# MicahZoltu/lodestar

Measured on AMD Instinct MI355X. Metric: verified signature sets/sec (mainnet attestation mix), higher is better.
Workload: dtype u32 (381-bit Montgomery; device products on 14x28-bit limbs); 1 GPU; c3: gossip attestation flood, 6 slot(s) per batch, 7 batches in flight per GPU; slots_per_batch=6, sets_per_gpu=116736, jobs_per_gpu=104448, pubkeys_per_gpu=1683456, parallelism=dp1 (sets sharded), exchange=False, inflight=7, world_size_seen=1, pubkeys=indices into the GPU-resident table, signing_roots_per_gpu=6918

## Files before the change

### include/lodestar_bls.h

```cpp
#ifndef LODESTAR_BLS_H
#define LODESTAR_BLS_H
#include <stddef.h>
#include <stdint.h>

#ifdef __cplusplus
extern "C" {
#endif

#define LB_OK 0
#define LB_BAD_ENCODING 1
#define LB_POINT_NOT_ON_CURVE 2
#define LB_POINT_NOT_IN_GROUP 3
#define LB_AGGR_TYPE_MISMATCH 4
#define LB_VERIFY_FAIL 5
#define LB_PK_IS_INFINITY 6
#define LB_BAD_SCALAR 7
#define LB_INVALID_SIZE 10
#define LB_EMPTY_AGGREGATE_ARRAY 11
#define LB_EMPTY_SIGNATURE_SET 12
#define LB_ERR_ARGUMENT 100
#define LB_ERR_DEVICE 101
#define LB_ERR_NO_DEVICE 102

typedef struct lb_engine lb_engine;
typedef struct lb_batch lb_batch;

const char* lb_error_name(int32_t code);

int32_t lb_abi_version(void);

int32_t lb_engine_create(int32_t device, lb_engine** out);
#define LB_ENGINE_LATENCY 1u
int32_t lb_engine_create_ex(int32_t device, uint32_t flags, lb_engine** out);
void lb_engine_destroy(lb_engine* e);
int32_t lb_engine_cu_count(const lb_engine* e);

int32_t lb_batch_create(lb_engine* e, uint32_t n_jobs, const uint32_t* job_offsets,
                        const uint32_t* set_pk_offsets, const uint8_t* pubkeys,
                        const uint8_t* signing_roots, const uint8_t* signatures,
                        const uint32_t* sig_sizes, lb_batch** out);
void lb_batch_destroy(lb_batch* b);
uint32_t lb_batch_num_sets(const lb_batch* b);
uint32_t lb_batch_num_jobs(const lb_batch* b);

int32_t lb_batch_verify(lb_engine* e, lb_batch* b, const uint64_t* scalars, int32_t* out_job);

int32_t lb_batch_partial(lb_engine* e, lb_batch* b, const uint64_t* scalars, uint8_t* out576,
                         int32_t* out_job);
int32_t lb_fp12_product_is_one(lb_engine* e, const uint8_t* partials576, uint32_t n, int32_t* ok);
int32_t lb_batch_search_after_partial(lb_engine* e, lb_batch* b, int32_t* out_job);

int32_t lb_verify_jobs(lb_engine* e, uint32_t n_jobs, const uint32_t* job_offsets,
                       const uint32_t* set_pk_offsets, const uint8_t* pubkeys,
                       const uint8_t* signing_roots, const uint8_t* signatures,
                       const uint32_t* sig_sizes, const uint64_t* scalars, int32_t* out_job);
int32_t lb_verify_jobs_indexed(lb_engine* e, uint32_t n_jobs, const uint32_t* job_offsets,
                               const uint32_t* set_pk_offsets, const uint32_t* pk_indices,
                               const uint8_t* signing_roots, const uint8_t* signatures,
                               const uint32_t* sig_sizes, const uint64_t* scalars, int32_t* out_job);

void* lb_host_alloc(size_t bytes);
void lb_host_free(void* p);

int32_t lb_aggregate_pubkeys(lb_engine* e, uint32_t n_sets, const uint32_t* set_pk_offsets,
                             const uint8_t* pubkeys, uint8_t* out96, int32_t* out_status);

int32_t lb_aggregate_signatures(lb_engine* e, uint32_t n_groups, const uint32_t* group_offsets,
                                const uint8_t* sigs96, const uint32_t* sig_sizes, int32_t validate,
                                uint8_t* out96, int32_t* out_status);

int32_t lb_g1_decompress(lb_engine* e, uint32_t n, const uint8_t* in48, uint8_t* out96, int32_t* out_status,
                         int32_t validate);

int32_t lb_merkleize(lb_engine* e, uint32_t n_trees, const uint32_t* chunk_offsets, const uint8_t* chunks32,
                     const uint32_t* depths, const uint64_t* mix_lengths, uint8_t* out_roots32);

int32_t lb_kzg_load_setup(lb_engine* e, const uint8_t* g1_48, uint32_t n_g1, const uint8_t* g2_96, uint32_t n_g2,
                          int32_t* out_status);

int32_t lb_g1_lincomb(lb_engine* e, uint32_t n, const uint8_t* points48, const uint8_t* scalars32, uint8_t* out48);

int32_t lb_kzg_verify_proof(lb_engine* e, const uint8_t* commitment48, const uint8_t* z32, const uint8_t* y32,
                            const uint8_t* proof48, int32_t* ok);

int32_t lb_sk_to_pk(lb_engine* e, uint32_t n, const uint8_t* sks32, uint8_t* out48, uint8_t* out96);
int32_t lb_sign(lb_engine* e, uint32_t n, const uint8_t* sks32, const uint8_t* msgs32, uint8_t* out96);

int32_t lb_pubkey_table_append(lb_engine* e, uint32_t n, const uint8_t* keys, uint32_t key_size, int32_t validate,
                               int32_t* out_status, uint32_t* out_first_index);
uint32_t lb_pubkey_table_size(const lb_engine* e);

int32_t lb_batch_create_indexed(lb_engine* e, uint32_t n_jobs, const uint32_t* job_offsets,
                                const uint32_t* set_pk_offsets, const uint32_t* pk_indices,
                                const uint8_t* signing_roots, const uint8_t* signatures,
                                const uint32_t* sig_sizes, lb_batch** out);

int32_t lb_engine_set_profiling(lb_engine* e, int32_t enable);
int32_t lb_engine_last_profile(lb_engine* e, const char** names, float* ms, int32_t cap, int32_t* n);

#ifdef __cplusplus
}
#endif
#endif
```

### lodestar_amd/_native.py

```python
from __future__ import annotations

import ctypes
import os

LIB_PATH = os.environ.get("LODESTAR_BLS_LIB") or os.path.join(os.path.dirname(os.path.abspath(__file__)),
                                                               "liblodestar_bls.so")

LB_OK = 0
LB_BAD_ENCODING = 1
LB_POINT_NOT_ON_CURVE = 2
LB_POINT_NOT_IN_GROUP = 3
LB_AGGR_TYPE_MISMATCH = 4
LB_VERIFY_FAIL = 5
LB_PK_IS_INFINITY = 6
LB_BAD_SCALAR = 7
LB_INVALID_SIZE = 10
LB_EMPTY_AGGREGATE_ARRAY = 11
LB_EMPTY_SIGNATURE_SET = 12
LB_ERR_ARGUMENT = 100
LB_ERR_DEVICE = 101
LB_ERR_NO_DEVICE = 102


class NativeUnavailable(RuntimeError):
    pass


_u8p = ctypes.POINTER(ctypes.c_uint8)
_u32p = ctypes.POINTER(ctypes.c_uint32)
_u64p = ctypes.POINTER(ctypes.c_uint64)
_i32p = ctypes.POINTER(ctypes.c_int32)
_vp = ctypes.c_void_p

SIGNATURES = {
    "lb_error_name": (ctypes.c_char_p, [ctypes.c_int32]),
    "lb_abi_version": (ctypes.c_int32, []),
    "lb_engine_create": (ctypes.c_int32, [ctypes.c_int32, ctypes.POINTER(_vp)]),
    "lb_engine_create_ex": (ctypes.c_int32, [ctypes.c_int32, ctypes.c_uint32, ctypes.POINTER(_vp)]),
    "lb_engine_destroy": (None, [_vp]),
    "lb_engine_cu_count": (ctypes.c_int32, [_vp]),
    "lb_batch_create": (ctypes.c_int32, [_vp, ctypes.c_uint32, _u32p, _u32p, _u8p, _u8p, _u8p, _u32p,
                                         ctypes.POINTER(_vp)]),
    "lb_batch_destroy": (None, [_vp]),
    "lb_batch_num_sets": (ctypes.c_uint32, [_vp]),
    "lb_batch_num_jobs": (ctypes.c_uint32, [_vp]),
    "lb_batch_verify": (ctypes.c_int32, [_vp, _vp, _u64p, _i32p]),
    "lb_batch_partial": (ctypes.c_int32, [_vp, _vp, _u64p, _u8p, _i32p]),
    "lb_batch_search_after_partial": (ctypes.c_int32, [_vp, _vp, _i32p]),
    "lb_fp12_product_is_one": (ctypes.c_int32, [_vp, _u8p, ctypes.c_uint32, _i32p]),
    "lb_verify_jobs": (ctypes.c_int32, [_vp, ctypes.c_uint32, _u32p, _u32p, _u8p, _u8p, _u8p, _u32p, _u64p,
                                        _i32p]),
    "lb_verify_jobs_indexed": (ctypes.c_int32, [_vp, ctypes.c_uint32, _u32p, _u32p, _u32p, _u8p, _u8p, _u32p,
                                                _u64p, _i32p]),
    "lb_host_alloc": (_vp, [ctypes.c_size_t]),
    "lb_host_free": (None, [_vp]),
    "lb_aggregate_pubkeys": (ctypes.c_int32, [_vp, ctypes.c_uint32, _u32p, _u8p, _u8p, _i32p]),
    "lb_aggregate_signatures": (ctypes.c_int32, [_vp, ctypes.c_uint32, _u32p, _u8p, _u32p, ctypes.c_int32, _u8p,
                                                 _i32p]),
    "lb_g1_decompress": (ctypes.c_int32, [_vp, ctypes.c_uint32, _u8p, _u8p, _i32p, ctypes.c_int32]),
    "lb_merkleize": (ctypes.c_int32, [_vp, ctypes.c_uint32, _u32p, _u8p, _u32p, _u64p, _u8p]),
    "lb_kzg_load_setup": (ctypes.c_int32, [_vp, _u8p, ctypes.c_uint32, _u8p, ctypes.c_uint32, _i32p]),
    "lb_g1_lincomb": (ctypes.c_int32, [_vp, ctypes.c_uint32, _u8p, _u8p, _u8p]),
    "lb_kzg_verify_proof": (ctypes.c_int32, [_vp, _u8p, _u8p, _u8p, _u8p, _i32p]),
    "lb_sk_to_pk": (ctypes.c_int32, [_vp, ctypes.c_uint32, _u8p, _u8p, _u8p]),
    "lb_sign": (ctypes.c_int32, [_vp, ctypes.c_uint32, _u8p, _u8p, _u8p]),
    "lb_pubkey_table_append": (ctypes.c_int32, [_vp, ctypes.c_uint32, _u8p, ctypes.c_uint32, ctypes.c_int32, _i32p,
                                                _u32p]),
    "lb_pubkey_table_size": (ctypes.c_uint32, [_vp]),
    "lb_batch_create_indexed": (ctypes.c_int32, [_vp, ctypes.c_uint32, _u32p, _u32p, _u32p, _u8p, _u8p, _u32p,
                                                 ctypes.POINTER(_vp)]),
    "lb_engine_set_profiling": (ctypes.c_int32, [_vp, ctypes.c_int32]),
    "lb_engine_last_profile": (ctypes.c_int32, [_vp, ctypes.POINTER(ctypes.c_char_p),
                                                ctypes.POINTER(ctypes.c_float), ctypes.c_int32, _i32p]),
}

_lib = None


def load(path: str = LIB_PATH) -> ctypes.CDLL:
    global _lib
    if _lib is not None:
        return _lib
    if not os.path.exists(path):
        raise NativeUnavailable(
            f"{path} not found: build it with `python -m lodestar_amd.build` (hipcc, gfx950)")
    lib = ctypes.CDLL(path)
    for name, (res, args) in SIGNATURES.items():
        fn = getattr(lib, name)
        fn.restype = res
        fn.argtypes = args
    _lib = lib
    return lib


def error_name(code: int) -> str:
    return load().lb_error_name(int(code)).decode()
```

### lodestar_amd/build.py

```python
from __future__ import annotations

import os
import subprocess
import sys
import time

ROOT = os.path.dirname(os.path.dirname(os.path.abspath(__file__)))
CSRC = os.path.join(ROOT, "lodestar_amd", "csrc")
INC = os.path.join(ROOT, "include")
LIB = os.path.join(ROOT, "lodestar_amd", "liblodestar_bls.so")
HARNESS = os.path.join(ROOT, "build", "lb_harness.so")
CPU_POOL = os.path.join(ROOT, "build", "lb_cpu_pool.so")
HIPCC = os.environ.get("HIPCC", "/opt/rocm/bin/hipcc")


def _sources(*names):
    return [os.path.join(CSRC, n) for n in names]


def _stale(target, deps):
    if not os.path.exists(target):
        return True
    t = os.path.getmtime(target)
    return any(os.path.getmtime(d) > t for d in deps)


def _deps():
    hdrs = [os.path.join(CSRC, f) for f in os.listdir(CSRC)]
    return hdrs + [os.path.join(INC, "lodestar_bls.h")]


def _jobs():
    n = os.cpu_count() or 4
    try:
        n = len(os.sched_getaffinity(0))
    except (AttributeError, OSError):
        pass
    return max(1, min(16, n, int(os.environ.get("MAX_JOBS", "16") or 16)))


def build_lib(force=False, verbose=True, extra_flags=(), out=None):
    out = out or LIB
    if not force and not extra_flags and not _stale(out, _deps()):
        return out
    sys.path.insert(0, os.path.join(ROOT, "tools"))
    import gen_kdecls
    cur = open(gen_kdecls.OUT).read() if os.path.exists(gen_kdecls.OUT) else ""
    if cur != gen_kdecls.render():
        with open(gen_kdecls.OUT, "w") as f:
            f.write(gen_kdecls.render())
    odir = os.path.join(ROOT, "build", "obj" + ("" if out == LIB else "_" + os.path.basename(out)))
    os.makedirs(odir, exist_ok=True)
    base = [HIPCC, "--offload-arch=gfx950", "-O3", "-std=c++17", "-fPIC", "-Wno-unused-result",
            "-Wno-unused-value", "-I" + INC, "-I" + CSRC, *extra_flags]
    units = [(os.path.join(CSRC, "lb_engine.hip"), "99", os.path.join(odir, "engine.o"))]
    units += [(os.path.join(CSRC, "lb_kgroup.hip"), str(g), os.path.join(odir, f"kgroup{g}.o"))
              for g in range(gen_kdecls.N_GROUPS)]
    order = [u for u in units if u[1] in ("3", "6", "8", "9", "7")] + [u for u in units if u[1] not in ("3", "6", "8", "9", "7")]
    running, failed = [], []
    t0 = time.time()
    kdeps = [d for d in _deps() if os.path.basename(d) != "lb_engine.hip"]
    pend = [u for u in order if force or extra_flags or _stale(u[2], _deps() if u[1] == "99" else kdeps)]
    while pend or running:
        while pend and len(running) < _jobs():
            src, g, obj = pend.pop(0)
            cmd = base + ["-DLB_KGROUP=" + g, "-c", src, "-o", obj]
            if verbose:
                print("[build]", " ".join(cmd[-5:]), flush=True)
            running.append((subprocess.Popen(cmd), g, time.time()))
        time.sleep(0.2)
        for r in list(running):
            rc = r[0].poll()
            if rc is not None:
                running.remove(r)
                if verbose:
                    print(f"[build] group {r[1]} done in {time.time() - r[2]:.0f} s (rc {rc})", flush=True)
                if rc != 0:
                    failed.append(r[1])
    if failed:
        raise subprocess.CalledProcessError(1, f"hipcc (groups {failed})")
    cmd = [HIPCC, "--offload-arch=gfx950", "-shared", "-fPIC", *[u[2] for u in units], "-o", out + ".tmp"]
    subprocess.run(cmd, check=True)
    os.replace(out + ".tmp", out)
    if verbose:
        print(f"[build] {out} in {time.time() - t0:.0f} s", flush=True)
    return out


def build_harness(force=False, verbose=True):
    src = os.path.join(ROOT, "tests", "harness", "lb_harness.cpp")
    os.makedirs(os.path.dirname(HARNESS), exist_ok=True)
    if not force and not _stale(HARNESS, _deps() + [src]):
        return HARNESS
    cmd = ["g++", "-O2", "-shared", "-fPIC", "-I" + INC, "-I" + CSRC, src, "-o", HARNESS + ".tmp"]
    if verbose:
        print("[build]", " ".join(cmd), flush=True)
    subprocess.run(cmd, check=True)
    os.replace(HARNESS + ".tmp", HARNESS)
    return HARNESS


def build_cpu_pool(force=False, verbose=True):
    src = os.path.join(ROOT, "oracle", "cpu_pool.cpp")
    if not os.path.exists(src):
        return None
    os.makedirs(os.path.dirname(CPU_POOL), exist_ok=True)
    if not force and not _stale(CPU_POOL, _deps() + [src]):
        return CPU_POOL
    cmd = ["g++", "-O3", "-shared", "-fPIC", "-pthread", "-I" + INC, "-I" + CSRC, src,
           "-o", CPU_POOL + ".tmp"]
    if verbose:
        print("[build]", " ".join(cmd), flush=True)
    subprocess.run(cmd, check=True)
    os.replace(CPU_POOL + ".tmp", CPU_POOL)
    return CPU_POOL


UBENCH = ["fpmul_asm"]


def build_ubench(force=False, verbose=True):
    out = []
    for name in UBENCH:
        src = os.path.join(ROOT, "tools", "ubench", name + ".hip")
        dst = os.path.join(ROOT, "tools", "ubench", name)
        if force or _stale(dst, _deps() + [src]):
            cmd = [HIPCC, "--offload-arch=gfx950", "-O3", "-std=c++17", "-Wno-unused-result", "-Wno-unused-value",
                   "-I" + INC, "-I" + CSRC, src, "-o", dst]
            if verbose:
                print("[build]", " ".join(cmd), flush=True)
            subprocess.run(cmd, check=True)
        out.append(dst)
    return out


NAPI = os.path.join(ROOT, "lodestar_amd", "napi", "lodestar_bls.node")


def build_napi(force=False, verbose=True):
    src = os.path.join(ROOT, "lodestar_amd", "napi", "lb_napi.c")
    hdr = "/usr/include/node/node_api.h"
    if not os.path.exists(hdr):
        return None
    if not force and not _stale(NAPI, [src, LIB, os.path.join(INC, "lodestar_bls.h")]):
        return NAPI
    cmd = ["gcc", "-O2", "-shared", "-fPIC", "-pthread", "-I/usr/include/node", "-I" + INC, src, "-o", NAPI + ".tmp",
           "-L" + os.path.dirname(LIB), "-llodestar_bls", "-Wl,-rpath,$ORIGIN/.."]
    if verbose:
        print("[build]", " ".join(cmd), flush=True)
    subprocess.run(cmd, check=True)
    os.replace(NAPI + ".tmp", NAPI)
    return NAPI


def build_all(force=False):
    build_lib(force)
    build_napi(force)
    build_harness(force)
    build_cpu_pool(force)
    build_ubench(force)


if __name__ == "__main__":
    build_all(force="--force" in sys.argv)
```

### lodestar_amd/csrc/lb_curve.h

```cpp
#pragma once
#include "lb_field.h"

template <class F>
struct jac {
  F x, y, z;
};
template <class F>
struct aff {
  F x, y;
};

typedef jac<fp> g1j;
typedef jac<fp2> g2j;
typedef aff<fp> g1a;
typedef aff<fp2> g2a;

template <class T, class S>
LB_HD aff<T> aff_as(const aff<S>& a) {
  return aff<T>{T{a.x}, T{a.y}};
}
template <class T, class S>
LB_HD jac<T> jac_as(const jac<S>& a) {
  return jac<T>{T{a.x}, T{a.y}, T{a.z}};
}
// ... 22 lines not shown
LB_HD jac<F> jac_neg(const jac<F>& p) {
  return jac<F>{p.x, f_neg(p.y), p.z};
}

template <class F>
LB_HD jac<F> jac_dbl_i(const jac<F>& p) {
  F A = f_sqr(p.x);
  F B = f_sqr(p.y);
  F C = f_sqr(B);
  F D = f_dbl(f_sub(f_sub(f_sqr(f_add(p.x, B)), A), C));
  F E = f_mul3(A);
  F Fv = f_sqr(E);
  jac<F> r;
  r.x = f_sub(Fv, f_dbl(D));
  r.y = f_sub(f_mul(E, f_sub(D, r.x)), f_mul8(C));
  r.z = f_dbl(f_mul(p.y, p.z));
  return r;
}

template <class F>
LB_NI jac<F> jac_dbl(jac<F> p) {
  return jac_dbl_i(p);
}

template <class F, bool kInl = false>
LB_HD jac<F> jac_add_i(const jac<F>& p, const jac<F>& q) {
  if (jac_is_inf(p)) return q;
  if (jac_is_inf(q)) return p;
  F Z1Z1 = f_sqr(p.z);
  F Z2Z2 = f_sqr(q.z);
  F U1 = f_mul(p.x, Z2Z2);
  F U2 = f_mul(q.x, Z1Z1);
  F S1 = f_mul(f_mul(p.y, q.z), Z2Z2);
  F S2 = f_mul(f_mul(q.y, p.z), Z1Z1);
  F H = f_sub(U2, U1);
  F rr = f_dbl(f_sub(S2, S1));
  if (f_is_zero(H)) {
    if (f_is_zero(rr)) {
      if constexpr (kInl) return jac_dbl_i(p);
      else return jac_dbl(p);
    }
    return jac_infinity<F>();
  }
  F I = f_sqr(f_dbl(H));
  F J = f_mul(H, I);
  F V = f_mul(U1, I);
  jac<F> r;
  r.x = f_sub(f_sub(f_sqr(rr), J), f_dbl(V));
  r.y = f_sub(f_mul(rr, f_sub(V, r.x)), f_dbl(f_mul(S1, J)));
  r.z = f_mul(f_sub(f_sub(f_sqr(f_add(p.z, q.z)), Z1Z1), Z2Z2), H);
  return r;
}

template <class F>
LB_NI jac<F> jac_add(jac<F> p, jac<F> q) {
  return jac_add_i(p, q);
}

template <class F, bool kInl = false>
LB_HD jac<F> jac_add_aff_i(const jac<F>& p, const aff<F>& q) {
  if (jac_is_inf(p)) return jac_from_aff(q);
  F Z1Z1 = f_sqr(p.z);
  F U2 = f_mul(q.x, Z1Z1);
  F S2 = f_mul(f_mul(q.y, p.z), Z1Z1);
  F H = f_sub(U2, p.x);
  F rr = f_dbl(f_sub(S2, p.y));
  if (f_is_zero(H)) {
    if (f_is_zero(rr)) {
      if constexpr (kInl) return jac_dbl_i(p);
      else return jac_dbl(p);
    }
    return jac_infinity<F>();
  }
  F HH = f_sqr(H);
  F I = f_dbl(f_dbl(HH));
  F J = f_mul(H, I);
  F V = f_mul(p.x, I);
  jac<F> r;
  r.x = f_sub(f_sub(f_sqr(rr), J), f_dbl(V));
  r.y = f_sub(f_mul(rr, f_sub(V, r.x)), f_dbl(f_mul(p.y, J)));
  r.z = f_sub(f_sub(f_sqr(f_add(p.z, H)), Z1Z1), HH);
  return r;
}

template <class F>
LB_NI jac<F> jac_add_aff(jac<F> p, aff<F> q) {
  return jac_add_aff_i(p, q);
}

template <class F>
LB_NI bool jac_eq(jac<F> p, jac<F> q) {
  bool pi = jac_is_inf(p), qi = jac_is_inf(q);
  if (pi || qi) return pi && qi;
  F Z1Z1 = f_sqr(p.z), Z2Z2 = f_sqr(q.z);
  if (!f_eq(f_mul(p.x, Z2Z2), f_mul(q.x, Z1Z1))) return false;
  return f_eq(f_mul(f_mul(p.y, q.z), Z2Z2), f_mul(f_mul(q.y, p.z), Z1Z1));
}

template <class F>
LB_NI bool jac_to_aff(aff<F>& out, jac<F> p) {
  F zi = f_inv(p.z);
  F zi2 = f_sqr(zi);
  out.x = f_mul(p.x, zi2);
  out.y = f_mul(f_mul(p.y, zi2), zi);
  return !jac_is_inf(p);
}

LB_HD void g1_to_aff_inl(g1a& out, const g1j& p) {
  const fp zi = fp_inv_i(p.z), zi2 = fp_sqr(zi);
  out.x = fp_mul(p.x, zi2);
  out.y = fp_mul(fp_mul(p.y, zi2), zi);
}
LB_HD void g2_to_aff_inl(g2a& out, const g2j& p) {
  const fp ni = fp_inv_i(fp_add(fp_sqr(p.z.c0), fp_sqr(p.z.c1)));
  const fp2 zi{fp_mul(p.z.c0, ni), fp_neg(fp_mul(p.z.c1, ni))};
  const fp2 zi2 = fp2_sqr(zi);
  out.x = fp2_mul(p.x, zi2);
  out.y = fp2_mul(fp2_mul(p.y, zi2), zi);
}

template <class F>
LB_NI jac<F> jac_mul_u64(aff<F> p, uint64_t k) {
  jac<F> acc = jac_infinity<F>();
  for (int i = 63; i >= 0; i--) {
    acc = jac_dbl_i(acc);
    if ((k >> i) & 1ull) acc = jac_add_aff_i(acc, p);
  }
  return acc;
}

template <class F, bool kInl = false>
LB_HD jac<F> jac_mul_2d_i(const aff<F>& t1, const aff<F>& t2, const aff<F>& t3, uint64_t k0, uint64_t k1, int bits) {
  jac<F> acc = jac_infinity<F>();
  for (int i = bits - 1; i >= 0; i--) {
    acc = jac_dbl_i(acc);
    const uint32_t d = (uint32_t)((k0 >> i) & 1u) | ((uint32_t)((k1 >> i) & 1u) << 1);
    aff<F> t;
    t.x = d == 1u ? t1.x : (d == 2u ? t2.x : t3.x);
    t.y = d == 1u ? t1.y : (d == 2u ? t2.y : t3.y);
    jac<F> s = jac_add_aff_i<F, kInl>(acc, t);
    if (d != 0u) acc = s;
  }
  return acc;
}
template <class F, bool kInl = false>
LB_HD jac<F> jac_mul_glv_i(const aff<F>& t1, const aff<F>& t2, const aff<F>& t3, uint64_t w) {
  return jac_mul_2d_i<F, kInl>(t1, t2, t3, w & 0xffffffffu, w >> 32, 32);
}
template <class F>
LB_NI jac<F> jac_mul_glv(aff<F> t1, aff<F> t2, aff<F> t3, uint64_t w) {
  return jac_mul_glv_i(t1, t2, t3, w);
}

template <class F>
LB_NI jac<F> jac_mul_u64_jac(jac<F> p, uint64_t k) {
  jac<F> acc = jac_infinity<F>();
  for (int i = 63; i >= 0; i--) {
    acc = jac_dbl_i(acc);
    if ((k >> i) & 1ull) acc = jac_add_i(acc, p);
  }
  return acc;
}

template <class F>
LB_NI jac<F> jac_mul_u256(aff<F> p, const uint32_t* k) {
  jac<F> acc = jac_infinity<F>();
  for (int i = 255; i >= 0; i--) {
    acc = jac_dbl_i(acc);
    if ((k[i >> 5] >> (i & 31)) & 1u) acc = jac_add_aff_i(acc, p);
  }
  return acc;
}

template <class F, bool kInl = false>
LB_HD jac<F> jac_mul_xabs_i(const jac<F>& p) {
  jac<F> acc = p;
  for (int i = 62; i >= 0; i--) {
    acc = jac_dbl_i(acc);
    if ((LB_X_ABS >> i) & 1ull) acc = jac_add_i<F, kInl>(acc, p);
  }
  return acc;
}
template <class F>
LB_NI jac<F> jac_mul_xabs(jac<F> p) {
  return jac_mul_xabs_i(p);
}

LB_HD g2j g2_psi(const g2j& p) {
  g2j r;
  r.x = fp2_mul(fp2_conj(p.x), fp2_load(LB_PSI_CX));
  r.y = fp2_mul(fp2_conj(p.y), fp2_load(LB_PSI_CY));
  r.z = fp2_conj(p.z);
  return r;
}
LB_HD g2j g2_psi2(const g2j& p) {
  g2j r;
  r.x = fp2_mul_fp(p.x, fp_load(LB_PSI2_CX));
  r.y = fp2_mul_fp(p.y, fp_load(LB_PSI2_CY));
  r.z = p.z;
  return r;
}

LB_HD bool g2_in_subgroup(const g2j& p) {
  if (jac_is_inf(p)) return true;
  g2j xp = jac_neg(jac_mul_xabs(p));
  return jac_eq(g2_psi(p), xp);
}

template <bool kInl>
LB_HD fp lean_mul(const fp& a, const fp& b) {
#if defined(__HIP_DEVICE_COMPILE__)
  if constexpr (kInl) {
    __builtin_amdgcn_sched_barrier(0);
    fp r = fp_mul28(a, b);
    __builtin_amdgcn_sched_barrier(0);
    return r;
  }
#endif
  return fp_mul(a, b);
}
template <bool kInl>
LB_HD fp lean_sqr(const fp& a) {
#if defined(__HIP_DEVICE_COMPILE__)
  if constexpr (kInl) {
    __builtin_amdgcn_sched_barrier(0);
    fp r = fp_sqr28(a);
    __builtin_amdgcn_sched_barrier(0);
    return r;
  }
#endif
  return fp_sqr(a);
}
template <bool kInl>
LB_HD fp2 lean2_mul(const fp2& a, const fp2& b) {
  fp t0 = lean_mul<kInl>(a.c0, b.c0);
  fp t1 = lean_mul<kInl>(a.c1, b.c1);
  fp t2 = lean_mul<kInl>(fp_add(a.c0, a.c1), fp_add(b.c0, b.c1));
  return fp2{fp_sub(t0, t1), fp_sub(fp_sub(t2, t0), t1)};
}
template <bool kInl>
LB_HD fp2 lean2_sqr(const fp2& a) {
  fp t0 = lean_mul<kInl>(fp_add(a.c0, a.c1), fp_sub(a.c0, a.c1));
  fp t1 = lean_mul<kInl>(a.c0, a.c1);
  return fp2{t0, fp_dbl(t1)};
}
template <bool kInl>
LB_HD void g2_dbl_lean(g2j& p) {
  p.z = fp2_dbl(lean2_mul<kInl>(p.y, p.z));
  fp2 B = lean2_sqr<kInl>(p.y);
  fp2 C = lean2_sqr<kInl>(B);
  fp2 A = lean2_sqr<kInl>(p.x);
  fp2 D = lean2_sqr<kInl>(fp2_add(p.x, B));
  D = fp2_dbl(fp2_sub(fp2_sub(D, A), C));
  fp2 E = fp2_mul3(A);
  p.x = fp2_sub(lean2_sqr<kInl>(E), fp2_dbl(D));
  p.y = fp2_sub(lean2_mul<kInl>(E, fp2_sub(D, p.x)), fp2_mul8(C));
}
template <bool kInl>
LB_HD void g2_add_aff_lean(g2j& p, const g2a& q) {
  fp2 Z1Z1 = lean2_sqr<kInl>(p.z);
  fp2 H = fp2_sub(lean2_mul<kInl>(q.x, Z1Z1), p.x);
  fp2 rr = lean2_mul<kInl>(lean2_mul<kInl>(q.y, p.z), Z1Z1);
  rr = fp2_dbl(fp2_sub(rr, p.y));
  if (fp2_is_zero(H)) {
    if (fp2_is_zero(rr)) {
      g2_dbl_lean<kInl>(p);
    } else {
      p = jac_infinity<fp2>();
    }
    return;
  }
  fp2 HH = lean2_sqr<kInl>(H);
  p.z = fp2_sub(fp2_sub(lean2_sqr<kInl>(fp2_add(p.z, H)), Z1Z1), HH);
  fp2 I = fp2_mul4(HH);
  fp2 J = lean2_mul<kInl>(H, I);
  fp2 V = lean2_mul<kInl>(p.x, I);
  fp2 YJ = fp2_dbl(lean2_mul<kInl>(p.y, J));
  p.x = fp2_sub(fp2_sub(lean2_sqr<kInl>(rr), J), fp2_dbl(V));
  p.y = fp2_sub(lean2_mul<kInl>(rr, fp2_sub(V, p.x)), YJ);
}

template <bool kInl>
LB_HD void g2_add_lean(g2j& p, const g2j& q) {
  if (jac_is_inf(q)) return;
  if (jac_is_inf(p)) {
    p = q;
    return;
  }
  const fp2 Z1Z1 = lean2_sqr<kInl>(p.z), Z2Z2 = lean2_sqr<kInl>(q.z);
  const fp2 ZZ = fp2_sub(fp2_sub(lean2_sqr<kInl>(fp2_add(p.z, q.z)), Z1Z1), Z2Z2);
  const fp2 U1 = lean2_mul<kInl>(p.x, Z2Z2);
  const fp2 S1 = lean2_mul<kInl>(lean2_mul<kInl>(p.y, q.z), Z2Z2);
  const fp2 H = fp2_sub(lean2_mul<kInl>(q.x, Z1Z1), U1);
  const fp2 rr = fp2_dbl(fp2_sub(lean2_mul<kInl>(lean2_mul<kInl>(q.y, p.z), Z1Z1), S1));
  if (fp2_is_zero(H)) {
    if (fp2_is_zero(rr)) {
      p = q;
      g2_dbl_lean<kInl>(p);
    } else {
      p = jac_infinity<fp2>();
    }
    return;
  }
  p.z = lean2_mul<kInl>(ZZ, H);
  const fp2 I = lean2_sqr<kInl>(fp2_dbl(H));
  const fp2 J = lean2_mul<kInl>(H, I);
// ... 39 lines not shown
```

### lodestar_amd/csrc/lb_engine.hip

```cpp
#include <hip/hip_runtime.h>
#include <hip/hip_ext.h>
#include <stdio.h>
#include <stdlib.h>
#include <string.h>
#include <sys/random.h>

#include <algorithm>
#include <chrono>
#include <cstdio>
#include <cstdlib>
#include <atomic>
#include <mutex>
#include <string>
#include <vector>

#include "lb_kernels.h"
#include "lb_kzg.h"
#include "lb_kdecl.h"

#define LB_ABI_VERSION 1

namespace {

struct dbuf {
  void* p = nullptr;
  size_t cap = 0;
  bool view = false;
  hipError_t ensure(size_t bytes) {
    if (view) {
      p = nullptr;
      cap = 0;
      view = false;
    }
    if (bytes <= cap) return hipSuccess;
    if (p) hipFree(p);
    p = nullptr;
    cap = 0;
    size_t want = bytes + bytes / 4 + 4096;
    hipError_t e = hipMalloc(&p, want);
    if (e == hipSuccess) cap = want;
    return e;
  }
  void release() {
    if (p && !view) hipFree(p);
    p = nullptr;
    cap = 0;
    view = false;
  }
  void set_view(void* q, size_t bytes) {
    if (p && !view) hipFree(p);
    p = q;
    cap = bytes;
    view = true;
  }
  template <class T>
  T* as() const { return reinterpret_cast<T*>(p); }
};

enum {
  ST_DECODE = 0,
  ST_DEDUP,
  ST_HASH_MAP,
  ST_HASH_FIN,
  ST_PK_CHUNKS,
  ST_PK_BLIND,
  ST_SIG_MSM,
  ST_GSUM,
  ST_MILLER,
  ST_TREE_P,
  ST_ML_S,
  ST_ROOT,
  ST_FALLBACK,
  ST_BISECT,
  ST_TOTAL,
  kStages
};
const char* const kStageNames[kStages] = {"decode_sigs", "dedup",   "hash_map", "hash_finish", "pk_chunks",
                                          "pk_blind",    "sig_msm", "group_sum", "miller",    "tree_up_P",
                                          "ml_S",        "root_check", "search_msm", "search_check", "total"};

}

struct lb_batch {
  uint32_t n_jobs = 0, n_sets = 0, n_pks = 0;
  uint64_t serial = 0;
  std::vector<uint32_t> job_off;
  std::vector<uint32_t> h_set_chunk_off, h_chunk_lo;
  uint32_t n_chunks = 0;
  bool indexed = false;
  dbuf d_job_off, d_pk_off, d_pks, d_msgs, d_sigs, d_sig_sizes, d_set_chunk_off, d_chunk_lo;
  dbuf d_arena;
  bool has_sizes = false;
  int device = 0;
  ~lb_batch() {
    d_job_off.release();
    d_arena.release();
    d_pk_off.release();
    d_pks.release();
    d_msgs.release();
    d_sigs.release();
    d_sig_sizes.release();
    d_set_chunk_off.release();
    d_chunk_lo.release();
  }
};

#ifndef LB_SEARCH_CHUNK_DEF
#define LB_SEARCH_CHUNK_DEF 8
#endif
struct lb_engine {
  int device = 0;
  bool latency = false;
  int n_cus = 0;
  hipStream_t stream = nullptr;
  hipStream_t stream2 = nullptr;
  hipStream_t stream3 = nullptr;
  hipStream_t hp[3] = {nullptr, nullptr, nullptr};
  uint32_t prio_max = 0;
  hipEvent_t ev_g1 = nullptr, ev_s = nullptr, ev_fork = nullptr, ev_dec = nullptr, ev_pk = nullptr;
  hipEvent_t ev_pkst = nullptr;
  hipEvent_t ev_sdec = nullptr, ev_sblind = nullptr;
  std::mutex mu;
  dbuf scalars, sig_aff, sig_inf, sig_status, q, h_aff, rpk, rsig, pk_status, ml, treeP, treeS, job_status,
      nodes, verdict, parts, ok, chunk_acc, chunk_status, fS;
  dbuf msg_tab, rep_of, uid_of, uniq_set, n_u, set_uid, gcnt, gpos, goff, gch, chunk_beg, chunk_end, members,
      set_live, gacc, gp_aff, gp_inf, chunk_root;
  uint32_t gmax_chunks = 0;
  bool straus = false, straus_run = false, rpk_stale = false;
  bool gsum_wave = true;
  dbuf pk3, corder;
  bool gsum_tree = true;
  bool alone = false, row_fe = true;
  int alone_force = -1;
  uint32_t gchunk = LB_GROUP_CHUNK;
  dbuf sig_aos, bcnt, bcursor, boff, bch, bchunk_beg, bchunk_end, bmembers, bacc, bsum, wsum;
  dbuf park;
  bool spec_gsum = false;
  dbuf set_spec, live_flag;
  uint32_t* h_flag = nullptr;
  uint64_t partial_serial = 0;
  uint32_t partial_mu = 0;
  bool msm_g8 = true;
  dbuf sx[32];
  dbuf pk_aff;
  dbuf y_root;
  uint64_t msg_key = 0;
  uint32_t miller_wave_max = 2048;
  uint32_t row_max = 256;
  int miller_form = 0;
  uint32_t miller_lds3_max = 32768;
  uint32_t hash_g8_max = 2048;
  uint32_t hash_row_max = 256;
  uint32_t hash_row_careful = 0;
  bool row_proj = true;
  bool small_par = true;
  uint32_t dec_row_max = 4096;
  uint32_t subgroup_g8_max = 4096;
  uint32_t small_s_max = 32768;
  uint32_t small_s_g8_max = 2048;
  uint32_t search_small_max = 32768;
  bool search_merge = true;
  dbuf s_terms, s_part;
  dbuf s_root, rs_idx, s_set;
  bool search_rootsum = true;
  bool search_pre = false;
  int smsm_form = 0;
  uint32_t search_chunk = LB_SEARCH_CHUNK_DEF;
  bool search_blk = true;
  bool root_shuffle = true;
  std::vector<uint64_t> h_scalars;
  dbuf table;
  uint32_t table_n = 0, table_cap = 0;
  dbuf kzg_g1, kzg_g2;
  uint32_t kzg_n = 0;
  bool profiling = false;
  hipEvent_t ev0[kStages] = {}, ev1[kStages] = {};
  bool used[kStages] = {};
  float last_ms[kStages] = {};
  float acc_ms[kStages] = {};
  uint32_t* h_nu = nullptr;
  void* h_stage = nullptr;
  size_t h_stage_cap = 0;
  lb_batch* scratch = nullptr;
};

static std::mutex g_engine_mu;
static int g_engine_count[64];
static std::atomic<uint64_t> g_batch_serial{0};
#ifndef LB_HASH_ALONE_G8
#define LB_HASH_ALONE_G8 1
#endif
static std::atomic<int> g_device_busy[64];
struct exit_rec {
  const void* eng = nullptr;
  int64_t ns = 0;
};
static std::mutex g_exit_mu[64];
static exit_rec g_device_exit[64][2];
static int64_t lb_now_ns() {
  return std::chrono::duration_cast<std::chrono::nanoseconds>(std::chrono::steady_clock::now().time_since_epoch()).count();
}
static int g_latency_cus[64];
static int g_latency_live[64];
struct busy_scope {
  int dev;
  const void* eng;
  bool counted;
  busy_scope(int d, const void* e, bool latency = false) : dev(d), eng(e), counted(!latency) {
    if (counted) g_device_busy[dev].fetch_add(1, std::memory_order_relaxed);
  }
  ~busy_scope() {
    if (!counted) return;
    {
      std::lock_guard<std::mutex> lk(g_exit_mu[dev]);
      exit_rec* r = g_device_exit[dev];
      if (r[0].eng != eng) r[1] = r[0];
      r[0] = exit_rec{eng, lb_now_ns()};
    }
    g_device_busy[dev].fetch_sub(1, std::memory_order_relaxed);
  }
};
#ifndef LB_ALONE_GRACE_MS
#define LB_ALONE_GRACE_MS 20
#endif
template <class E>
static bool device_alone(const E* e) {
  if (e->latency) return true;
  if (e->alone_force >= 0) return e->alone_force != 0;
  if (g_device_busy[e->device].load(std::memory_order_relaxed) > 1) return false;
  int64_t other;
  {
    std::lock_guard<std::mutex> lk(g_exit_mu[e->device]);
    const exit_rec* r = g_device_exit[e->device];
    other = r[0].eng != (const void*)e ? r[0].ns : r[1].ns;
  }
  return other == 0 || lb_now_ns() - other > (int64_t)LB_ALONE_GRACE_MS * 1000000;
}
static int max_engines_per_device() {
  const char* v = getenv("LB_MAX_ENGINES_PER_DEVICE");
  int k = v ? atoi(v) : 0;
  return k > 0 ? k : 10;
}

#define LB_HIP(call)                                                                        \
  do {                                                                                      \
    hipError_t _e = (call);                                                                 \
    if (_e != hipSuccess) {                                                                 \
      fprintf(stderr, "lodestar_bls: %s failed: %s (%s:%d)\n", #call, hipGetErrorString(_e), \
              __FILE__, __LINE__);                                                          \
      return LB_ERR_DEVICE;                                                                 \
    }                                                                                       \
  } while (0)

static inline uint32_t nblk(uint32_t n) { return (n + LB_TPB - 1) / LB_TPB; }
static inline uint32_t nblk_inv(uint32_t n) { return (n + LB_INV_TPB - 1) / LB_INV_TPB; }

static int fill_scalars(lb_engine* e, uint32_t n, const uint64_t* user, bool unblinded) {
  e->h_scalars.resize(n);
  if (!user && n == 1 && unblinded) {
    e->h_scalars[0] = 1;
    return LB_OK;
  }
  if (user) {
    for (uint32_t i = 0; i < n; i++)
      if (user[i] == 0) return LB_BAD_SCALAR;
    memcpy(e->h_scalars.data(), user, (size_t)n * 8);
  } else {
    size_t need = (size_t)n * 8, got = 0;
    uint8_t* dst = reinterpret_cast<uint8_t*>(e->h_scalars.data());
    while (got < need) {
      ssize_t r = getrandom(dst + got, need - got, 0);
      if (r < 0) return LB_ERR_DEVICE;
      got += (size_t)r;
    }
    for (uint32_t i = 0; i < n; i++)
      while (e->h_scalars[i] == 0) getrandom(&e->h_scalars[i], 8, 0);
  }
  return LB_OK;
}

extern "C" {

int32_t lb_abi_version(void) { return LB_ABI_VERSION; }

const char* lb_error_name(int32_t code) {
  switch (code) {
    case LB_OK: return "BLST_SUCCESS";
    case LB_BAD_ENCODING: return "BLST_BAD_ENCODING";
    case LB_POINT_NOT_ON_CURVE: return "BLST_POINT_NOT_ON_CURVE";
    case LB_POINT_NOT_IN_GROUP: return "BLST_POINT_NOT_IN_GROUP";
    case LB_AGGR_TYPE_MISMATCH: return "BLST_AGGR_TYPE_MISMATCH";
    case LB_VERIFY_FAIL: return "BLST_VERIFY_FAIL";
    case LB_PK_IS_INFINITY: return "BLST_PK_IS_INFINITY";
    case LB_BAD_SCALAR: return "BLST_BAD_SCALAR";
    case LB_INVALID_SIZE: return "BLST_INVALID_SIZE";
    case LB_EMPTY_AGGREGATE_ARRAY: return "EMPTY_AGGREGATE_ARRAY";
    case LB_EMPTY_SIGNATURE_SET: return "Empty signature set";
    case LB_ERR_ARGUMENT: return "LB_ERR_ARGUMENT";
    case LB_ERR_DEVICE: return "LB_ERR_DEVICE";
    case LB_ERR_NO_DEVICE: return "LB_ERR_NO_DEVICE";
    default: return "LB_UNKNOWN_ERROR";
  }
}

int32_t lb_engine_create(int32_t device, lb_engine** out) { return lb_engine_create_ex(device, 0u, out); }
static std::vector<uint32_t> cu_mask(int ncu, int lo, int hi) {
  std::vector<uint32_t> m((size_t)(ncu + 31) / 32, 0u);
  for (int c = lo; c < hi && c < ncu; c++) m[(size_t)c / 32] |= 1u << (c % 32);
  return m;
}
int32_t lb_engine_create_ex(int32_t device, uint32_t flags, lb_engine** out) {
  if (!out || (flags & ~LB_ENGINE_LATENCY)) return LB_ERR_ARGUMENT;
  *out = nullptr;
  int count = 0;
  if (hipGetDeviceCount(&count) != hipSuccess || count == 0) return LB_ERR_NO_DEVICE;
  if (device < 0) LB_HIP(hipGetDevice(&device));
  if (device >= count) return LB_ERR_NO_DEVICE;
  hipDeviceProp_t prop;
  LB_HIP(hipGetDeviceProperties(&prop, device));
  if (strncmp(prop.gcnArchName, "gfx950", 6) != 0) {
    fprintf(stderr, "lodestar_bls: device %d is %s, this build targets gfx950 only\n", device, prop.gcnArchName);
    return LB_ERR_NO_DEVICE;
  }
  LB_HIP(hipSetDevice(device));
  if (device >= 64) return LB_ERR_NO_DEVICE;
  {
    std::lock_guard<std::mutex> lk(g_engine_mu);
    if (g_engine_count[device] >= max_engines_per_device()) {
      fprintf(stderr, "lodestar_bls: engine limit (%d per device) reached on device %d\n", max_engines_per_device(),
              device);
      return LB_ERR_DEVICE;
    }
    g_engine_count[device]++;
  }
  lb_engine* e = new lb_engine();
  e->device = device;
  while (getrandom(&e->msg_key, 8, 0) != 8) {
  }
  int prio_least = 0, prio_greatest = 0;
  hipDeviceGetStreamPriorityRange(&prio_least, &prio_greatest);
  if (const char* mw = getenv("LB_MILLER_WAVE_MAX")) e->miller_wave_max = (uint32_t)strtoul(mw, nullptr, 10);
  if (const char* rm = getenv("LB_ROW_MAX")) e->row_max = (uint32_t)strtoul(rm, nullptr, 10);
  if (const char* gt = getenv("LB_GSUM_TREE")) e->gsum_tree = std::atoi(gt) != 0;
  if (const char* gs = getenv("LB_GSUM_STRAUS")) e->straus = std::atoi(gs) != 0;
  if (const char* gw = getenv("LB_GSUM_WAVE")) e->gsum_wave = std::atoi(gw) != 0;
  if (const char* rf = getenv("LB_ROW_FE")) e->row_fe = std::atoi(rf) != 0;
  if (const char* pm = getenv("LB_PRIO_MAX")) e->prio_max = (uint32_t)strtoul(pm, nullptr, 10);
  if (const char* ml = getenv("LB_MILLER_LDS3_MAX")) e->miller_lds3_max = (uint32_t)strtoul(ml, nullptr, 10);
  if (const char* mf = getenv("LB_MILLER_FORM")) e->miller_form = !strcmp(mf, "lane") ? 1 : !strcmp(mf, "g8") ? 2 : 0;
  if (const char* hg = getenv("LB_HASH_G8_MAX")) e->hash_g8_max = (uint32_t)strtoul(hg, nullptr, 10);
  if (const char* hr = getenv("LB_HASH_ROW_MAX")) e->hash_row_max = (uint32_t)strtoul(hr, nullptr, 10);
  if (const char* dr = getenv("LB_DEC_ROW_MAX")) e->dec_row_max = (uint32_t)strtoul(dr, nullptr, 10);
  if (const char* hc = getenv("LB_HASH_ROW_CAREFUL")) e->hash_row_careful = (uint32_t)strtoul(hc, nullptr, 10);
  if (const char* rp = getenv("LB_ROW_PROJ")) e->row_proj = std::atoi(rp) != 0;
  if (const char* sp = getenv("LB_SMALL_PAR")) e->small_par = std::atoi(sp) != 0;
  if (const char* sg = getenv("LB_SUBGROUP_G8_MAX")) e->subgroup_g8_max = (uint32_t)strtoul(sg, nullptr, 10);
  if (const char* ss = getenv("LB_SMALL_S_MAX")) e->small_s_max = (uint32_t)strtoul(ss, nullptr, 10);
  if (const char* sg8 = getenv("LB_SMALL_S_G8_MAX")) e->small_s_g8_max = (uint32_t)strtoul(sg8, nullptr, 10);
  if (const char* sm = getenv("LB_SEARCH_SMALL_MAX")) e->search_small_max = (uint32_t)strtoul(sm, nullptr, 10);
  if (const char* sm = getenv("LB_SEARCH_MERGE")) e->search_merge = std::atoi(sm) != 0;
  if (const char* sm = getenv("LB_SEARCH_ROOTSUM")) e->search_rootsum = std::atoi(sm) != 0;
  if (const char* sm = getenv("LB_SEARCH_PRE")) e->search_pre = std::atoi(sm) != 0;
  if (const char* sf = getenv("LB_SMSM_FORM")) e->smsm_form = !strcmp(sf, "lane") ? 1 : !strcmp(sf, "g8") ? 2 : 0;
  if (const char* sc = getenv("LB_SEARCH_CHUNK")) {
    const uint32_t v = (uint32_t)strtoul(sc, nullptr, 10);
    if (v >= 1 && v <= 64) e->search_chunk = v;
  }
  if (const char* sm = getenv("LB_SEARCH_BLOCKS")) e->search_blk = std::atoi(sm) != 0;
  if (const char* sm = getenv("LB_ROOT_SHUFFLE")) e->root_shuffle = std::atoi(sm) != 0;
  if (const char* sm = getenv("LB_MSM_G8")) e->msm_g8 = std::atoi(sm) != 0;
  if (const char* sm = getenv("LB_SPEC_GSUM")) e->spec_gsum = std::atoi(sm) != 0;
  if (const char* al = getenv("LB_ALONE")) e->alone_force = std::atoi(al) != 0 ? 1 : 0;
  bool masked = false;
  std::vector<uint32_t> mask;
  {
    std::lock_guard<std::mutex> lk(g_engine_mu);
    const int ncu = prop.multiProcessorCount;
    e->n_cus = ncu;
    if (flags & LB_ENGINE_LATENCY) {
      if (g_latency_cus[device] == 0) {
        const char* v = getenv("LB_LATENCY_CUS");
        const int r = v ? atoi(v) : 8;
        g_latency_cus[device] = std::max(1, std::min(r, ncu / 4));
        if (g_engine_count[device] > 1)
          fprintf(stderr, "lodestar_bls: latency engine created after %d other engine(s) on device %d: "
                  "those still run on every CU (create the latency engine first)\n", g_engine_count[device] - 1, device);
      }
      g_latency_live[device]++;
      e->latency = true;
      mask = cu_mask(ncu, 0, g_latency_cus[device]);
      e->n_cus = g_latency_cus[device];
      masked = true;
    } else if (g_latency_cus[device] > 0) {
      mask = cu_mask(ncu, g_latency_cus[device], ncu);
      e->n_cus = ncu - g_latency_cus[device];
      masked = true;
    }
  }
  auto mk = [&](hipStream_t* st, bool prio) {
    if (masked) return hipExtStreamCreateWithCUMask(st, (uint32_t)mask.size(), mask.data());
    return prio ? hipStreamCreateWithPriority(st, hipStreamNonBlocking, prio_least)
                : hipStreamCreateWithFlags(st, hipStreamNonBlocking);
  };
  if (mk(&e->stream, true) != hipSuccess || mk(&e->stream2, false) != hipSuccess || mk(&e->stream3, false) != hipSuccess ||

      hipHostMalloc((void**)&e->h_nu, 8, hipHostMallocDefault) != hipSuccess ||
      hipHostMalloc((void**)&e->h_flag, 4, hipHostMallocDefault) != hipSuccess) {
    if (e->stream) hipStreamDestroy(e->stream);
    if (e->stream2) hipStreamDestroy(e->stream2);
    if (e->stream3) hipStreamDestroy(e->stream3);
    if (e->h_nu) hipHostFree(e->h_nu);
    std::lock_guard<std::mutex> lk(g_engine_mu);
    g_engine_count[device]--;
    if (e->latency && --g_latency_live[device] == 0) g_latency_cus[device] = 0;
    delete e;
    return LB_ERR_DEVICE;
  }
  hipEventCreateWithFlags(&e->ev_g1, hipEventDisableTiming);
  hipEventCreateWithFlags(&e->ev_s, hipEventDisableTiming);
  hipEventCreateWithFlags(&e->ev_fork, hipEventDisableTiming);
  hipEventCreateWithFlags(&e->ev_dec, hipEventDisableTiming);
  hipEventCreateWithFlags(&e->ev_pk, hipEventDisableTiming);
  hipEventCreateWithFlags(&e->ev_pkst, hipEventDisableTiming);
  hipEventCreateWithFlags(&e->ev_sdec, hipEventDisableTiming);
  hipEventCreateWithFlags(&e->ev_sblind, hipEventDisableTiming);
  for (int i = 0; i < kStages; i++) {
    hipEventCreate(&e->ev0[i]);
    hipEventCreate(&e->ev1[i]);
  }
  {
    bool ok;
    {
      std::lock_guard<std::mutex> lk(g_engine_mu);
      ok = e->n_u.ensure(4) == hipSuccess && hipMemsetAsync(e->n_u.p, 0, 4, e->stream) == hipSuccess;
      if (ok) {
        hipLaunchKernelGGL(k_miller_lane<2>, dim3(4096), dim3(LB_TPB), 0, e->stream, 0u, 1u, e->n_u.as<uint32_t>(),
                           nullptr, nullptr, nullptr, nullptr, nullptr);
        hipLaunchKernelGGL(k_hash_finish, dim3(4096), dim3(LB_INV_TPB), 0, e->stream, 0u, e->n_u.as<uint32_t>(),
                           nullptr, nullptr, nullptr, 0u);
        const char* rv = getenv("LB_RESERVE_S23");
        const int res23 = rv ? atoi(rv) : 2;
        if (res23 >= 1) {
          hipLaunchKernelGGL(k_decompress_sigs, dim3(4096), dim3(LB_TPB), 0, e->stream2, 0u, nullptr, nullptr, nullptr,
                             nullptr, nullptr, nullptr);
          hipLaunchKernelGGL(k_pk_chunks, dim3(4096), dim3(LB_TPB), 0, e->stream3, 0u, nullptr, nullptr, nullptr, nullptr);
          hipLaunchKernelGGL(k_pk_blind_rowp, dim3(std::max<uint32_t>(1u, e->row_max)), dim3(64), 0, e->stream3,
                             0u, nullptr, nullptr, nullptr, nullptr);
        }
        if (res23 >= 2) {
          auto g8_waves = [](uint32_t sets) { return dim3(std::min<uint32_t>(16384u, std::max<uint32_t>(1u, sets / 8 + 1))); };
          hipLaunchKernelGGL(k_sig_subgroup_g8, g8_waves(e->subgroup_g8_max), dim3(64), 0, e->stream2, 0u, nullptr,
                             nullptr, nullptr);
          hipLaunchKernelGGL(k_sig_blind_g8, g8_waves(e->small_s_g8_max), dim3(64), 0, e->stream2, 0u, nullptr, nullptr,
                             nullptr, nullptr, nullptr);
        }
        ok = hipGetLastError() == hipSuccess && hipStreamSynchronize(e->stream) == hipSuccess &&
             hipStreamSynchronize(e->stream2) == hipSuccess && hipStreamSynchronize(e->stream3) == hipSuccess;
      }
    }
    if (!ok) {
      fprintf(stderr, "lodestar_bls: engine scratch reservation failed on device %d\n", device);
      lb_engine_destroy(e);
      return LB_ERR_DEVICE;
    }
  }
  *out = e;
  return LB_OK;
}

void lb_engine_destroy(lb_engine* e) {
  if (!e) return;
  hipSetDevice(e->device);
  hipStreamSynchronize(e->stream);
  dbuf* bufs[] = {&e->scalars, &e->sig_aff, &e->sig_inf, &e->sig_status, &e->q, &e->h_aff, &e->rpk, &e->rsig,
                  &e->pk_status, &e->ml, &e->treeP, &e->treeS, &e->job_status, &e->nodes, &e->verdict, &e->parts,
                  &e->ok, &e->chunk_acc, &e->chunk_status, &e->fS, &e->table, &e->msg_tab,
                  &e->rep_of, &e->uid_of, &e->uniq_set, &e->n_u, &e->set_uid, &e->gcnt, &e->gpos, &e->goff,
                  &e->gch, &e->chunk_beg, &e->chunk_end, &e->members, &e->set_live, &e->gacc, &e->gp_aff,
                  &e->gp_inf, &e->chunk_root, &e->sig_aos, &e->bcnt, &e->bcursor, &e->boff, &e->bch, &e->bchunk_beg,
                  &e->bchunk_end, &e->bmembers, &e->bacc, &e->bsum, &e->wsum, &e->park, &e->set_spec, &e->live_flag, &e->pk_aff, &e->y_root, &e->kzg_g1,
                  &e->kzg_g2, &e->s_terms, &e->s_part, &e->s_root, &e->rs_idx, &e->s_set, &e->pk3, &e->corder};
  for (dbuf* b : bufs) b->release();
  for (dbuf& b : e->sx) b.release();
  for (int i = 0; i < kStages; i++) {
    if (e->ev0[i]) hipEventDestroy(e->ev0[i]);
    if (e->ev1[i]) hipEventDestroy(e->ev1[i]);
  }
  hipEventDestroy(e->ev_g1);
  hipEventDestroy(e->ev_s);
  hipEventDestroy(e->ev_fork);
  hipEventDestroy(e->ev_dec);
  hipEventDestroy(e->ev_pk);
  if (e->ev_pkst) hipEventDestroy(e->ev_pkst);
  if (e->ev_sdec) hipEventDestroy(e->ev_sdec);
  if (e->ev_sblind) hipEventDestroy(e->ev_sblind);
  hipStreamSynchronize(e->stream2);
  hipStreamSynchronize(e->stream3);
  if (e->scratch) delete e->scratch;
  if (e->h_nu) hipHostFree(e->h_nu);
  if (e->h_flag) hipHostFree(e->h_flag);
  if (e->h_stage) hipHostFree(e->h_stage);
  hipStreamDestroy(e->stream2);
  hipStreamDestroy(e->stream3);
  hipStreamDestroy(e->stream);
  for (hipStream_t h : e->hp)
    if (h) {
      hipStreamSynchronize(h);
      hipStreamDestroy(h);
    }
  {
    std::lock_guard<std::mutex> lk(g_engine_mu);
    g_engine_count[e->device]--;
    if (e->latency && --g_latency_live[e->device] == 0) g_latency_cus[e->device] = 0;
  }
  delete e;
}

int32_t lb_engine_cu_count(const lb_engine* e) { return e ? e->n_cus : 0; }

int32_t lb_engine_set_profiling(lb_engine* e, int32_t enable) {
  if (!e) return LB_ERR_ARGUMENT;
  e->profiling = enable != 0;
  return LB_OK;
}

int32_t lb_engine_last_profile(lb_engine* e, const char** names, float* ms, int32_t cap, int32_t* n) {
  if (!e || !n) return LB_ERR_ARGUMENT;
  int k = cap < kStages ? cap : kStages;
  for (int i = 0; i < k; i++) {
    if (names) names[i] = kStageNames[i];
    if (ms) ms[i] = e->last_ms[i];
  }
  *n = k;
  return LB_OK;
}

}

static constexpr size_t kStageMax = (size_t)1 << 20;
static int32_t batch_fill(lb_engine* e, lb_batch* b, uint32_t n_jobs, const uint32_t* job_offsets,
                          const uint32_t* set_pk_offsets, const uint8_t* pubkeys, const uint32_t* pk_indices,
                          const uint8_t* signing_roots, const uint8_t* signatures, const uint32_t* sig_sizes) {
  if (!e || !job_offsets || !set_pk_offsets) return LB_ERR_ARGUMENT;
  if (job_offsets[0] != 0) return LB_ERR_ARGUMENT;
  for (uint32_t j = 0; j < n_jobs; j++)
    if (job_offsets[j + 1] < job_offsets[j]) return LB_ERR_ARGUMENT;
  const uint32_t n_sets = job_offsets[n_jobs];
  if (set_pk_offsets[0] != 0) return LB_ERR_ARGUMENT;
  for (uint32_t i = 0; i < n_sets; i++)
    if (set_pk_offsets[i + 1] < set_pk_offsets[i]) return LB_ERR_ARGUMENT;
  const uint32_t n_pks = set_pk_offsets[n_sets];
  if (n_pks & LB_CHUNK_FIRST) return LB_ERR_ARGUMENT;
  const bool indexed = pk_indices != nullptr;
  if ((n_sets && (!signing_roots || !signatures)) || (n_pks && !pubkeys && !indexed)) return LB_ERR_ARGUMENT;
  LB_HIP(hipSetDevice(e->device));
  b->device = e->device;
  b->serial = g_batch_serial.fetch_add(1, std::memory_order_relaxed) + 1;
  b->n_jobs = n_jobs;
  b->n_sets = n_sets;
  b->n_pks = n_pks;
  b->job_off.assign(job_offsets, job_offsets + n_jobs + 1);
  b->has_sizes = sig_sizes != nullptr;
  auto up = [&](dbuf& d, const void* src, size_t bytes) -> hipError_t {
    hipError_t r = d.ensure(bytes ? bytes : 16);
    if (r != hipSuccess || !bytes) return r;
    return hipMemcpyAsync(d.p, src, bytes, hipMemcpyHostToDevice, e->stream);
  };
  std::vector<uint32_t>& set_chunk_off = b->h_set_chunk_off;
  std::vector<uint32_t>& chunk_lo = b->h_chunk_lo;
  set_chunk_off.resize(n_sets + 1);
  chunk_lo.clear();
  const uint32_t pkc = n_sets <= e->row_max ? LB_PK_CHUNK_SMALL : LB_PK_CHUNK;
  for (uint32_t i = 0; i < n_sets; i++) {
    set_chunk_off[i] = (uint32_t)chunk_lo.size();
    for (uint32_t k = set_pk_offsets[i]; k < set_pk_offsets[i + 1]; k += pkc)
      chunk_lo.push_back(k | (k == set_pk_offsets[i] ? LB_CHUNK_FIRST : 0u));
  }
  set_chunk_off[n_sets] = (uint32_t)chunk_lo.size();
  b->n_chunks = (uint32_t)chunk_lo.size();
  chunk_lo.push_back(n_pks | LB_CHUNK_FIRST);
  b->indexed = indexed;
  struct part {
    dbuf* d;
    const void* src;
    size_t bytes;
  };
  const part parts[] = {{&b->d_job_off, job_offsets, (size_t)(n_jobs + 1) * 4},
                        {&b->d_set_chunk_off, set_chunk_off.data(), set_chunk_off.size() * 4},
                        {&b->d_chunk_lo, chunk_lo.data(), chunk_lo.size() * 4},
                        {&b->d_pk_off, set_pk_offsets, (size_t)(n_sets + 1) * 4},
                        {&b->d_pks, indexed ? (const void*)pk_indices : (const void*)pubkeys,
                         (size_t)n_pks * (indexed ? 4 : 96)},
                        {&b->d_msgs, signing_roots, (size_t)n_sets * 32},
                        {&b->d_sigs, signatures, (size_t)n_sets * 96},
                        {&b->d_sig_sizes, sig_sizes, sig_sizes ? (size_t)n_sets * 4 : 0}};
  size_t total = 0;
  for (const part& q : parts) total += ((q.bytes > 16 ? q.bytes : 16) + 255) & ~(size_t)255;
  bool staged = total <= kStageMax;
  if (staged && e->h_stage_cap < total) {
    if (e->h_stage) hipHostFree(e->h_stage);
    e->h_stage = nullptr;
    e->h_stage_cap = 0;
    if (hipHostMalloc(&e->h_stage, kStageMax, hipHostMallocDefault) == hipSuccess) e->h_stage_cap = kStageMax;
    else staged = false;
  }
  hipError_t r = hipSuccess;
  if (staged) {
    r = b->d_arena.ensure(total);
    size_t off = 0;
    for (const part& q : parts) {
      if (q.bytes) memcpy(static_cast<uint8_t*>(e->h_stage) + off, q.src, q.bytes);
      off += ((q.bytes > 16 ? q.bytes : 16) + 255) & ~(size_t)255;
    }
    if (r == hipSuccess) r = hipMemcpyAsync(b->d_arena.p, e->h_stage, total, hipMemcpyHostToDevice, e->stream);
    off = 0;
    for (const part& q : parts) {
      const size_t sz = ((q.bytes > 16 ? q.bytes : 16) + 255) & ~(size_t)255;
      if (r == hipSuccess && (q.bytes || q.d != &b->d_sig_sizes)) q.d->set_view(static_cast<uint8_t*>(b->d_arena.p) + off, sz);
      off += sz;
    }
  } else {
    for (const part& q : parts)
      if (r == hipSuccess && (q.bytes || q.d != &b->d_sig_sizes)) r = up(*q.d, q.src, q.bytes);
  }
  if (r == hipSuccess) r = hipStreamSynchronize(e->stream);
  if (r != hipSuccess) {
    for (const part& q : parts) q.d->release();
    b->d_arena.release();
    b->n_jobs = b->n_sets = b->n_pks = b->n_chunks = 0;
    b->job_off.assign(1, 0u);
    fprintf(stderr, "lodestar_bls: batch upload failed: %s\n", hipGetErrorString(r));
    return LB_ERR_DEVICE;
  }
  return LB_OK;
}

static int32_t batch_create(lb_engine* e, uint32_t n_jobs, const uint32_t* job_offsets, const uint32_t* set_pk_offsets,
                            const uint8_t* pubkeys, const uint32_t* pk_indices, const uint8_t* signing_roots,
                            const uint8_t* signatures, const uint32_t* sig_sizes, lb_batch** out) {
  if (!e || !out) return LB_ERR_ARGUMENT;
  *out = nullptr;
  std::lock_guard<std::mutex> lk(e->mu);
  lb_batch* b = new lb_batch();
  int32_t st = batch_fill(e, b, n_jobs, job_offsets, set_pk_offsets, pubkeys, pk_indices, signing_roots, signatures,
                          sig_sizes);
  if (st != LB_OK) {
    delete b;
    return st;
  }
  *out = b;
  return LB_OK;
}

static const uint32_t kNoIndices[1] = {0};
static int32_t check_null_indices(uint32_t n_jobs, const uint32_t* job_offsets, const uint32_t* set_pk_offsets) {
  if (!job_offsets || !set_pk_offsets) return LB_ERR_ARGUMENT;
  return set_pk_offsets[job_offsets[n_jobs]] == 0 ? LB_OK : LB_ERR_ARGUMENT;
}

extern "C" {

int32_t lb_batch_create(lb_engine* e, uint32_t n_jobs, const uint32_t* job_offsets, const uint32_t* set_pk_offsets,
                        const uint8_t* pubkeys, const uint8_t* signing_roots, const uint8_t* signatures,
                        const uint32_t* sig_sizes, lb_batch** out) {
  return batch_create(e, n_jobs, job_offsets, set_pk_offsets, pubkeys, nullptr, signing_roots, signatures, sig_sizes,
                      out);
}

int32_t lb_batch_create_indexed(lb_engine* e, uint32_t n_jobs, const uint32_t* job_offsets,
                                const uint32_t* set_pk_offsets, const uint32_t* pk_indices,
                                const uint8_t* signing_roots, const uint8_t* signatures, const uint32_t* sig_sizes,
                                lb_batch** out) {
  if (!pk_indices) {
    const int32_t st = check_null_indices(n_jobs, job_offsets, set_pk_offsets);
    if (st != LB_OK) return st;
    pk_indices = kNoIndices;
  }
  return batch_create(e, n_jobs, job_offsets, set_pk_offsets, nullptr, pk_indices, signing_roots, signatures,
                      sig_sizes, out);
}

void* lb_host_alloc(size_t bytes) {
  void* p = nullptr;
  if (hipHostMalloc(&p, bytes ? bytes : 1, hipHostMallocDefault) != hipSuccess) return nullptr;
  return p;
}

void lb_host_free(void* p) {
  if (p) hipHostFree(p);
}

uint32_t lb_pubkey_table_size(const lb_engine* e) { return e ? e->table_n : 0; }

int32_t lb_pubkey_table_append(lb_engine* e, uint32_t n, const uint8_t* keys, uint32_t key_size, int32_t validate,
                               int32_t* out_status, uint32_t* out_first_index) {
  if (!e || (n && (!keys || !out_status)) || (key_size != 48 && key_size != 96)) return LB_ERR_ARGUMENT;
  std::lock_guard<std::mutex> lk(e->mu);
  LB_HIP(hipSetDevice(e->device));
  const uint32_t first = e->table_n;
  if (out_first_index) *out_first_index = first;
  if (!n) return LB_OK;
  const uint32_t need = first + n;
  if (need > e->table_cap) {
    uint32_t cap = e->table_cap ? e->table_cap : 1024;
    while (cap < need) cap *= 2;
    dbuf nt;
    LB_HIP(nt.ensure((size_t)cap * LB_TABLE_REC * 4));
    if (first)
      LB_HIP(hipMemcpyAsync(nt.p, e->table.p, (size_t)first * LB_TABLE_REC * 4, hipMemcpyDeviceToDevice, e->stream));
    LB_HIP(hipStreamSynchronize(e->stream));
    e->table.release();
    e->table = nt;
    e->table_cap = cap;
  }
  dbuf kin, st;
  hipError_t r = kin.ensure((size_t)n * key_size);
  if (r == hipSuccess) r = st.ensure((size_t)n * 4);
  if (r == hipSuccess) r = hipMemcpyAsync(kin.p, keys, (size_t)n * key_size, hipMemcpyHostToDevice, e->stream);
  if (r == hipSuccess) {
    hipLaunchKernelGGL(k_table_fill, dim3(nblk(n)), dim3(LB_TPB), 0, e->stream, n, kin.as<uint8_t>(), key_size,
                       validate, first, e->table.as<uint32_t>(), st.as<int32_t>());
    r = hipGetLastError();
  }
  if (r == hipSuccess) r = hipMemcpyAsync(out_status, st.p, (size_t)n * 4, hipMemcpyDeviceToHost, e->stream);
  if (r == hipSuccess) r = hipStreamSynchronize(e->stream);
  kin.release();
  st.release();
  if (r != hipSuccess) {
    fprintf(stderr, "lodestar_bls: pubkey table append failed: %s\n", hipGetErrorString(r));
    return LB_ERR_DEVICE;
  }
  e->table_n = need;
  return LB_OK;
}

void lb_batch_destroy(lb_batch* b) {
  if (!b) return;
  hipSetDevice(b->device);
  delete b;
}
uint32_t lb_batch_num_sets(const lb_batch* b) { return b ? b->n_sets : 0; }
uint32_t lb_batch_num_jobs(const lb_batch* b) { return b ? b->n_jobs : 0; }

}

struct stage_scope {
  lb_engine* e;
  int k;
  hipStream_t st;
  stage_scope(lb_engine* e_, int k_, hipStream_t st_) : e(e_), k(k_), st(st_) {
    if (e->profiling) {
      hipEventRecord(e->ev0[k], st);
      e->used[k] = true;
    }
  }
  ~stage_scope() {
    if (e->profiling) hipEventRecord(e->ev1[k], st);
  }
};

static hipError_t msm_reduce(lb_engine* e, hipStream_t st, uint32_t bcap, uint32_t nb, uint32_t n_inst, int W,
                             uint32_t* out, uint32_t n_out, uint32_t out0, uint64_t entries, uint32_t chunk) {
  if (e->msm_g8) {
    hipError_t r = e->wsum.ensure((size_t)n_inst * W * sizeof(g2j));
    if (r != hipSuccess) return r;
    if (entries >= (uint64_t)4 * chunk * nb && device_alone(e))
      hipLaunchKernelGGL(k_msm_buckets_g8, dim3(nb), dim3(64), 0, st, e->bch.as<uint32_t>(), e->bacc.as<uint32_t>(),
                         bcap, e->bsum.as<uint32_t>(), nb);
    else
      hipLaunchKernelGGL(k_msm_buckets, dim3(nblk(nb)), dim3(LB_TPB), 0, st, e->bch.as<uint32_t>(),
                         e->bacc.as<uint32_t>(), bcap, e->bsum.as<uint32_t>(), nb);
    hipLaunchKernelGGL(k_msm_window_g8, dim3(n_inst * W), dim3(256), 0, st, e->bsum.as<uint32_t>(), nb,
                       e->wsum.as<uint32_t>(), n_inst * W);
    if (W == LB_MSM_W)
      hipLaunchKernelGGL(k_msm_horner_g8<LB_MSM_W>, dim3((n_inst + 7) / 8), dim3(64), 0, st, e->wsum.as<uint32_t>(),
                         n_inst, out, n_out, out0);
    else
      hipLaunchKernelGGL(k_msm_horner_g8<LB_SMSM_W>, dim3((n_inst + 7) / 8), dim3(64), 0, st, e->wsum.as<uint32_t>(),
                         n_inst, out, n_out, out0);
    return hipGetLastError();
  }
  hipLaunchKernelGGL(k_msm_buckets, dim3(nblk(nb)), dim3(LB_TPB), 0, st, e->bch.as<uint32_t>(), e->bacc.as<uint32_t>(),
                     bcap, e->bsum.as<uint32_t>(), nb);
  if (W == LB_MSM_W)
    hipLaunchKernelGGL(k_msm_reduce<LB_MSM_W>, dim3(n_inst), dim3(64 * LB_MSM_W), 0, st, e->bsum.as<uint32_t>(), nb, out,
                       n_out, out0);
  else
    hipLaunchKernelGGL(k_msm_reduce<LB_SMSM_W>, dim3(n_inst), dim3(64 * LB_SMSM_W), 0, st, e->bsum.as<uint32_t>(), nb,
                       out, n_out, out0);
  return hipGetLastError();
}

static hipError_t per_root_chain(lb_engine* e, uint32_t n, uint32_t nuh, uint32_t mu, const uint32_t* live) {
  hipStream_t s1 = e->stream;
  const uint32_t* nu = e->n_u.as<uint32_t>();
  {
    stage_scope sc(e, ST_GSUM, s1);
    const uint32_t nch = nuh + n / e->gchunk;
    const bool wave = e->gsum_tree && e->alone && e->gsum_wave;
    if (wave)
      hipLaunchKernelGGL(k_gsum_wave, dim3(nblk(nch)), dim3(LB_TPB), 0, s1, n, nu, e->gch.as<uint32_t>(),
                         e->chunk_beg.as<uint32_t>(), e->chunk_end.as<uint32_t>(), e->chunk_root.as<uint32_t>(),
                         e->members.as<uint32_t>(), live, e->rpk.as<uint32_t>(), e->gacc.as<uint32_t>());
    else if (e->straus_run) {
      hipError_t r = e->corder.ensure((size_t)(nch + 2 * (LB_STRAUS_CHUNK + 1)) * 4);
      if (r != hipSuccess) return r;
      uint32_t* cnt = e->corder.as<uint32_t>() + nch;
      r = hipMemsetAsync(cnt, 0, (size_t)2 * (LB_STRAUS_CHUNK + 1) * 4, s1);
      if (r != hipSuccess) return r;
      for (uint32_t pass = 0; pass < 2; pass++)
        hipLaunchKernelGGL(k_chunk_order, dim3(nblk(nch)), dim3(LB_TPB), 0, s1, nu, e->gch.as<uint32_t>(),
                           e->chunk_beg.as<uint32_t>(), e->chunk_end.as<uint32_t>(), cnt, e->corder.as<uint32_t>(), pass);
      hipLaunchKernelGGL(k_gsum_straus, dim3(nblk(nch)), dim3(LB_TPB), 0, s1, n, nu, e->gch.as<uint32_t>(),
                         e->chunk_beg.as<uint32_t>(), e->chunk_end.as<uint32_t>(), e->corder.as<uint32_t>(),
                         e->members.as<uint32_t>(), live, e->pk3.as<uint32_t>(), e->scalars.as<uint64_t>(),
                         e->gacc.as<uint32_t>());
    }
    else
      hipLaunchKernelGGL(k_gsum_chunks, dim3(nblk(nch)), dim3(LB_TPB), 0, s1, n, nu,
                         e->gch.as<uint32_t>(), e->chunk_beg.as<uint32_t>(), e->chunk_end.as<uint32_t>(),
                         e->members.as<uint32_t>(), live, e->rpk.as<uint32_t>(), e->gacc.as<uint32_t>());
    const bool tree = e->gsum_tree && e->alone && !wave;
    for (uint32_t st = 1; tree && st < e->gmax_chunks; st *= LB_GSUM_FAN)
      hipLaunchKernelGGL(k_gsum_tree, dim3(nblk(nch)), dim3(LB_TPB), 0, s1, n, nu, e->gch.as<uint32_t>(),
                         e->chunk_root.as<uint32_t>(), st, e->gacc.as<uint32_t>());
    hipLaunchKernelGGL(k_gsum_final, dim3(nblk_inv(nuh)), dim3(LB_INV_TPB), 0, s1, n, nu, e->gch.as<uint32_t>(),
                       e->gacc.as<uint32_t>(), e->gp_aff.as<uint32_t>(), e->gp_inf.as<uint32_t>(),
                       wave ? 2u : (tree ? 0u : 1u));
  }
  {
    stage_scope sc(e, ST_MILLER, s1);
    const bool shared = e->miller_form == 1 ||
                        (e->miller_form == 0 && !device_alone(e));
    if (nuh <= e->row_max && e->alone && e->row_fe) {
      hipLaunchKernelGGL(k_miller_row, dim3(nuh), dim3(LBR_NT), 0, s1, n, mu, nu, e->gp_aff.as<uint32_t>(),
                         e->gp_inf.as<uint32_t>(), e->h_aff.as<uint32_t>(), e->treeP.as<uint32_t>());
    } else if (nuh <= e->miller_wave_max) {
      hipLaunchKernelGGL(k_miller_wave, dim3(nuh), dim3(64), 0, s1, n, mu, nu, e->gp_aff.as<uint32_t>(),
                         e->gp_inf.as<uint32_t>(), e->h_aff.as<uint32_t>(), e->treeP.as<uint32_t>());
    } else if (shared) {
      hipError_t r = e->park.ensure((size_t)2 * 72 * 4 * n);
      if (r != hipSuccess) return r;
      if (nuh <= e->miller_lds3_max)
        hipLaunchKernelGGL(k_miller_lane<3>, dim3(nblk(nuh)), dim3(LB_TPB), 0, s1, n, mu, nu, e->gp_aff.as<uint32_t>(),
                           e->gp_inf.as<uint32_t>(), e->h_aff.as<uint32_t>(), e->treeP.as<uint32_t>(),
                           e->park.as<uint32_t>());
      else
        hipLaunchKernelGGL(k_miller_lane<2>, dim3(nblk(nuh)), dim3(LB_TPB), 0, s1, n, mu, nu, e->gp_aff.as<uint32_t>(),
                           e->gp_inf.as<uint32_t>(), e->h_aff.as<uint32_t>(), e->treeP.as<uint32_t>(),
                           e->park.as<uint32_t>());
    } else {
      hipLaunchKernelGGL(k_miller_g8, dim3((nuh + LBG_ROOTS - 1) / LBG_ROOTS), dim3(64 * LBG_WAVES), 0, s1, n, mu, nu,
                         e->gp_aff.as<uint32_t>(), e->gp_inf.as<uint32_t>(), e->h_aff.as<uint32_t>(),
                         e->treeP.as<uint32_t>());
    }
  }
  {
    stage_scope sc(e, ST_TREE_P, s1);
    for (uint32_t lo = mu / 2; lo >= 1; lo /= 2) {
      if (lo <= e->row_max && e->alone && e->row_fe)
        hipLaunchKernelGGL(k_tree_up_row, dim3(lo), dim3(LBR_NT), 0, s1, mu, lo, nu, e->treeP.as<uint32_t>());
      else
        hipLaunchKernelGGL(k_tree_up_U, dim3(lo), dim3(64), 0, s1, mu, lo, nu, e->treeP.as<uint32_t>());
    }
  }
  return hipGetLastError();
}

static int32_t run_pipeline(lb_engine* e, lb_batch* b, const uint64_t* scalars, uint32_t& mj, uint32_t& mu,
                            bool unblinded) {
  const uint32_t n = b->n_sets, nj = b->n_jobs;
  e->partial_serial = 0;
  e->alone = device_alone(e);
  e->straus_run = e->straus && !e->alone;
  e->rpk_stale = e->straus_run;
  e->gchunk = (e->alone && e->gsum_tree) ? (e->gsum_wave ? LB_GROUP_CHUNK_WAVE : LB_GROUP_CHUNK_ALONE)
                                          : (e->straus_run ? LB_STRAUS_CHUNK : LB_GROUP_CHUNK);
  const bool one_unblinded = n == 1 && !scalars && unblinded;
  int st = fill_scalars(e, n, scalars, unblinded);
  if (st != LB_OK) return st;
  mj = 1;
  while (mj < nj) mj <<= 1;
  mu = 1;
  while (mu < n) mu <<= 1;
  const uint32_t mt = mj > mu ? mj : mu;
  const uint32_t ns = n ? n : 1;
  uint32_t cap = 64;
  while (cap < 2 * ns) cap <<= 1;
  LB_HIP(e->scalars.ensure((size_t)ns * 8));
  LB_HIP(e->sig_aff.ensure((size_t)ns * sizeof(g2a)));
  LB_HIP(e->sig_inf.ensure((size_t)ns * 4));
  LB_HIP(e->sig_status.ensure((size_t)ns * 4));
  LB_HIP(e->q.ensure((size_t)ns * 2 * sizeof(g2j)));
  LB_HIP(e->h_aff.ensure((size_t)ns * sizeof(g2a)));
  LB_HIP(e->rpk.ensure((size_t)ns * sizeof(g1j)));
  LB_HIP(e->pk_aff.ensure((size_t)ns * sizeof(g1a)));
  LB_HIP(e->pk_status.ensure((size_t)ns * 4));
  LB_HIP(e->treeP.ensure((size_t)2 * mt * sizeof(fp12)));
  LB_HIP(e->treeS.ensure((size_t)2 * mj * sizeof(g2j)));
  LB_HIP(e->job_status.ensure((size_t)(nj ? nj : 1) * 4));
  LB_HIP(e->fS.ensure(sizeof(fp12)));
  LB_HIP(e->msg_tab.ensure((size_t)cap * 4));
  dbuf* per_set[] = {&e->rep_of, &e->uid_of, &e->uniq_set, &e->set_uid, &e->gcnt, &e->gpos, &e->chunk_beg,
                     &e->chunk_end, &e->members, &e->set_live, &e->gp_inf, &e->chunk_root};
  for (dbuf* d : per_set) LB_HIP(d->ensure((size_t)ns * 4));
  LB_HIP(e->goff.ensure((size_t)(ns + 1) * 4));
  LB_HIP(e->gch.ensure((size_t)(ns + 1) * 4));
  LB_HIP(e->n_u.ensure(8));
  LB_HIP(e->gacc.ensure((size_t)ns * sizeof(g1j)));
  LB_HIP(e->gp_aff.ensure((size_t)ns * sizeof(g1a)));
  const uint32_t bcap = (2 * LB_MSM_W * ns) / LB_MSM_CHUNK + LB_MSM_NB;
  LB_HIP(e->sig_aos.ensure((size_t)ns * sizeof(g2a)));
  LB_HIP(e->bcnt.ensure((size_t)LB_MSM_NB * 4));
  LB_HIP(e->bcursor.ensure((size_t)LB_MSM_NB * 4));
  LB_HIP(e->boff.ensure((size_t)(LB_MSM_NB + 1) * 4));
  LB_HIP(e->bch.ensure((size_t)(LB_MSM_NB + 1) * 4));
  LB_HIP(e->bchunk_beg.ensure((size_t)bcap * 4));
  LB_HIP(e->bchunk_end.ensure((size_t)bcap * 4));
  LB_HIP(e->bmembers.ensure((size_t)2 * LB_MSM_W * ns * 4));
  LB_HIP(e->bacc.ensure((size_t)bcap * sizeof(g2j)));
  LB_HIP(e->bsum.ensure((size_t)LB_MSM_NB * sizeof(g2j)));
  const uint32_t nc = b->n_chunks;
  LB_HIP(e->chunk_acc.ensure((size_t)(nc ? nc : 1) * sizeof(g1j)));
  LB_HIP(e->chunk_status.ensure((size_t)(nc ? nc : 1) * 4));
  for (int k = 0; k < kStages; k++) {
    e->used[k] = false;
    e->acc_ms[k] = 0.f;
  }
  hipStream_t s1 = e->stream, s2 = e->stream2, s3_ = e->stream3;
  if (e->profiling) {
    hipEventRecord(e->ev0[ST_TOTAL], s1);
    e->used[ST_TOTAL] = true;
  }
  if (n) LB_HIP(hipMemcpyAsync(e->scalars.p, e->h_scalars.data(), (size_t)n * 8, hipMemcpyHostToDevice, s1));
  LB_HIP(hipEventRecord(e->ev_fork, s1));
  LB_HIP(hipStreamWaitEvent(s2, e->ev_fork, 0));
  LB_HIP(hipStreamWaitEvent(s3_, e->ev_fork, 0));
  const uint32_t* nu = e->n_u.as<uint32_t>();
  if (n) {
    const hipStream_t s3 = (e->spec_gsum || n <= e->small_s_max) ? s3_ : s2;
    {
      stage_scope sc(e, ST_PK_CHUNKS, s3);
      if (nc && b->indexed)
        hipLaunchKernelGGL(k_pk_chunks_idx, dim3(nblk(nc)), dim3(LB_TPB), 0, s3, nc, b->d_chunk_lo.as<uint32_t>(),
                           b->d_pks.as<uint32_t>(), e->table.as<uint32_t>(), e->table_n, e->chunk_acc.as<uint32_t>(),
                           e->chunk_status.as<int32_t>());
      else if (nc)
        hipLaunchKernelGGL(k_pk_chunks, dim3(nblk(nc)), dim3(LB_TPB), 0, s3, nc, b->d_chunk_lo.as<uint32_t>(),
                           b->d_pks.as<uint8_t>(), e->chunk_acc.as<uint32_t>(), e->chunk_status.as<int32_t>());
    }
    const bool pk_split = s3 != s2;
    const bool pk_rowp = e->small_par && pk_split && !e->straus_run && n <= e->row_max && e->alone && e->row_fe;
    const bool sb_par = e->small_par && pk_split && !one_unblinded && n <= e->small_s_max && n <= e->small_s_g8_max &&
                        n <= e->row_max && e->alone && e->row_fe && !e->straus_run;
    {
      stage_scope sc(e, ST_PK_BLIND, s3);
      const uint32_t m0 = (pk_split || e->straus_run) ? 1u : 0u;
      const uint32_t m1 = e->straus_run ? 1u : (pk_split ? 2u : 0u);
      if (e->straus_run) LB_HIP(e->pk3.ensure((size_t)ns * sizeof(g1x3)));
      for (uint32_t mode = m0; mode <= m1; mode++) {
        if (mode == 2u && pk_rowp) {
          hipLaunchKernelGGL(k_pk_blind_rowp, dim3(n), dim3(64), 0, s3, n, e->pk_aff.as<uint32_t>(),
                             e->scalars.as<uint64_t>(), e->rpk.as<uint32_t>(), e->pk_status.as<int32_t>());
          continue;
        }
        hipLaunchKernelGGL(k_pk_blind, dim3(nblk_inv(n)), dim3(LB_INV_TPB), 0, s3, n, nc, b->d_set_chunk_off.as<uint32_t>(),
                           e->chunk_acc.as<uint32_t>(), e->chunk_status.as<int32_t>(), e->pk_aff.as<uint32_t>(),
                           e->scalars.as<uint64_t>(), e->rpk.as<uint32_t>(), e->pk_status.as<int32_t>(), mode,
                           (mode == 1u && e->straus_run) ? e->pk3.as<uint32_t>() : nullptr);
        if (mode == 1u) LB_HIP(hipEventRecord(e->ev_pkst, s3));
      }
    }
    LB_HIP(hipEventRecord(e->ev_pk, s3));
    {
      stage_scope sc(e, ST_DECODE, s2);
      if (n <= e->dec_row_max && e->alone && e->row_fe)
        hipLaunchKernelGGL(k_decompress_sigs_row, dim3(LB_H2C_FOLD ? (n + 1) / 2 : (n + 3) / 4), dim3(64), 0, s2, n, b->d_sigs.as<uint8_t>(),
                           b->has_sizes ? b->d_sig_sizes.as<uint32_t>() : nullptr, e->sig_aff.as<uint32_t>(),
                           e->sig_aos.as<uint4>(), e->sig_inf.as<uint32_t>(), e->sig_status.as<int32_t>());
      else
        hipLaunchKernelGGL(k_decompress_sigs, dim3(nblk(n)), dim3(LB_TPB), 0, s2, n, b->d_sigs.as<uint8_t>(),
                           b->has_sizes ? b->d_sig_sizes.as<uint32_t>() : nullptr, e->sig_aff.as<uint32_t>(),
                           e->sig_aos.as<uint4>(), e->sig_inf.as<uint32_t>(), e->sig_status.as<int32_t>());
      if (sb_par) LB_HIP(hipEventRecord(e->ev_sdec, s2));
      if (n <= e->row_max && e->alone && e->row_fe && e->small_par)
        hipLaunchKernelGGL(k_sig_subgroup_w4, dim3(n), dim3(64), 0, s2, n, e->sig_aff.as<uint32_t>(),
                           e->sig_inf.as<uint32_t>(), e->sig_status.as<int32_t>());
      else if (n <= e->row_max && e->alone && e->row_fe)
        hipLaunchKernelGGL(k_sig_subgroup_row, dim3(n), dim3(LBR_NT), 0, s2, n, e->sig_aff.as<uint32_t>(),
                           e->sig_inf.as<uint32_t>(), e->sig_status.as<int32_t>(), e->row_proj ? 1u : 0u);
      else if (n <= e->subgroup_g8_max)
        hipLaunchKernelGGL(k_sig_subgroup_g8, dim3((n + 7) / 8), dim3(64), 0, s2, n, e->sig_aff.as<uint32_t>(),
                           e->sig_inf.as<uint32_t>(), e->sig_status.as<int32_t>());
      else
        hipLaunchKernelGGL(k_sig_subgroup, dim3(nblk(n)), dim3(LB_TPB), 0, s2, n, e->sig_aff.as<uint32_t>(),
                           e->sig_inf.as<uint32_t>(), e->sig_status.as<int32_t>());
      LB_HIP(hipStreamWaitEvent(s2, pk_split ? e->ev_pkst : e->ev_pk, 0));
      hipLaunchKernelGGL(k_job_status, dim3(nblk(nj)), dim3(LB_TPB), 0, s2, nj, b->d_job_off.as<uint32_t>(),
                         e->sig_status.as<int32_t>(), e->pk_status.as<int32_t>(), e->job_status.as<int32_t>(),
                         e->set_live.as<uint32_t>());
    }
    LB_HIP(hipEventRecord(e->ev_dec, s2));
    if (sb_par) {
      LB_HIP(hipStreamWaitEvent(s3, e->ev_sdec, 0));
      if (e->profiling) {
        hipEventRecord(e->ev0[ST_SIG_MSM], s3);
        e->used[ST_SIG_MSM] = true;
      }
      LB_HIP(e->s_terms.ensure((size_t)n * sizeof(g2j)));
      hipLaunchKernelGGL(k_sig_blind_w4, dim3(n), dim3(64), 0, s3, n, e->sig_aff.as<uint32_t>(),
                         e->scalars.as<uint64_t>(), e->sig_inf.as<uint32_t>(), e->s_terms.as<uint32_t>());
      LB_HIP(hipEventRecord(e->ev_sblind, s3));
    }
    {
      stage_scope sc(e, ST_DEDUP, s1);
      if (n == 1) {
        hipLaunchKernelGGL(k_dedup_one, dim3(1), dim3(64), 0, s1, e->rep_of.as<uint32_t>(), e->uid_of.as<uint32_t>(),
                           e->uniq_set.as<uint32_t>(), e->n_u.as<uint32_t>(), e->set_uid.as<uint32_t>(),
                           e->gcnt.as<uint32_t>(), e->gpos.as<uint32_t>(), e->goff.as<uint32_t>(), e->gch.as<uint32_t>(),
                           e->chunk_beg.as<uint32_t>(), e->chunk_end.as<uint32_t>(), e->chunk_root.as<uint32_t>(),
                           e->members.as<uint32_t>());
      } else {
        LB_HIP(hipMemsetAsync(e->msg_tab.p, 0xff, (size_t)cap * 4, s1));
        LB_HIP(hipMemsetAsync(e->n_u.p, 0, 4, s1));
        LB_HIP(hipMemsetAsync(e->gcnt.p, 0, (size_t)n * 4, s1));
        hipLaunchKernelGGL(k_msg_insert, dim3(nblk(n)), dim3(LB_TPB), 0, s1, n, b->d_msgs.as<uint8_t>(), e->msg_key,
                           cap, e->msg_tab.as<uint32_t>(), e->rep_of.as<uint32_t>());
        if (e->root_shuffle)
          hipLaunchKernelGGL(k_msg_uid, dim3(nblk(cap)), dim3(LB_TPB), 0, s1, cap, e->msg_tab.as<uint32_t>(),
                             e->uid_of.as<uint32_t>(), e->uniq_set.as<uint32_t>(), e->n_u.as<uint32_t>());
        else {
          std::vector<uint32_t> rep(n), uid(n, 0xffffffffu), uniq, suid(n), cnt, pos(n);
          LB_HIP(hipMemcpyAsync(rep.data(), e->rep_of.p, (size_t)n * 4, hipMemcpyDeviceToHost, s1));
          LB_HIP(hipStreamSynchronize(s1));
          for (uint32_t i = 0; i < n; i++) {
            const uint32_t r = rep[i];
            if (uid[r] == 0xffffffffu) {
              uid[r] = (uint32_t)uniq.size();
              uniq.push_back(r);
              cnt.push_back(0);
            }
            suid[i] = uid[r];
            pos[i] = cnt[uid[r]]++;
          }
          const uint32_t nun = (uint32_t)uniq.size();
          LB_HIP(hipMemcpyAsync(e->uid_of.p, uid.data(), (size_t)n * 4, hipMemcpyHostToDevice, s1));
          LB_HIP(hipMemcpyAsync(e->uniq_set.p, uniq.data(), (size_t)nun * 4, hipMemcpyHostToDevice, s1));
          LB_HIP(hipMemcpyAsync(e->set_uid.p, suid.data(), (size_t)n * 4, hipMemcpyHostToDevice, s1));
          LB_HIP(hipMemcpyAsync(e->gcnt.p, cnt.data(), (size_t)nun * 4, hipMemcpyHostToDevice, s1));
          LB_HIP(hipMemcpyAsync(e->gpos.p, pos.data(), (size_t)n * 4, hipMemcpyHostToDevice, s1));
          LB_HIP(hipMemcpyAsync(e->n_u.p, &nun, 4, hipMemcpyHostToDevice, s1));
          LB_HIP(hipStreamSynchronize(s1));
        }
        if (e->root_shuffle)
          hipLaunchKernelGGL(k_msg_count, dim3(nblk(n)), dim3(LB_TPB), 0, s1, n, e->rep_of.as<uint32_t>(),
                             e->uid_of.as<uint32_t>(), e->set_uid.as<uint32_t>(), e->gcnt.as<uint32_t>(),
                             e->gpos.as<uint32_t>());
        hipLaunchKernelGGL(k_msg_scan, dim3(1), dim3(1024), 0, s1, nu, 0u, e->gchunk, e->gcnt.as<uint32_t>(), e->goff.as<uint32_t>(),
                           e->gch.as<uint32_t>(), nullptr, nullptr, nullptr, e->n_u.as<uint32_t>() + 1);
        hipLaunchKernelGGL(k_chunk_fill, dim3(nblk(n + n / e->gchunk + 1)), dim3(LB_TPB), 0, s1, nu,
                           e->gchunk, e->goff.as<uint32_t>(), e->gch.as<uint32_t>(),
                           e->chunk_beg.as<uint32_t>(), e->chunk_end.as<uint32_t>(), e->chunk_root.as<uint32_t>());
        hipLaunchKernelGGL(k_msg_scatter, dim3(nblk(n)), dim3(LB_TPB), 0, s1, n, e->set_uid.as<uint32_t>(),
                           e->gpos.as<uint32_t>(), e->goff.as<uint32_t>(), e->members.as<uint32_t>());
      }
      if (n == 1) {
        e->h_nu[0] = 1;
        e->h_nu[1] = 1;
      } else {
        LB_HIP(hipMemcpyAsync(e->h_nu, e->n_u.p, 8, hipMemcpyDeviceToHost, s1));
        LB_HIP(hipStreamSynchronize(s1));
      }
    }
    const uint32_t nuh = e->h_nu[0];
    e->gmax_chunks = e->h_nu[1];
    if (nuh == 0 || nuh > n) return LB_ERR_DEVICE;
    mu = 1;
    while (mu < nuh) mu <<= 1;
    {
      stage_scope sc(e, ST_HASH_MAP, s1);
      if (nuh <= e->hash_row_max && e->alone && e->row_fe)
        hipLaunchKernelGGL(k_hash_map_row, dim3(LB_H2C_FOLD ? (LBR_FP2_W4 ? 2 * nuh : nuh) : (2 * nuh + 3) / 4), dim3(64), 0, s1, n, nuh,
                           e->uniq_set.as<uint32_t>(), b->d_msgs.as<uint8_t>(), e->q.as<uint32_t>());
      else
        hipLaunchKernelGGL(k_hash_map, dim3(nblk(2 * nuh)), dim3(LB_TPB), 0, s1, n, nuh, e->uniq_set.as<uint32_t>(),
                           b->d_msgs.as<uint8_t>(), e->q.as<uint32_t>());
    }
    {
      stage_scope sc(e, ST_HASH_FIN, s1);
      const bool alone = e->miller_form == 0 && device_alone(e);
      if (nuh <= e->hash_row_max && e->alone && e->row_fe)
        hipLaunchKernelGGL(k_hash_finish_row, dim3(nuh), dim3(LBR_NT), 0, s1, n, nu, e->q.as<uint32_t>(),
                           e->h_aff.as<uint32_t>(), e->hash_row_careful ? 1u : (e->row_proj ? 0u : 2u));
      else if (nuh <= e->hash_g8_max || (LB_HASH_ALONE_G8 && alone))
        hipLaunchKernelGGL(k_hash_finish_g8, dim3((nuh + 7) / 8), dim3(64), 0, s1, n, nu, e->q.as<uint32_t>(),
                           e->h_aff.as<uint32_t>());
      else
      {
        const uint32_t pn = nblk_inv(nuh) * LB_INV_TPB;
        LB_HIP(e->park.ensure((size_t)4 * 72 * 4 * (pn > n ? pn : n)));
        hipLaunchKernelGGL(k_hash_finish, dim3(nblk_inv(nuh)), dim3(LB_INV_TPB), 0, s1, n, nu, e->q.as<uint32_t>(),
                           e->h_aff.as<uint32_t>(), e->park.as<uint32_t>(), pn);
      }
    }
    if (sb_par) {
      LB_HIP(hipStreamWaitEvent(s2, e->ev_sblind, 0));
      hipLaunchKernelGGL(k_g2_sum_g8, dim3(1), dim3(8 * LB_SUM_G8_GROUPS), 0, s2, n, e->s_terms.as<uint32_t>(),
                         2 * mj, e->treeS.as<uint32_t>(), 1u, e->set_live.as<uint32_t>());
      if (e->profiling) hipEventRecord(e->ev1[ST_SIG_MSM], s2);
    } else if (one_unblinded) {
      stage_scope sc(e, ST_SIG_MSM, s2);
      hipLaunchKernelGGL(k_sig_unblinded, dim3(1), dim3(64), 0, s2, e->sig_aff.as<uint32_t>(),
                         e->set_live.as<uint32_t>(), e->sig_inf.as<uint32_t>(), 2 * mj, e->treeS.as<uint32_t>());
    } else if (n <= e->small_s_max) {
      stage_scope sc(e, ST_SIG_MSM, s2);
      LB_HIP(e->s_terms.ensure((size_t)n * sizeof(g2j)));
      LB_HIP(e->s_part.ensure((size_t)((n + 63) / 64) * sizeof(g2j)));
      if (n <= e->row_max && e->alone && e->row_fe)
        hipLaunchKernelGGL(k_sig_blind_row, dim3(n), dim3(LBR_NT), 0, s2, n, e->sig_aff.as<uint32_t>(),
                           e->scalars.as<uint64_t>(), e->set_live.as<uint32_t>(), e->sig_inf.as<uint32_t>(),
                           e->s_terms.as<uint32_t>(), e->row_proj ? 1u : 0u);
      else if (n <= e->small_s_g8_max)
// ... 286 lines not shown
                           e->members.as<uint32_t>(), e->set_uid.as<uint32_t>(), e->scalars.as<uint64_t>(),
                           e->set_live.as<uint32_t>(), e->sig_inf.as<uint32_t>(), e->sig_aff.as<uint32_t>(), n,
                           e->s_terms.as<uint32_t>());
      else
        hipLaunchKernelGGL(k_smsm_terms_g8, dim3((T + 7) / 8), dim3(64), 0, s1, T, cm, ma, e->members.as<uint32_t>(),
                           e->set_uid.as<uint32_t>(), e->scalars.as<uint64_t>(), e->set_live.as<uint32_t>(),
                           e->sig_inf.as<uint32_t>(), e->sig_aff.as<uint32_t>(), n, e->s_terms.as<uint32_t>());
      if (nbk)
        hipLaunchKernelGGL(k_seg_sum64, dim3(nbk), dim3(64), 0, s1, U(SX_BLO), U(SX_BHI), T, e->s_terms.as<uint32_t>(),
                           nbk, e->s_part.as<uint32_t>(), nullptr);
      hipLaunchKernelGGL(k_seg_final, dim3(cm), dim3(64), 0, s1, U(SX_BO), e->s_part.as<uint32_t>(), nbk ? nbk : 1u,
                         U(SX_S), cm);
    } else if (cm) {
      LB_HIP(e->bcnt.ensure((size_t)nb * 4));
      LB_HIP(e->bcursor.ensure((size_t)nb * 4));
      LB_HIP(e->boff.ensure((size_t)(nb + 1) * 4));
      LB_HIP(e->bch.ensure((size_t)(nb + 1) * 4));
      LB_HIP(e->bchunk_beg.ensure((size_t)bcap * 4));
      LB_HIP(e->bchunk_end.ensure((size_t)bcap * 4));
      LB_HIP(e->bmembers.ensure((size_t)2 * nwin * (T ? T : 1) * 4));
      LB_HIP(e->bacc.ensure((size_t)bcap * sizeof(g2j)));
      LB_HIP(e->bsum.ensure((size_t)nb * sizeof(g2j)));
      LB_HIP(hipMemsetAsync(e->bcnt.p, 0, (size_t)nb * 4, s1));
      LB_HIP(hipMemsetAsync(e->bcursor.p, 0, (size_t)nb * 4, s1));
      const smsm_args ma{U(SX_MPRE), U(SX_MLO), U(SX_MMODE), U(SX_MWA), U(SX_MWB)};
      if (T) {
        if (w4)
          hipLaunchKernelGGL(k_smsm_count<LB_MSM_W>, dim3(nblk(T)), dim3(LB_TPB), 0, s1, T, cm, ma,
                             e->members.as<uint32_t>(), e->set_uid.as<uint32_t>(), e->scalars.as<uint64_t>(),
                             e->set_live.as<uint32_t>(), e->sig_inf.as<uint32_t>(), e->bcnt.as<uint32_t>());
        else
          hipLaunchKernelGGL(k_smsm_count<LB_SMSM_W>, dim3(nblk(T)), dim3(LB_TPB), 0, s1, T, cm, ma,
                             e->members.as<uint32_t>(), e->set_uid.as<uint32_t>(), e->scalars.as<uint64_t>(),
                             e->set_live.as<uint32_t>(), e->sig_inf.as<uint32_t>(), e->bcnt.as<uint32_t>());
      }
      hipLaunchKernelGGL(k_msg_scan, dim3(1), dim3(1024), 0, s1, nullptr, nb, schunk, e->bcnt.as<uint32_t>(),
                         e->boff.as<uint32_t>(), e->bch.as<uint32_t>(), e->bchunk_beg.as<uint32_t>(),
                         e->bchunk_end.as<uint32_t>(), nullptr, nullptr);
      if (T) {
        if (w4)
          hipLaunchKernelGGL(k_smsm_scatter<LB_MSM_W>, dim3(nblk(T)), dim3(LB_TPB), 0, s1, T, cm, ma,
                             e->members.as<uint32_t>(), e->set_uid.as<uint32_t>(), e->scalars.as<uint64_t>(),
                             e->set_live.as<uint32_t>(), e->sig_inf.as<uint32_t>(), e->boff.as<uint32_t>(),
                             e->bcursor.as<uint32_t>(), e->bmembers.as<uint32_t>());
        else
          hipLaunchKernelGGL(k_smsm_scatter<LB_SMSM_W>, dim3(nblk(T)), dim3(LB_TPB), 0, s1, T, cm, ma,
                             e->members.as<uint32_t>(), e->set_uid.as<uint32_t>(), e->scalars.as<uint64_t>(),
                             e->set_live.as<uint32_t>(), e->sig_inf.as<uint32_t>(), e->boff.as<uint32_t>(),
                             e->bcursor.as<uint32_t>(), e->bmembers.as<uint32_t>());
      }
      hipLaunchKernelGGL(k_msm_chunks, dim3(nblk(bcap)), dim3(LB_TPB), 0, s1, e->bch.as<uint32_t>(),
                         e->bchunk_beg.as<uint32_t>(), e->bchunk_end.as<uint32_t>(), e->bmembers.as<uint32_t>(),
                         e->sig_aos.as<uint4>(), bcap, e->bacc.as<uint32_t>(), nb);
      LB_HIP(msm_reduce(e, s1, bcap, nb, cm, w4 ? LB_MSM_W : LB_SMSM_W, U(SX_S), cm, 0u, (uint64_t)2 * nwin * T,
                        schunk));
    }
    if (c)
      hipLaunchKernelGGL(k_range_pk, dim3(nblk(c)), dim3(LB_TPB), 0, s1, c, U(SX_KIND), U(SX_LO), U(SX_LEN),
                         e->members.as<uint32_t>(), e->set_live.as<uint32_t>(), n, e->rpk.as<uint32_t>(), U(SX_PK));
    if (nt)
      hipLaunchKernelGGL(k_test_pk, dim3(nt), dim3(64), 0, s1, nt, U(SX_TMODE), U(SX_TLO), U(SX_TLEN), U(SX_TPER),
                         e->members.as<uint32_t>(), e->set_live.as<uint32_t>(), n, e->rpk.as<uint32_t>(), U(SX_TPK));
  }
  {
    stage_scope sc(e, ST_BISECT, s1);
    const srch_items I{c, nt, n_fresh, e->search_merge ? 0u : 1u, U(SX_KIND), U(SX_KEY), U(SX_MIDX), U(SX_TMODE), U(SX_TF), U(SX_TV0),
                       U(SX_TU), U(SX_TMIDX), U(SX_TYIDX)};
    auto stage = [&](uint32_t it0, uint32_t cnt) {
      if (!cnt) return;
      hipLaunchKernelGGL(k_search_ml, dim3(2 * cnt), dim3(64), 0, s1, I, it0, cnt, cm ? cm : 1u, e->treeP.as<uint32_t>(),
                         2 * x.mu, U(SX_PK), U(SX_TPK), e->h_aff.as<uint32_t>(), n, U(SX_S), e->pk_aff.as<uint32_t>(),
                         e->sig_aff.as<uint32_t>(), e->sig_inf.as<uint32_t>(), e->set_live.as<uint32_t>(),
                         e->set_uid.as<uint32_t>(), U(SX_Y), U(SX_ML));
      hipLaunchKernelGGL(k_search_fe, dim3(cnt), dim3(64), 0, s1, I, it0, cnt, U(SX_ML), U(SX_Y),
                         e->sx[SX_VERDICT].as<int32_t>());
    };
    if (e->search_merge) {
      stage(0, c + nt);
    } else {
      stage(0, c + n_fresh);
      stage(c + n_fresh, nt - n_fresh);
    }
    if (nt) hipLaunchKernelGGL(k_search_match, dim3(nt), dim3(64), 0, s1, I, U(SX_YUP), U(SX_Y), e->sx[SX_TOUT].as<int32_t>());
  }
  LB_HIP(hipGetLastError());
  verdict.resize(c);
  ydir.resize((size_t)144 * N);
  tout.resize(nt);
  if (c) {
    LB_HIP(hipMemcpyAsync(verdict.data(), e->sx[SX_VERDICT].p, (size_t)c * 4, hipMemcpyDeviceToHost, s1));
    LB_HIP(hipMemcpyAsync(ydir.data(), e->sx[SX_Y].p, (size_t)N * 576, hipMemcpyDeviceToHost, s1));
  }
  if (nt) LB_HIP(hipMemcpyAsync(tout.data(), e->sx[SX_TOUT].p, (size_t)nt * 4, hipMemcpyDeviceToHost, s1));
  LB_HIP(hipStreamSynchronize(s1));
  if (e->profiling)
    for (int k : {(int)ST_FALLBACK, (int)ST_BISECT}) {
      float ms = 0.f;
      if (e->used[k] && hipEventElapsedTime(&ms, e->ev0[k], e->ev1[k]) == hipSuccess) e->acc_ms[k] += ms;
      e->used[k] = false;
    }
  return LB_OK;
}

static int32_t search_root_sums(lb_engine* e, const search_ctx& x) {
  hipStream_t s1 = e->stream;
  const uint32_t n = x.n, nu = x.nu;
  std::vector<uint32_t> idx;
  std::vector<uint32_t> blo, bhi, bo{0};
  for (uint32_t u = 0; u < nu; u++) {
    for (uint32_t p = x.goff[u]; p < x.goff[u + 1]; p += 64) {
      blo.push_back(p);
      bhi.push_back(std::min(p + 64, x.goff[u + 1]));
    }
    bo.push_back((uint32_t)blo.size());
  }
  const uint32_t nbk = (uint32_t)blo.size();
  idx.insert(idx.end(), blo.begin(), blo.end());
  idx.insert(idx.end(), bhi.begin(), bhi.end());
  idx.insert(idx.end(), bo.begin(), bo.end());
  LB_HIP(e->rs_idx.ensure(idx.size() * 4));
  LB_HIP(e->s_set.ensure((size_t)n * sizeof(g2j)));
  LB_HIP(e->s_part.ensure((size_t)(nbk ? nbk : 1) * sizeof(g2j)));
  LB_HIP(e->s_root.ensure((size_t)nu * sizeof(g2j)));
  LB_HIP(hipMemcpyAsync(e->rs_idx.p, idx.data(), idx.size() * 4, hipMemcpyHostToDevice, s1));
  const uint32_t* d_idx = e->rs_idx.as<uint32_t>();
  {
    stage_scope sc(e, ST_FALLBACK, s1);
    hipLaunchKernelGGL(k_sig_blind, dim3(nblk_inv(n)), dim3(LB_INV_TPB), 0, s1, n, e->sig_aff.as<uint32_t>(),
                       e->scalars.as<uint64_t>(), e->set_live.as<uint32_t>(), e->sig_inf.as<uint32_t>(),
                       e->s_set.as<uint32_t>());
    if (nbk)
      hipLaunchKernelGGL(k_seg_sum64, dim3(nbk), dim3(64), 0, s1, d_idx, d_idx + nbk, n, e->s_set.as<uint32_t>(), nbk,
                         e->s_part.as<uint32_t>(), e->members.as<uint32_t>());
    hipLaunchKernelGGL(k_seg_final, dim3(nu), dim3(64), 0, s1, d_idx + 2 * nbk, e->s_part.as<uint32_t>(),
                       nbk ? nbk : 1u, e->s_root.as<uint32_t>(), nu);
  }
  LB_HIP(hipGetLastError());
  LB_HIP(hipStreamSynchronize(s1));
  if (e->profiling) {
    float ms = 0.f;
    if (e->used[ST_FALLBACK] && hipEventElapsedTime(&ms, e->ev0[ST_FALLBACK], e->ev1[ST_FALLBACK]) == hipSuccess)
      e->acc_ms[ST_FALLBACK] += ms;
    e->used[ST_FALLBACK] = false;
  }
  return LB_OK;
}

static int32_t search_invalid(lb_engine* e, lb_batch* b, uint32_t mu, int32_t* out_job) {
  const uint32_t n = b->n_sets, nj = b->n_jobs;
  if (e->rpk_stale && n) {
    hipLaunchKernelGGL(k_pk_blind, dim3(nblk_inv(n)), dim3(LB_INV_TPB), 0, e->stream, n, b->n_chunks,
                       b->d_set_chunk_off.as<uint32_t>(), e->chunk_acc.as<uint32_t>(), e->chunk_status.as<int32_t>(),
                       e->pk_aff.as<uint32_t>(), e->scalars.as<uint64_t>(), e->rpk.as<uint32_t>(),
                       e->pk_status.as<int32_t>(), 2u, nullptr);
    LB_HIP(hipGetLastError());
    e->rpk_stale = false;
  }
  search_ctx x;
  x.n = n;
  x.mu = mu;
  x.L = 0;
  while ((1u << x.L) < mu) x.L++;
  x.nu = *e->h_nu;
  x.goff.resize(x.nu + 1);
  x.members.resize(n);
  fnode root{{0u, 1u, 0u, n, 0u}, true, std::vector<uint32_t>(144)};
  LB_HIP(hipMemcpyAsync(x.goff.data(), e->goff.p, (size_t)(x.nu + 1) * 4, hipMemcpyDeviceToHost, e->stream));
  LB_HIP(hipMemcpyAsync(x.members.data(), e->members.p, (size_t)n * 4, hipMemcpyDeviceToHost, e->stream));
  LB_HIP(hipMemcpyAsync(root.y.data(), e->y_root.p, 576, hipMemcpyDeviceToHost, e->stream));
  LB_HIP(hipStreamSynchronize(e->stream));
  const bool r1_plain = e->search_blk && x.nu > 1 && n > e->search_small_max;
  if (!r1_plain && e->search_rootsum && x.nu > 1 && n > e->search_small_max) {
    const int32_t st = search_root_sums(e, x);
    if (st != LB_OK) return st;
    x.rs = true;
  }
  std::vector<fnode> F{root};
  std::vector<uint32_t> bad_pos;
  auto condemn = [&](const snode& a) {
    for (uint32_t q = 0; q < a.len; q++) bad_pos.push_back(a.lo + q);
  };
  const bool trace = std::getenv("LB_SEARCH_TRACE") != nullptr;
  const size_t kMaxMsm = 1024;
  std::vector<snode> ch;
  for (int round = 1; !F.empty(); round++) {
    if (round > 64) {
      for (const fnode& f : F) condemn(f.s);
      break;
    }
    std::vector<fnode> next;
    std::vector<fnode> work;
    for (fnode& f : F) {
      while (true) {
        if (f.s.len <= 1) {
          bad_pos.push_back(f.s.lo);
          break;
        }
        search_children(x, f.s, f.multi, ch);
        if (ch.size() == 1) {
          f.s = ch[0];
          f.multi = false;
          continue;
        }
        if (ch.empty()) condemn(f.s);
        else work.push_back(f);
        break;
      }
    }
    const bool spec_on = LB_SEARCH_SPEC && device_alone(e);
    for (size_t a = 0; a < work.size();) {
      std::vector<fnode> Fs;
      std::vector<snode> D;
      std::vector<uint32_t> d_owner;
      std::vector<test_job> fresh, spec, ahead;
      size_t inst = 0;
      while (a < work.size() && (Fs.empty() || inst < kMaxMsm)) {
        const fnode& f = work[a++];
        const uint32_t fi = (uint32_t)Fs.size();
        Fs.push_back(f);
        if (!f.multi) {
          test_job t{f.s, {}, true, fi};
          search_children(x, f.s, false, t.ch);
          if (spec_on && !t.ch.empty() && t.ch[0].kind == 0u && t.ch[0].d == x.L && f.s.len <= kSpecMaxSets)
            for (uint32_t k = 0; k < (uint32_t)t.ch.size(); k++) {
              test_job g{t.ch[k], {}, true, fi};
              search_children(x, t.ch[k], false, g.ch);
              if (g.ch.size() < 2) continue;
              g.spec = (int32_t)fresh.size();
              g.spec_k = k;
              spec.push_back(std::move(g));
              inst++;
            }
          fresh.push_back(std::move(t));
          inst++;
          continue;
        }
        std::vector<snode> dch;
        search_children(x, f.s, true, dch);
        for (const snode& c : dch) {
          const uint32_t di = (uint32_t)D.size();
          D.push_back(c);
          d_owner.push_back(fi);
          inst += c.kind != 2u;
          test_job t{c, {}, false, di};
          search_children(x, c, false, t.ch);
          if (t.ch.size() >= 2 && !(r1_plain && round == 1)) {
            ahead.push_back(std::move(t));
            inst++;
          }
        }
      }
      std::vector<test_job> tests(fresh);
      const uint32_t n_own = (uint32_t)fresh.size();
      tests.insert(tests.end(), spec.begin(), spec.end());
      const uint32_t n_fresh = (uint32_t)tests.size();
      tests.insert(tests.end(), ahead.begin(), ahead.end());
      std::vector<int32_t> verdict, tout;
      std::vector<uint32_t> ydir;
      const auto t0 = std::chrono::steady_clock::now();
      const int32_t st = search_round(e, x, Fs, D, tests, n_fresh, verdict, ydir, tout);
      if (st != LB_OK) return st;
      if (trace)
        std::fprintf(stderr, "[lb search] round %d: %zu failing nodes, %zu direct checks, %zu weighted tests: %.3f ms\n",
                     round, Fs.size(), D.size(), tests.size(),
                     std::chrono::duration<double, std::milli>(std::chrono::steady_clock::now() - t0).count());
      std::vector<int32_t> spec_of;
      std::vector<uint32_t> spec_base(n_own + 1, 0);
      for (uint32_t t = n_own; t < n_fresh; t++) spec_base[tests[t].spec + 1]++;
      for (uint32_t t = 0; t < n_own; t++) spec_base[t + 1] += spec_base[t];
      for (uint32_t t = n_own; t < n_fresh; t++) spec_of.push_back((int32_t)t);
      for (uint32_t t = 0; t < n_own; t++) {
        const fnode& f = Fs[tests[t].src];
        const int k = tout[t];
        if (k < 1 || (size_t)k > tests[t].ch.size()) {
          next.push_back({f.s, true, f.y});
          continue;
        }
        int32_t st = -1;
        for (uint32_t q = spec_base[t]; q < spec_base[t + 1]; q++)
          if (tests[spec_of[q]].spec_k == (uint32_t)(k - 1)) st = spec_of[q];
        if (st < 0) {
          next.push_back({tests[t].ch[k - 1], false, f.y});
          continue;
        }
        const int k2 = tout[st];
        if (k2 >= 1 && (size_t)k2 <= tests[st].ch.size()) next.push_back({tests[st].ch[k2 - 1], false, f.y});
        else next.push_back({tests[t].ch[k - 1], true, f.y});
      }
      std::vector<int> any_fail(Fs.size(), 0);
      std::vector<int32_t> ahead_of(D.size(), -1);
      for (uint32_t t = n_fresh; t < tests.size(); t++) ahead_of[tests[t].src] = (int32_t)t;
      for (uint32_t j = 0; j < D.size(); j++) {
        if (verdict[j]) continue;
        any_fail[d_owner[j]] = 1;
        std::vector<uint32_t> yc(144);
        for (int q = 0; q < 144; q++) yc[q] = ydir[(size_t)q * (D.size() + tests.size()) + j];
        const int32_t t = ahead_of[j];
        if (t < 0) {
          next.push_back({D[j], false, yc});
          continue;
        }
        const int k = tout[t];
        if (k >= 1 && (size_t)k <= tests[t].ch.size()) next.push_back({tests[t].ch[k - 1], false, yc});
        else next.push_back({D[j], true, yc});
      }
      for (size_t fi = 0; fi < Fs.size(); fi++)
        if (Fs[fi].multi && !any_fail[fi]) condemn(Fs[fi].s);
// ... 515 lines not shown
```

### lodestar_amd/csrc/lb_kdecl.h

```cpp
#pragma once

__global__ void k_decompress_sigs(uint32_t n, const uint8_t* __restrict__ sigs, const uint32_t* __restrict__ sig_sizes, uint32_t* __restrict__ sig_aff, uint4* __restrict__ sig_aos, uint32_t* __restrict__ sig_inf, int32_t* __restrict__ sig_status);
__global__ void k_sig_subgroup(uint32_t n, const uint32_t* __restrict__ sig_aff, const uint32_t* __restrict__ sig_inf, int32_t* __restrict__ sig_status);
__global__ void k_sig_subgroup_g8(uint32_t n, const uint32_t* __restrict__ sig_aff, const uint32_t* __restrict__ sig_inf, int32_t* __restrict__ sig_status);
__global__ void k_sig_subgroup_row(uint32_t n, const uint32_t* __restrict__ sig_aff, const uint32_t* __restrict__ sig_inf, int32_t* __restrict__ sig_status, uint32_t proj);
__global__ void k_hash_map(uint32_t n, uint32_t nu, const uint32_t* __restrict__ uniq_set, const uint8_t* __restrict__ msgs, uint32_t* __restrict__ q);
__global__ void k_decompress_sigs_row(uint32_t n, const uint8_t* __restrict__ sigs, const uint32_t* __restrict__ sig_sizes, uint32_t* __restrict__ sig_aff, uint4* __restrict__ sig_aos, uint32_t* __restrict__ sig_inf, int32_t* __restrict__ sig_status);
__global__ void k_hash_map_row(uint32_t n, uint32_t nu, const uint32_t* __restrict__ uniq_set, const uint8_t* __restrict__ msgs, uint32_t* __restrict__ q);
__global__ void k_hash_finish(uint32_t n, const uint32_t* __restrict__ n_u, const uint32_t* __restrict__ q, uint32_t* __restrict__ h_aff, uint32_t* __restrict__ park, uint32_t pn);
__global__ void k_hash_finish_g8(uint32_t n, const uint32_t* __restrict__ n_u, const uint32_t* __restrict__ q, uint32_t* __restrict__ h_aff);
__global__ void k_hash_finish_row(uint32_t n, const uint32_t* __restrict__ n_u, const uint32_t* __restrict__ q, uint32_t* __restrict__ h_aff, uint32_t careful);
__global__ void k_pk_chunks(uint32_t nc, const uint32_t* __restrict__ chunk_lo, const uint8_t* __restrict__ pks, uint32_t* __restrict__ chunk_acc, int32_t* __restrict__ chunk_status);
__global__ void k_pk_chunks_idx(uint32_t nc, const uint32_t* __restrict__ chunk_lo, const uint32_t* __restrict__ idx, const uint32_t* __restrict__ table, uint32_t table_n, uint32_t* __restrict__ chunk_acc, int32_t* __restrict__ chunk_status);
__global__ void k_table_fill(uint32_t n, const uint8_t* __restrict__ keys, uint32_t key_size, int32_t validate, uint32_t first, uint32_t* __restrict__ table, int32_t* __restrict__ status);
__global__ void k_pk_blind(uint32_t n, uint32_t nc, const uint32_t* __restrict__ set_chunk_off, const uint32_t* __restrict__ chunk_acc, const int32_t* __restrict__ chunk_status, uint32_t* __restrict__ pk_aff, const uint64_t* __restrict__ scalars, uint32_t* __restrict__ rpk, int32_t* __restrict__ pk_status, uint32_t mode, uint32_t* __restrict__ pk3);
__global__ void k_pk_blind_rowp(uint32_t n, const uint32_t* __restrict__ pk_aff, const uint64_t* __restrict__ scalars, uint32_t* __restrict__ rpk, const int32_t* __restrict__ pk_status);
__global__ void k_sig_subgroup_w4(uint32_t n, const uint32_t* __restrict__ sig_aff, const uint32_t* __restrict__ sig_inf, int32_t* __restrict__ sig_status);
__global__ void k_sig_blind_w4(uint32_t n, const uint32_t* __restrict__ sig_aff, const uint64_t* __restrict__ scalars, const uint32_t* __restrict__ sig_inf, uint32_t* __restrict__ terms);
template <int NL> __global__ void k_miller_lane(uint32_t n, uint32_t m, const uint32_t* __restrict__ n_u, const uint32_t* __restrict__ gp_aff, const uint32_t* __restrict__ gp_inf, const uint32_t* __restrict__ h_aff, uint32_t* __restrict__ treeP, uint32_t* __restrict__ tpark);
__global__ void k_miller_wave(uint32_t n, uint32_t m, const uint32_t* __restrict__ n_u, const uint32_t* __restrict__ gp_aff, const uint32_t* __restrict__ gp_inf, const uint32_t* __restrict__ h_aff, uint32_t* __restrict__ treeP);
__global__ void k_msg_insert(uint32_t n, const uint8_t* __restrict__ msgs, uint64_t key, uint32_t cap, uint32_t* __restrict__ tab, uint32_t* __restrict__ rep_of);
__global__ void k_dedup_one(uint32_t* __restrict__ rep_of, uint32_t* __restrict__ uid_of, uint32_t* __restrict__ uniq_set, uint32_t* __restrict__ n_u, uint32_t* __restrict__ set_uid, uint32_t* __restrict__ cnt, uint32_t* __restrict__ pos, uint32_t* __restrict__ goff, uint32_t* __restrict__ gch, uint32_t* __restrict__ chunk_beg, uint32_t* __restrict__ chunk_end, uint32_t* __restrict__ chunk_root, uint32_t* __restrict__ members);
__global__ void k_msg_uid_input(uint32_t n, const uint32_t* __restrict__ rep_of, uint32_t* __restrict__ uid_of, uint32_t* __restrict__ uniq_set, uint32_t* __restrict__ n_u);
__global__ void k_msg_uid(uint32_t cap, const uint32_t* __restrict__ tab, uint32_t* __restrict__ uid_of, uint32_t* __restrict__ uniq_set, uint32_t* __restrict__ n_u);
__global__ void k_msg_count(uint32_t n, const uint32_t* __restrict__ rep_of, const uint32_t* __restrict__ uid_of, uint32_t* __restrict__ set_uid, uint32_t* __restrict__ cnt, uint32_t* __restrict__ pos);
__global__ void k_msg_scan(const uint32_t* __restrict__ n_u, uint32_t nu_const, uint32_t chunk, const uint32_t* __restrict__ cnt, uint32_t* __restrict__ goff, uint32_t* __restrict__ gch, uint32_t* __restrict__ chunk_beg, uint32_t* __restrict__ chunk_end, uint32_t* __restrict__ chunk_root, uint32_t* __restrict__ max_chunks);
__global__ void k_chunk_fill(const uint32_t* __restrict__ n_u, uint32_t chunk, const uint32_t* __restrict__ goff, const uint32_t* __restrict__ gch, uint32_t* __restrict__ chunk_beg, uint32_t* __restrict__ chunk_end, uint32_t* __restrict__ chunk_root);
__global__ void k_msg_scatter(uint32_t n, const uint32_t* __restrict__ set_uid, const uint32_t* __restrict__ pos, const uint32_t* __restrict__ goff, uint32_t* __restrict__ members);
__global__ void k_msm_count(uint32_t n, const uint64_t* __restrict__ scalars, const uint32_t* __restrict__ set_live, const uint32_t* __restrict__ sig_inf, uint32_t* __restrict__ cnt);
__global__ void k_msm_scatter(uint32_t n, const uint64_t* __restrict__ scalars, const uint32_t* __restrict__ set_live, const uint32_t* __restrict__ sig_inf, const uint32_t* __restrict__ boff, uint32_t* __restrict__ cursor, uint32_t* __restrict__ members);
__global__ void k_msm_chunks(const uint32_t* __restrict__ bch, const uint32_t* __restrict__ chunk_beg, const uint32_t* __restrict__ chunk_end, const uint32_t* __restrict__ members, const uint4* __restrict__ sig_aos, uint32_t cap, uint32_t* __restrict__ bacc, uint32_t nb);
__global__ void k_msm_buckets(const uint32_t* __restrict__ bch, const uint32_t* __restrict__ bacc, uint32_t cap, uint32_t* __restrict__ bsum, uint32_t nb);
template <int W> __global__ void k_msm_reduce(const uint32_t* __restrict__ bsum, uint32_t nb, uint32_t* __restrict__ out, uint32_t n_out, uint32_t out0);
__global__ void k_msm_buckets_g8(const uint32_t* __restrict__ bch, const uint32_t* __restrict__ bacc, uint32_t cap, uint32_t* __restrict__ bsum, uint32_t nb);
__global__ void k_msm_window_g8(const uint32_t* __restrict__ bsum, uint32_t nb, uint32_t* __restrict__ wsum, uint32_t n_w);
template <int W> __global__ void k_msm_horner_g8(const uint32_t* __restrict__ wsum, uint32_t n_inst, uint32_t* __restrict__ out, uint32_t n_out, uint32_t out0);
__global__ void k_sig_blind_g8(uint32_t n, const uint32_t* __restrict__ sig_aff, const uint64_t* __restrict__ scalars, const uint32_t* __restrict__ set_live, const uint32_t* __restrict__ sig_inf, uint32_t* __restrict__ terms);
__global__ void k_sig_unblinded(const uint32_t* __restrict__ sig_aff, const uint32_t* __restrict__ set_live, const uint32_t* __restrict__ sig_inf, uint32_t n_out, uint32_t* __restrict__ out);
__global__ void k_sig_blind(uint32_t n, const uint32_t* __restrict__ sig_aff, const uint64_t* __restrict__ scalars, const uint32_t* __restrict__ set_live, const uint32_t* __restrict__ sig_inf, uint32_t* __restrict__ terms);
__global__ void k_g2_sum64(uint32_t n_in, const uint32_t* __restrict__ in, uint32_t n_out, uint32_t* __restrict__ out, uint32_t out0);
__global__ void k_sig_blind_row(uint32_t n, const uint32_t* __restrict__ sig_aff, const uint64_t* __restrict__ scalars, const uint32_t* __restrict__ set_live, const uint32_t* __restrict__ sig_inf, uint32_t* __restrict__ terms, uint32_t proj);
__global__ void k_g2_sum_g8(uint32_t n, const uint32_t* __restrict__ in, uint32_t n_out, uint32_t* __restrict__ out, uint32_t out0, const uint32_t* __restrict__ live);
template <int W> __global__ void k_smsm_count(uint32_t T, uint32_t c, smsm_args a, const uint32_t* __restrict__ members, const uint32_t* __restrict__ set_uid, const uint64_t* __restrict__ scalars, const uint32_t* __restrict__ set_live, const uint32_t* __restrict__ sig_inf, uint32_t* __restrict__ cnt);
template <int W> __global__ void k_smsm_scatter(uint32_t T, uint32_t c, smsm_args a, const uint32_t* __restrict__ members, const uint32_t* __restrict__ set_uid, const uint64_t* __restrict__ scalars, const uint32_t* __restrict__ set_live, const uint32_t* __restrict__ sig_inf, const uint32_t* __restrict__ boff, uint32_t* __restrict__ cursor, uint32_t* __restrict__ bmembers);
__global__ void k_smsm_terms_g8(uint32_t T, uint32_t c, smsm_args a, const uint32_t* __restrict__ members, const uint32_t* __restrict__ set_uid, const uint64_t* __restrict__ scalars, const uint32_t* __restrict__ set_live, const uint32_t* __restrict__ sig_inf, const uint32_t* __restrict__ sig_aff, uint32_t n, uint32_t* __restrict__ terms);
__global__ void k_smsm_terms_lane(uint32_t T, uint32_t c, smsm_args a, const uint32_t* __restrict__ members, const uint32_t* __restrict__ set_uid, const uint64_t* __restrict__ scalars, const uint32_t* __restrict__ set_live, const uint32_t* __restrict__ sig_inf, const uint32_t* __restrict__ sig_aff, uint32_t n, uint32_t* __restrict__ terms);
__global__ void k_seg_sum64(const uint32_t* __restrict__ blo, const uint32_t* __restrict__ bhi, uint32_t T, const uint32_t* __restrict__ terms, uint32_t nb, uint32_t* __restrict__ part, const uint32_t* __restrict__ perm);
__global__ void k_seg_final(const uint32_t* __restrict__ bo, const uint32_t* __restrict__ part, uint32_t nb, uint32_t* __restrict__ out, uint32_t n_out);
__global__ void k_rsm_terms(uint32_t T, uint32_t c, smsm_args a, const uint32_t* __restrict__ s_root, uint32_t nu, uint32_t* __restrict__ terms);
__global__ void k_smsm_terms_pre(uint32_t T, uint32_t c, smsm_args a, const uint32_t* __restrict__ members, const uint32_t* __restrict__ set_uid, const uint32_t* __restrict__ set_terms, uint32_t n, uint32_t* __restrict__ terms);
__global__ void k_range_pk(uint32_t c, const uint32_t* __restrict__ kind, const uint32_t* __restrict__ rlo, const uint32_t* __restrict__ rlen, const uint32_t* __restrict__ members, const uint32_t* __restrict__ set_live, uint32_t n, const uint32_t* __restrict__ rpk, uint32_t* __restrict__ pk_out);
__global__ void k_test_pk(uint32_t nt, const uint32_t* __restrict__ mode, const uint32_t* __restrict__ tlo, const uint32_t* __restrict__ tlen, const uint32_t* __restrict__ per, const uint32_t* __restrict__ members, const uint32_t* __restrict__ set_live, uint32_t n, const uint32_t* __restrict__ rpk, uint32_t* __restrict__ pk_out);
__global__ void k_search_ml(srch_items I, uint32_t it0, uint32_t cnt, uint32_t cm, const uint32_t* __restrict__ treeP, uint32_t n2m, const uint32_t* __restrict__ pk_d, const uint32_t* __restrict__ pk_t, const uint32_t* __restrict__ h_aff, uint32_t n, const uint32_t* __restrict__ s_out, const uint32_t* __restrict__ pk_aff, const uint32_t* __restrict__ sig_aff, const uint32_t* __restrict__ sig_inf, const uint32_t* __restrict__ set_live, const uint32_t* __restrict__ set_uid, const uint32_t* __restrict__ ybuf, uint32_t* __restrict__ ml);
__global__ void k_search_fe(srch_items I, uint32_t it0, uint32_t cnt, const uint32_t* __restrict__ ml, uint32_t* __restrict__ ybuf, int32_t* __restrict__ verdict);
__global__ void k_search_match(srch_items I, const uint32_t* __restrict__ y_up, const uint32_t* __restrict__ ybuf, int32_t* __restrict__ out_k);
__global__ void k_job_status(uint32_t n_jobs, const uint32_t* __restrict__ job_off, const int32_t* __restrict__ sig_status, const int32_t* __restrict__ pk_status, int32_t* __restrict__ job_status, uint32_t* __restrict__ set_live);
__global__ void k_spec_live(uint32_t n_jobs, const uint32_t* __restrict__ job_off, const int32_t* __restrict__ pk_status, uint32_t* __restrict__ set_spec);
__global__ void k_live_mismatch(uint32_t n, const uint32_t* __restrict__ set_live, const uint32_t* __restrict__ set_spec, uint32_t* __restrict__ flag);
__global__ void k_gsum_chunks(uint32_t n, const uint32_t* __restrict__ n_u, const uint32_t* __restrict__ gch, const uint32_t* __restrict__ chunk_beg, const uint32_t* __restrict__ chunk_end, const uint32_t* __restrict__ members, const uint32_t* __restrict__ set_live, const uint32_t* __restrict__ rpk, uint32_t* __restrict__ gacc);
__global__ void k_chunk_order(const uint32_t* __restrict__ n_u, const uint32_t* __restrict__ gch, const uint32_t* __restrict__ chunk_beg, const uint32_t* __restrict__ chunk_end, uint32_t* __restrict__ cnt, uint32_t* __restrict__ order, uint32_t pass);
__global__ void k_gsum_straus(uint32_t n, const uint32_t* __restrict__ n_u, const uint32_t* __restrict__ gch, const uint32_t* __restrict__ chunk_beg, const uint32_t* __restrict__ chunk_end, const uint32_t* __restrict__ order, const uint32_t* __restrict__ members, const uint32_t* __restrict__ set_live, const uint32_t* __restrict__ pk3, const uint64_t* __restrict__ scalars, uint32_t* __restrict__ gacc);
__global__ void k_gsum_wave(uint32_t n, const uint32_t* __restrict__ n_u, const uint32_t* __restrict__ gch, const uint32_t* __restrict__ chunk_beg, const uint32_t* __restrict__ chunk_end, const uint32_t* __restrict__ chunk_root, const uint32_t* __restrict__ members, const uint32_t* __restrict__ set_live, const uint32_t* __restrict__ rpk, uint32_t* __restrict__ gacc);
__global__ void k_gsum_tree(uint32_t n, const uint32_t* __restrict__ n_u, const uint32_t* __restrict__ gch, const uint32_t* __restrict__ chunk_root, uint32_t s, uint32_t* __restrict__ gacc);
__global__ void k_gsum_final(uint32_t n, const uint32_t* __restrict__ n_u, const uint32_t* __restrict__ gch, const uint32_t* __restrict__ gacc, uint32_t* __restrict__ gp_aff, uint32_t* __restrict__ gp_inf, uint32_t serial);
__global__ void k_set_one(uint32_t* __restrict__ base, uint32_t n, uint32_t e);
__global__ void k_g2_set_inf(uint32_t* __restrict__ base, uint32_t n, uint32_t e);
__global__ void k_tree_up_U(uint32_t m, uint32_t lo, const uint32_t* __restrict__ n_u, uint32_t* __restrict__ treeP);
__global__ void k_miller_row(uint32_t n, uint32_t m, const uint32_t* __restrict__ n_u, const uint32_t* __restrict__ gp_aff, const uint32_t* __restrict__ gp_inf, const uint32_t* __restrict__ h_aff, uint32_t* __restrict__ treeP);
__global__ void k_tree_up_row(uint32_t m, uint32_t lo, const uint32_t* __restrict__ n_u, uint32_t* __restrict__ treeP);
__global__ void k_ml_S(uint32_t m, const uint32_t* __restrict__ treeS, uint32_t* __restrict__ fS);
__global__ void k_ml_S_row(uint32_t m, const uint32_t* __restrict__ treeS, uint32_t* __restrict__ fS);
__global__ void k_root_check(uint32_t m, const uint32_t* __restrict__ treeP, const uint32_t* __restrict__ fS, int32_t* __restrict__ verdict, uint32_t* __restrict__ y_out);
__global__ void k_root_check_row(uint32_t m, const uint32_t* __restrict__ treeP, const uint32_t* __restrict__ fS, int32_t* __restrict__ verdict, uint32_t* __restrict__ y_out);
__global__ void k_root_partial(uint32_t m, const uint32_t* __restrict__ treeP, const uint32_t* __restrict__ fS, uint8_t* __restrict__ out576);
__global__ void k_root_partial_row(uint32_t m, const uint32_t* __restrict__ treeP, const uint32_t* __restrict__ fS, uint8_t* __restrict__ out576);
__global__ void k_partials_check(uint32_t n, const uint8_t* __restrict__ parts, int32_t* __restrict__ ok);
__global__ void k_partials_check_row(uint32_t n, const uint8_t* __restrict__ parts, int32_t* __restrict__ ok);
__global__ void k_pk_out96(uint32_t n, uint32_t nc, const uint32_t* __restrict__ set_chunk_off, const uint32_t* __restrict__ chunk_acc, const int32_t* __restrict__ chunk_status, uint8_t* __restrict__ out96, int32_t* __restrict__ status);
__global__ void k_sig_agg_chunks(uint32_t nc, const uint32_t* __restrict__ chunk_lo, const uint32_t* __restrict__ sig_aff, uint32_t n, const uint32_t* __restrict__ sig_inf, const int32_t* __restrict__ sig_status, uint32_t* __restrict__ chunk_acc, int32_t* __restrict__ chunk_status);
__global__ void k_sig_agg_groups(uint32_t ng, const uint32_t* __restrict__ group_chunk_off, const uint32_t* __restrict__ chunk_acc, uint32_t nc, const int32_t* __restrict__ chunk_status, uint8_t* __restrict__ out96, int32_t* __restrict__ status);
__global__ void k_g1_decompress(uint32_t n, const uint8_t* __restrict__ in48, uint8_t* __restrict__ out96, int32_t* __restrict__ status, int32_t validate);
__global__ void k_sk_to_pk(uint32_t n, const uint8_t* __restrict__ sks, uint8_t* __restrict__ out48, uint8_t* __restrict__ out96);
__global__ void k_sign(uint32_t n, const uint8_t* __restrict__ sks, const uint8_t* __restrict__ msgs, uint8_t* __restrict__ out96);
__global__ void k_miller_g8(uint32_t n, uint32_t m, const uint32_t* __restrict__ n_u, const uint32_t* __restrict__ gp_aff, const uint32_t* __restrict__ gp_inf, const uint32_t* __restrict__ h_aff, uint32_t* __restrict__ treeP);
__global__ void k_g1_terms(uint32_t n, const uint8_t* __restrict__ pts48, const uint32_t* __restrict__ table, uint32_t table_cap, const uint32_t* __restrict__ scalars, uint32_t* __restrict__ terms, int32_t* __restrict__ status);
__global__ void k_g1_sum64(uint32_t n_in, const uint32_t* __restrict__ in, uint32_t n_out, uint32_t* __restrict__ out);
__global__ void k_g1_out48(const uint32_t* __restrict__ in, uint32_t n, uint8_t* __restrict__ out48);
__global__ void k_kzg_setup_g1(uint32_t n, const uint8_t* __restrict__ in48, uint32_t* __restrict__ table, uint32_t cap, int32_t* __restrict__ status);
__global__ void k_kzg_setup_g2(const uint8_t* __restrict__ in96, uint32_t* __restrict__ g2, int32_t* __restrict__ status);
__global__ void k_kzg_check(const uint8_t* __restrict__ io, const uint32_t* __restrict__ yz, const uint32_t* __restrict__ g2, int32_t* __restrict__ ok);
__global__ void k_ssz_zero_hashes(uint8_t* __restrict__ zh);
__global__ void k_merkleize(uint32_t n, const uint32_t* __restrict__ chunk_off, const uint32_t* __restrict__ depth, const uint64_t* __restrict__ mix_len, uint8_t* __restrict__ chunks, const uint8_t* __restrict__ zh, uint8_t* __restrict__ roots);

#ifdef LB_KDECL_INSTANTIATE
#if LB_KG(4)
template __global__ void k_miller_lane<2>(uint32_t n, uint32_t m, const uint32_t* __restrict__ n_u, const uint32_t* __restrict__ gp_aff, const uint32_t* __restrict__ gp_inf, const uint32_t* __restrict__ h_aff, uint32_t* __restrict__ treeP, uint32_t* __restrict__ tpark);
template __global__ void k_miller_lane<3>(uint32_t n, uint32_t m, const uint32_t* __restrict__ n_u, const uint32_t* __restrict__ gp_aff, const uint32_t* __restrict__ gp_inf, const uint32_t* __restrict__ h_aff, uint32_t* __restrict__ treeP, uint32_t* __restrict__ tpark);
#endif
#if LB_KG(6)
template __global__ void k_msm_reduce<LB_MSM_W>(const uint32_t* __restrict__ bsum, uint32_t nb, uint32_t* __restrict__ out, uint32_t n_out, uint32_t out0);
template __global__ void k_msm_reduce<LB_SMSM_W>(const uint32_t* __restrict__ bsum, uint32_t nb, uint32_t* __restrict__ out, uint32_t n_out, uint32_t out0);
#endif
#if LB_KG(7)
template __global__ void k_smsm_count<LB_MSM_W>(uint32_t T, uint32_t c, smsm_args a, const uint32_t* __restrict__ members, const uint32_t* __restrict__ set_uid, const uint64_t* __restrict__ scalars, const uint32_t* __restrict__ set_live, const uint32_t* __restrict__ sig_inf, uint32_t* __restrict__ cnt);
template __global__ void k_smsm_count<LB_SMSM_W>(uint32_t T, uint32_t c, smsm_args a, const uint32_t* __restrict__ members, const uint32_t* __restrict__ set_uid, const uint64_t* __restrict__ scalars, const uint32_t* __restrict__ set_live, const uint32_t* __restrict__ sig_inf, uint32_t* __restrict__ cnt);
template __global__ void k_smsm_scatter<LB_MSM_W>(uint32_t T, uint32_t c, smsm_args a, const uint32_t* __restrict__ members, const uint32_t* __restrict__ set_uid, const uint64_t* __restrict__ scalars, const uint32_t* __restrict__ set_live, const uint32_t* __restrict__ sig_inf, const uint32_t* __restrict__ boff, uint32_t* __restrict__ cursor, uint32_t* __restrict__ bmembers);
template __global__ void k_smsm_scatter<LB_SMSM_W>(uint32_t T, uint32_t c, smsm_args a, const uint32_t* __restrict__ members, const uint32_t* __restrict__ set_uid, const uint64_t* __restrict__ scalars, const uint32_t* __restrict__ set_live, const uint32_t* __restrict__ sig_inf, const uint32_t* __restrict__ boff, uint32_t* __restrict__ cursor, uint32_t* __restrict__ bmembers);
#endif
#if LB_KG(9)
template __global__ void k_msm_horner_g8<LB_MSM_W>(const uint32_t* __restrict__ wsum, uint32_t n_inst, uint32_t* __restrict__ out, uint32_t n_out, uint32_t out0);
template __global__ void k_msm_horner_g8<LB_SMSM_W>(const uint32_t* __restrict__ wsum, uint32_t n_inst, uint32_t* __restrict__ out, uint32_t n_out, uint32_t out0);
#endif
#endif
#define LB_N_KGROUPS 15
```

### lodestar_amd/csrc/lb_kernels.h

```cpp
#pragma once
#include "lb_serial.h"
#include "lb_h2c.h"
#include "lb_pairing.h"

#define LB_TPB 64
#ifndef LB_MINW
#define LB_MINW 1
#endif
#ifndef LB_MINW_DEC
#define LB_MINW_DEC 2
#endif
#ifndef LB_MINW_SUB
#define LB_MINW_SUB LB_MINW_DEC
#endif
#ifndef LB_SUBGROUP_INL
#define LB_SUBGROUP_INL true
#endif
#ifndef LB_MINW_MSM
#define LB_MINW_MSM 1
#endif
#ifndef LB_MINW_GSUM
#define LB_MINW_GSUM 1
#endif
#ifndef LB_G1_INL
// ... 757 lines not shown
#ifndef LB_PK_CHUNK_SMALL
#define LB_PK_CHUNK_SMALL 4
#endif
#define LB_CHUNK_FIRST 0x80000000u
#define LB_CHUNK_LO(v) ((v) & 0x7fffffffu)

__device__ __forceinline__ g1j g1j_shfl_down(const g1j& a, unsigned d) {
  return g1j{fp_shfl_down(a.x, d), fp_shfl_down(a.y, d), fp_shfl_down(a.z, d)};
}
template <class F>
__device__ __forceinline__ jac<F> wave_seg_sum(jac<F> v, uint32_t rel, uint32_t left) {
  LB_UNROLL for (uint32_t s = 1; s < 64; s <<= 1) {
    const jac<F> o = jac_as<F>(g1j_shfl_down(jac_as<fp>(v), s));
    if ((rel & (2 * s - 1)) == 0 && s < left) v = jac_add_i<F, true>(v, o);
  }
  return v;
}
__device__ __forceinline__ void wave_segments(bool starts, uint32_t& rel, uint32_t& left) {
  const uint64_t heads = __ballot(starts) | 1ull;
  const uint32_t lane = threadIdx.x & 63;
  const uint64_t upto = lane == 63 ? ~0ull : ((2ull << lane) - 1);
  const uint32_t hl = 63 - __clzll(heads & upto);
  const uint64_t after = heads & ~upto;
  const uint32_t el = after ? (uint32_t)__ffsll((long long)after) - 1 : 64;
  rel = lane - hl;
  left = el - lane;
}
#if LB_KG(4)
__global__ void __launch_bounds__(LB_TPB, LB_MINW) k_pk_chunks(uint32_t nc, const uint32_t* __restrict__ chunk_lo,
                                                      const uint8_t* __restrict__ pks, uint32_t* __restrict__ chunk_acc,
                                                      int32_t* __restrict__ chunk_status) {
  uint32_t c = lb_tid();
  if (blockIdx.x * LB_TPB >= nc) return;
  const bool act = c < nc;
  const uint32_t cl = act ? chunk_lo[c] : LB_CHUNK_FIRST;
  int st = LB_OK;
  g1j acc = jac_infinity<fp>();
  if (act) {
    const uint32_t a = LB_CHUNK_LO(cl), e = LB_CHUNK_LO(chunk_lo[c + 1]);
    for (uint32_t k = a; k < e && st == LB_OK; k++) {
      uint8_t b[96];
      ld_bytes<96>(b, pks + (size_t)96 * k);
      g1a p;
      bool inf;
      st = g1_deserialize96(b, p, inf);
      if (st == LB_OK && !inf) acc = jac_add_aff(acc, p);
    }
  }
  uint32_t rel, left;
  wave_segments((cl & LB_CHUNK_FIRST) != 0, rel, left);
  acc = wave_seg_sum(acc, rel, left);
  if (!act) return;
  soa_st(chunk_acc, nc, c, acc);
  chunk_status[c] = st;
}
#endif

#define LB_TABLE_REC 32
struct g1x3 {
  fp x, y, bx;
};
__device__ __forceinline__ g1a table_ld(const uint32_t* __restrict__ table, uint32_t t) {
  return aos_ld<g1a>(table + (size_t)LB_TABLE_REC * t, 0);
}
__device__ __forceinline__ uint32_t table_flag_ld(const uint32_t* __restrict__ table, uint32_t t) {
  return table[(size_t)LB_TABLE_REC * t + 24];
}

#if LB_KG(4)
__global__ void __launch_bounds__(LB_TPB, LB_MINW_G1) k_pk_chunks_idx(uint32_t nc, const uint32_t* __restrict__ chunk_lo,
                                                          const uint32_t* __restrict__ idx,
                                                          const uint32_t* __restrict__ table, uint32_t table_n,
                                                          uint32_t* __restrict__ chunk_acc,
                                                          int32_t* __restrict__ chunk_status) {
  uint32_t c = lb_tid();
  if (blockIdx.x * LB_TPB >= nc) return;
  const bool act = c < nc;
  const uint32_t cl = act ? chunk_lo[c] : LB_CHUNK_FIRST;
  int st = LB_OK;
  jac<lb_g1f> acc = jac_infinity<lb_g1f>();
  if (act) {
    const uint32_t a = LB_CHUNK_LO(cl), e = LB_CHUNK_LO(chunk_lo[c + 1]);
    for (uint32_t k = a; k < e; k++) {
      uint32_t t = idx[k];
      if (t >= table_n) {
        st = LB_ERR_ARGUMENT;
        break;
      }
      const uint32_t fl = table_flag_ld(table, t);
      if (fl >> 1) {
        st = (int)(fl >> 1);
        break;
      }
      if (fl & 1u) continue;
      acc = jac_add_aff_i<lb_g1f, true>(acc, aff_as<lb_g1f>(table_ld(table, t)));
    }
  }
  uint32_t rel, left;
  wave_segments((cl & LB_CHUNK_FIRST) != 0, rel, left);
  acc = wave_seg_sum(acc, rel, left);
  if (!act) return;
  soa_st(chunk_acc, nc, c, jac_as<fp>(acc));
  chunk_status[c] = st;
}
#endif

#if LB_KG(0)
__global__ void __launch_bounds__(LB_TPB, LB_MINW) k_table_fill(uint32_t n, const uint8_t* __restrict__ keys,
                                                       uint32_t key_size, int32_t validate, uint32_t first,
                                                       uint32_t* __restrict__ table, int32_t* __restrict__ status) {
  uint32_t i = lb_tid();
  if (i >= n) return;
  g1a a;
  bool inf = false;
  int st;
  if (key_size == 48) {
    uint8_t b[48];
    for (int k = 0; k < 48; k++) b[k] = keys[(size_t)48 * i + k];
    st = g1_decompress48(b, a, inf);
  } else {
    uint8_t b[96];
    for (int k = 0; k < 96; k++) b[k] = keys[(size_t)96 * i + k];
    st = g1_deserialize96(b, a, inf);
  }
  if (st == LB_OK && validate) {
    if (inf) {
      st = LB_PK_IS_INFINITY;
    } else {
      const uint32_t rr[8] = {0x00000001u, 0xffffffffu, 0xfffe5bfeu, 0x53bda402u,
                              0x09a1d805u, 0x3339d808u, 0x299d7d48u, 0x73eda753u};
      if (!jac_is_inf(jac_mul_u256(a, rr))) st = LB_POINT_NOT_IN_GROUP;
    }
  }
  if (st != LB_OK) {
    a.x = fp_zero();
    a.y = fp_zero();
  }
  uint32_t* rec = table + (size_t)LB_TABLE_REC * (first + i);
  aos_st(rec, 0, a);
  uint4 tail = {((uint32_t)st << 1) | (inf ? 1u : 0u), 0u, 0u, 0u};
  reinterpret_cast<uint4*>(rec)[6] = tail;
  status[i] = st;
}
#endif

#if LB_KG(4)
__global__ void __launch_bounds__(LB_INV_TPB, LB_MINW_G1) k_pk_blind(uint32_t n, uint32_t nc, const uint32_t* __restrict__ set_chunk_off,
                                                         const uint32_t* __restrict__ chunk_acc,
                                                         const int32_t* __restrict__ chunk_status,
                                                         uint32_t* __restrict__ pk_aff,
                                                         const uint64_t* __restrict__ scalars,
                                                         uint32_t* __restrict__ rpk,
                                                         int32_t* __restrict__ pk_status, uint32_t mode,
                                                         uint32_t* __restrict__ pk3) {
  const uint32_t i = blockIdx.x * LB_INV_TPB + threadIdx.x;
  const bool act = i < n;
  int st = LB_ERR_ARGUMENT;
  g1j rj = jac_infinity<fp>();
  if (mode == 2) {
    if (!act) return;
    st = pk_status[i];
    if (st == LB_OK && scalars[i] == 1) {
      const g1a pk = soa_ld<g1a>(pk_aff, n, i);
      rj = g1j{pk.x, pk.y, fp_one()};
    } else if (st == LB_OK) {
      const g1a pk = soa_ld<g1a>(pk_aff, n, i);
      const g1a t2{fp_mul(pk.x, fp_load(LB_GLV_BETA)), pk.y};
      const g1a t3{fp_mul(pk.x, fp_load(LB_GLV_BETA2)), fp_neg(pk.y)};
#if LB_G1_INL
      rj = jac_as<fp>(jac_mul_glv_i<fpi, true>(aff_as<fpi>(pk), aff_as<fpi>(t2), aff_as<fpi>(t3), scalars[i]));
#else
      rj = jac_mul_glv_i<fp, true>(pk, t2, t3, scalars[i]);
#endif
    }
    aos_st(rpk, i, rj);
    return;
  }
  if (act) {
    uint32_t c0 = set_chunk_off[i], c1 = set_chunk_off[i + 1];
    st = (c0 == c1) ? LB_EMPTY_AGGREGATE_ARRAY : LB_OK;
    g1j acc = jac_infinity<fp>();
    for (uint32_t c = c0; c < c1 && st == LB_OK; c++) {
      st = chunk_status[c];
      if (st == LB_OK && (c == c0 || (c & (LB_TPB - 1)) == 0))
        acc = (c == c0) ? soa_ld<g1j>(chunk_acc, nc, c) : jac_add_i<fp, true>(acc, soa_ld<g1j>(chunk_acc, nc, c));
    }
    if (st == LB_OK && jac_is_inf(acc)) st = LB_PK_IS_INFINITY;
    rj = acc;
  }
  const bool ok = act && st == LB_OK;
  const fp one = fp_one();
  const bool need = ok && !fp_eq(rj.z, one);
  g1a pk;
  if (__syncthreads_or(need)) {
    const fp ai = fp_inv_block<true>(need ? rj.z : one);
    const fp ai2 = fp_sqr(ai);
    pk.x = fp_mul(rj.x, ai2);
    pk.y = fp_mul(fp_mul(rj.y, ai2), ai);
  } else {
    pk.x = rj.x;
    pk.y = rj.y;
  }
  if (mode == 1) {
    if (!act) return;
    if (ok) soa_st(pk_aff, n, i, pk);
    if (pk3 != nullptr) aos_st(pk3, i, g1x3{pk.x, pk.y, ok ? fp_mul(pk.x, fp_load(LB_GLV_BETA)) : fp_zero()});
    pk_status[i] = st;
    return;
  }
  if (ok) {
    const g1a t2{fp_mul(pk.x, fp_load(LB_GLV_BETA)), pk.y};
    const g1a t3{fp_mul(pk.x, fp_load(LB_GLV_BETA2)), fp_neg(pk.y)};
#if LB_G1_INL
    rj = jac_as<fp>(jac_mul_glv_i<fpi, true>(aff_as<fpi>(pk), aff_as<fpi>(t2), aff_as<fpi>(t3), scalars[i]));
#else
    rj = jac_mul_glv_i<fp, true>(pk, t2, t3, scalars[i]);
#endif
  } else {
    rj = jac_infinity<fp>();
  }
  if (!act) return;
  aos_st(rpk, i, rj);
  if (ok) soa_st(pk_aff, n, i, pk);
  pk_status[i] = st;
}
#endif

#if LB_KG(13)
__global__ void __launch_bounds__(64) k_pk_blind_rowp(uint32_t n, const uint32_t* __restrict__ pk_aff,
                                                     const uint64_t* __restrict__ scalars, uint32_t* __restrict__ rpk,
                                                     const int32_t* __restrict__ pk_status) {
  const uint32_t i = blockIdx.x;
  if (i >= n) return;
  const int st = pk_status[i];
  const uint64_t w = scalars[i];
  g1j rj = jac_infinity<fp>();
  if (st == LB_OK) {
    const g1a pk = soa_ld<g1a>(pk_aff, n, i);
    if (w == 1) {
      rj = g1j{pk.x, pk.y, fp_one()};
    } else {
      const aff<rfp> t1 = rf_of(pk);
      const aff<rfp> t2{f_mul(t1.x, rf_of(fp_load(LB_GLV_BETA))), t1.y};
      const aff<rfp> t3{f_mul(t1.x, rf_of(fp_load(LB_GLV_BETA2))), f_neg(t1.y)};
      const uint32_t k0 = (uint32_t)w, k1 = (uint32_t)(w >> 32);
      auto digit = [&](int b) { return ((k0 >> b) & 1u) | (((k1 >> b) & 1u) << 1); };
      int b = 31;
      while (b > 0 && digit(b) == 0) b--;
      auto tab = [&](uint32_t d) { return d == 1u ? t1 : (d == 2u ? t2 : t3); };
      const aff<rfp> top = tab(digit(b));
      rfp X = top.x, Y = top.y, Z;
      f_set_one(Z);
      for (b--; b >= 0; b--) {
        const uint32_t d = digit(b);
        rfp o[4];
        w4_mul<3>({X, Y, Y}, {X, Y, Z}, o);
        const rfp A = o[0], B = o[1], E = lz_mul(A, 3), XB = lz_add(X, B);
        const rfp Z3 = rf_red(2 * (int64_t)o[2].v);
        if (d == 0u) {
          w4_mul<3>({B, XB, E}, {B, XB, E}, o);
          const rfp C = o[0], D = lz_mul(lz_sub(lz_sub(o[1], A), C), 2);
          X = rf_red((int64_t)o[2].v - 2 * (int64_t)D.v);
          w4_mul<1>({E}, {lz_sub(D, X)}, o);
          Y = rf_red((int64_t)o[0].v - 8 * (int64_t)C.v);
          Z = Z3;
          continue;
        }
        const aff<rfp> q = tab(d);
        w4_mul<4>({B, XB, E, Z3}, {B, XB, E, Z3}, o);
        const rfp C = o[0], D = lz_mul(lz_sub(lz_sub(o[1], A), C), 2), Z1Z1 = o[3];
        const rfp X3 = rf_red((int64_t)o[2].v - 2 * (int64_t)D.v);
        w4_mul<3>({E, q.x, q.y}, {lz_sub(D, X3), Z1Z1, Z3}, o);
        const rfp Y3 = rf_red((int64_t)o[0].v - 8 * (int64_t)C.v), H = lz_sub(o[1], X3), Y2Z = o[2];
        const rfp ZH = lz_add(Z3, H);
        w4_mul<3>({Y2Z, H, ZH}, {Z1Z1, H, ZH}, o);
        const rfp rr = lz_mul(lz_sub(o[0], Y3), 2), HH = o[1], I = lz_mul(HH, 4);
        Z = rf_red((int64_t)o[2].v - Z1Z1.v - HH.v);
        w4_mul<3>({H, X3, rr}, {I, I, rr}, o);
        const rfp J = o[0], V = o[1];
        X = rf_red((int64_t)o[2].v - J.v - 2 * (int64_t)V.v);
        w4_mul<2>({rr, Y3}, {lz_sub(V, X), J}, o);
        Y = rf_red((int64_t)o[0].v - 2 * (int64_t)o[1].v);
      }
      rj = rf_fp(jac<rfp>{X, Y, Z});
    }
  }
  if (threadIdx.x == 0) aos_st(rpk, i, rj);
}
#endif

#if LB_KG(13)
__global__ void __launch_bounds__(64) k_sig_subgroup_w4(uint32_t n, const uint32_t* __restrict__ sig_aff,
                                                       const uint32_t* __restrict__ sig_inf,
                                                       int32_t* __restrict__ sig_status) {
  const uint32_t i = blockIdx.x;
  if (i >= n) return;
  if (sig_status[i] != LB_OK || sig_inf[i]) return;
  const g2a P = soa_ld<g2a>(sig_aff, n, i);
  const rfp2* t2 = nullptr;
  const rfp2 px = fl_in(P.x, t2), py = fl_in(P.y, t2);
  rfp2 X = px, Y = py, Z;
  f_set_one(Z);
#pragma clang loop unroll(disable)
  for (int b = 62; b >= 0; b--) {
    w4_g2_dbl(X, Y, Z);
    if ((LB_X_ABS >> b) & 1ull) w4_g2_madd(X, Y, Z, px, py);
  }
  bool ok;
  if (fp2_is_zero(fl_out(Z))) {
    ok = g2_aff_in_subgroup_i(P);
  } else {
    const rfp2 Z2 = f_sqr(Z);
    const rfp2 sx = f_mul(fl_conj(px), fl_in(fp2_load(LB_PSI_CX), t2));
    const rfp2 sy = f_mul(fl_conj(py), fl_in(fp2_load(LB_PSI_CY), t2));
    ok = fp2_eq(fl_out(f_mul(sx, Z2)), fl_out(X)) && fp2_eq(fl_out(f_mul(f_mul(sy, Z2), Z)), fl_out(f_neg(Y)));
  }
  if (!ok && threadIdx.x == 0) sig_status[i] = LB_POINT_NOT_IN_GROUP;
}
#endif
#if LB_KG(13)
__global__ void __launch_bounds__(64) k_sig_blind_w4(uint32_t n, const uint32_t* __restrict__ sig_aff,
                                                    const uint64_t* __restrict__ scalars,
                                                    const uint32_t* __restrict__ sig_inf, uint32_t* __restrict__ terms) {
  const uint32_t i = blockIdx.x;
  if (i >= n) return;
  const uint64_t w = scalars[i];
  g2j r = jac_infinity<fp2>();
  if (!sig_inf[i] && w != 0) {
    const g2a S = soa_ld<g2a>(sig_aff, n, i);
    const rfp2* t2p = nullptr;
    const rfp* t1p = nullptr;
    const rfp2 x1 = fl_in(S.x, t2p), y1 = fl_in(S.y, t2p);
    const rfp c2x = fl_in(fp_load(LB_PSI2_CX), t1p), c2y = fl_in(fp_load(LB_PSI2_CY), t1p);
    const rfp c4x = fl_in(fp_load(LB_PSI4_CX), t1p), c4y = fl_in(fp_load(LB_PSI4_CY), t1p);
    const rfp2 x2 = fl_mulb(x1, c2x), y2 = f_neg(fl_mulb(y1, c2y));
    const rfp2 x3 = fl_mulb(x1, c4x), y3 = f_neg(fl_mulb(y1, c4y));
    const uint32_t k0 = (uint32_t)w, k1 = (uint32_t)(w >> 32);
    auto digit = [&](int b) { return ((k0 >> b) & 1u) | (((k1 >> b) & 1u) << 1); };
    int b = 31;
    while (b > 0 && digit(b) == 0) b--;
    const uint32_t d0 = digit(b);
    rfp2 X = d0 == 1u ? x1 : (d0 == 2u ? x2 : x3), Y = d0 == 1u ? y1 : (d0 == 2u ? y2 : y3), Z;
    f_set_one(Z);
#pragma clang loop unroll(disable)
    for (b--; b >= 0; b--) {
      w4_g2_dbl(X, Y, Z);
      const uint32_t d = digit(b);
      if (d != 0u) w4_g2_madd(X, Y, Z, d == 1u ? x1 : (d == 2u ? x2 : x3), d == 1u ? y1 : (d == 2u ? y2 : y3));
    }
    r = g2j{fl_out(X), fl_out(Y), fl_out(Z)};
  }
  if (threadIdx.x == 0) soa_st(terms, n, i, r);
}
#endif

#ifndef LB_MILLER_LANE_REG
#define LB_MILLER_LANE_REG 0
#endif
typedef __attribute__((address_space(3))) uint32_t lds_w;
template <int NL>
struct lane_lds {
  lds_w* L;
  uint32_t* g;
  uint32_t n, u;
  int lane;
  __device__ __forceinline__ void put(int k, const fp6& v) const {
    const uint32_t* w = reinterpret_cast<const uint32_t*>(&v);
    if (k < NL)
      LB_UNROLL for (int i = 0; i < 72; i++) L[(k * 72 + i) * 64 + lane] = w[i];
    else
      LB_UNROLL for (int i = 0; i < 72; i++) g[((size_t)(k - 2) * 72 + i) * n + u] = w[i];
    __asm__ volatile("" ::: "memory");
  }
  __device__ __forceinline__ fp6 get(int k) const {
    __asm__ volatile("" ::: "memory");
    fp6 v;
    uint32_t* w = reinterpret_cast<uint32_t*>(&v);
// ... 1812 lines not shown
```

### lodestar_amd/engine.py

```python
from __future__ import annotations

import ctypes
from dataclasses import dataclass
from typing import List, Optional, Sequence, Tuple

import numpy as np

from . import _native as N


class BlsError(Exception):

    def __init__(self, code: int, message: Optional[str] = None):
        self.code = int(code)
        self.name = N.error_name(code)
        super().__init__(message if message is not None else self.name)


@dataclass
class SetInput:
    pubkeys: Sequence[bytes]
    signing_root: bytes
    signature: bytes

# ... 64 lines not shown

    def __init__(self, engine: "Engine", packed: PackedJobs):
        self.engine = engine
        self.packed = packed
        h = ctypes.c_void_p()
        if packed.pk_indices is not None:
            idx = np.ascontiguousarray(packed.pk_indices, dtype=np.uint32)
            if idx.size == 0:
                idx = np.zeros(1, dtype=np.uint32)
            _check(engine.lib.lb_batch_create_indexed(
                engine.h, packed.n_jobs, _p(packed.job_off, ctypes.c_uint32), _p(packed.pk_off, ctypes.c_uint32),
                _p(idx, ctypes.c_uint32), _p(packed.msgs, ctypes.c_uint8), _p(packed.sigs, ctypes.c_uint8),
                _p(packed.sig_sizes, ctypes.c_uint32), ctypes.byref(h)))
        else:
            _check(engine.lib.lb_batch_create(
                engine.h, packed.n_jobs, _p(packed.job_off, ctypes.c_uint32), _p(packed.pk_off, ctypes.c_uint32),
                _p(packed.pubkeys, ctypes.c_uint8), _p(packed.msgs, ctypes.c_uint8), _p(packed.sigs, ctypes.c_uint8),
                _p(packed.sig_sizes, ctypes.c_uint32), ctypes.byref(h)))
        self.h = h

    @property
    def n_jobs(self):
        return self.packed.n_jobs

    @property
    def n_sets(self):
        return self.packed.n_sets

    def verify(self, scalars: Optional[np.ndarray] = None) -> np.ndarray:
        out = np.zeros(max(self.n_jobs, 1), dtype=np.int32)
        sc = None if scalars is None else np.ascontiguousarray(scalars, dtype=np.uint64)
        _check(self.engine.lib.lb_batch_verify(self.engine.h, self.h, _p(sc, ctypes.c_uint64),
                                               _p(out, ctypes.c_int32)))
        return out[: self.n_jobs]

    def partial(self, scalars: Optional[np.ndarray] = None) -> Tuple[bytes, np.ndarray]:
        out = np.zeros(max(self.n_jobs, 1), dtype=np.int32)
        buf = (ctypes.c_uint8 * 576)()
        sc = None if scalars is None else np.ascontiguousarray(scalars, dtype=np.uint64)
        _check(self.engine.lib.lb_batch_partial(self.engine.h, self.h, _p(sc, ctypes.c_uint64),
                                                ctypes.cast(buf, ctypes.POINTER(ctypes.c_uint8)),
                                                _p(out, ctypes.c_int32)))
        return bytes(buf), out[: self.n_jobs]

    def search_after_partial(self, fallback: bool = True) -> np.ndarray:
        out = np.zeros(max(self.n_jobs, 1), dtype=np.int32)
        st = self.engine.lib.lb_batch_search_after_partial(self.engine.h, self.h, _p(out, ctypes.c_int32))
        if st == N.LB_ERR_ARGUMENT and fallback:
            return self.verify()
        _check(st)
        return out[: self.n_jobs]

    def free(self):
        if self.h:
            self.engine.lib.lb_batch_destroy(self.h)
            self.h = None

    def __del__(self):
        try:
            self.free()
        except Exception:
            pass


class Engine:

    LATENCY = 1

    def __init__(self, device: int = 0, flags: int = 0):
        self.lib = N.load()
        h = ctypes.c_void_p()
        _check(self.lib.lb_engine_create_ex(int(device), ctypes.c_uint32(flags), ctypes.byref(h)))
        self.h = h
        self.device = device

    def close(self):
        if self.h:
            self.lib.lb_engine_destroy(self.h)
            self.h = None

    def __enter__(self):
        return self

    def __exit__(self, *a):
        self.close()

    @property
    def cu_count(self) -> int:
        return int(self.lib.lb_engine_cu_count(self.h))

    def upload(self, jobs_or_packed) -> Batch:
        packed = jobs_or_packed if isinstance(jobs_or_packed, PackedJobs) else pack_jobs(jobs_or_packed)
        return Batch(self, packed)

    def verify_jobs(self, jobs, scalars: Optional[np.ndarray] = None) -> List[int]:
        return self.verify_jobs_packed(pack_jobs(jobs), scalars)

    def verify_jobs_packed(self, packed: PackedJobs, scalars: Optional[np.ndarray] = None) -> List[int]:
        out = np.zeros(max(packed.n_jobs, 1), dtype=np.int32)
        sc = None if scalars is None else np.ascontiguousarray(scalars, dtype=np.uint64)
        if packed.pk_indices is not None:
            idx = np.ascontiguousarray(packed.pk_indices, dtype=np.uint32)
            st = self.lib.lb_verify_jobs_indexed(
                self.h, packed.n_jobs, _p(packed.job_off, ctypes.c_uint32), _p(packed.pk_off, ctypes.c_uint32),
                _p(idx if idx.size else None, ctypes.c_uint32), _p(packed.msgs, ctypes.c_uint8),
                _p(packed.sigs, ctypes.c_uint8), _p(packed.sig_sizes, ctypes.c_uint32), _p(sc, ctypes.c_uint64),
                _p(out, ctypes.c_int32))
        else:
            st = self.lib.lb_verify_jobs(
                self.h, packed.n_jobs, _p(packed.job_off, ctypes.c_uint32), _p(packed.pk_off, ctypes.c_uint32),
                _p(packed.pubkeys, ctypes.c_uint8), _p(packed.msgs, ctypes.c_uint8), _p(packed.sigs, ctypes.c_uint8),
                _p(packed.sig_sizes, ctypes.c_uint32), _p(sc, ctypes.c_uint64), _p(out, ctypes.c_int32))
        _check(st)
        return [int(x) for x in out[: packed.n_jobs]]

    def verify_jobs_indexed(self, jobs, indices, scalars: Optional[np.ndarray] = None) -> List[int]:
        packed = pack_jobs([[SetInput([], s.signing_root, s.signature) for s in job] for job in jobs])
        counts = [len(ix) for jix in indices for ix in jix]
        packed.pk_off = np.zeros(len(counts) + 1, dtype=np.uint32)
        packed.pk_off[1:] = np.cumsum(counts, dtype=np.uint64).astype(np.uint32)
        packed.pubkeys = None
        packed.pk_indices = np.asarray([i for jix in indices for ix in jix for i in ix], dtype=np.uint32)
        return self.verify_jobs_packed(packed, scalars)

    def product_is_one(self, partials: Sequence[bytes]) -> bool:
        buf = np.frombuffer(b"".join(partials), dtype=np.uint8).copy() if partials else np.zeros(1, np.uint8)
        ok = ctypes.c_int32(0)
        _check(self.lib.lb_fp12_product_is_one(self.h, _p(buf, ctypes.c_uint8), len(partials), ctypes.byref(ok)))
        return bool(ok.value)

    def pubkey_table_append(self, keys: Sequence[bytes], validate: bool = False) -> Tuple[int, List[int]]:
        n = len(keys)
        if n == 0:
            return self.pubkey_table_size(), []
        if isinstance(keys, np.ndarray) and keys.ndim == 2:
            size = int(keys.shape[1])
            if size not in (48, 96):
                raise ValueError("keys must all be 48 or all be 96 bytes")
            buf = np.ascontiguousarray(keys, dtype=np.uint8).reshape(-1).copy()
        else:
            size = len(keys[0])
            if any(len(k) != size for k in keys) or size not in (48, 96):
                raise ValueError("keys must all be 48 or all be 96 bytes")
            buf = np.frombuffer(b"".join(bytes(k) for k in keys), dtype=np.uint8).copy()
        st = np.zeros(n, dtype=np.int32)
        first = ctypes.c_uint32(0)
        _check(self.lib.lb_pubkey_table_append(self.h, n, _p(buf, ctypes.c_uint8), size, 1 if validate else 0,
                                               _p(st, ctypes.c_int32), ctypes.byref(first)))
        return int(first.value), [int(x) for x in st]

    def pubkey_table_size(self) -> int:
        return int(self.lib.lb_pubkey_table_size(self.h))

    def aggregate_pubkeys(self, sets_pubkeys: Sequence[Sequence[bytes]]) -> Tuple[List[bytes], List[int]]:
        off = [0]
        flat = []
        for pks in sets_pubkeys:
            flat.extend(bytes(p) for p in pks)
            off.append(off[-1] + len(pks))
        n = len(sets_pubkeys)
        offa = np.asarray(off, dtype=np.uint32)
        pka = np.frombuffer(b"".join(flat), dtype=np.uint8).copy() if flat else np.zeros(1, np.uint8)
        out = np.zeros(max(n, 1) * 96, dtype=np.uint8)
        st = np.zeros(max(n, 1), dtype=np.int32)
        _check(self.lib.lb_aggregate_pubkeys(self.h, n, _p(offa, ctypes.c_uint32), _p(pka, ctypes.c_uint8),
                                             _p(out, ctypes.c_uint8), _p(st, ctypes.c_int32)))
        ob = out.tobytes()
        return [ob[96 * i: 96 * i + 96] for i in range(n)], [int(x) for x in st[:n]]

    def aggregate_signatures(self, groups: Sequence[Sequence[bytes]], validate: bool = True
                             ) -> Tuple[List[bytes], List[int]]:
        off = [0]
        flat, sizes, odd = [], [], False
        for g in groups:
            for sg in g:
                sg = bytes(sg)
                sizes.append(len(sg))
                if len(sg) != 96:
                    odd = True
                    sg = (sg + bytes(96))[:96]
                flat.append(sg)
            off.append(off[-1] + len(g))
        n = len(groups)
        offa = np.asarray(off, dtype=np.uint32)
        buf = np.frombuffer(b"".join(flat), dtype=np.uint8).copy() if flat else np.zeros(1, np.uint8)
        sz = np.asarray(sizes, dtype=np.uint32) if odd else None
        out = np.zeros(max(n, 1) * 96, dtype=np.uint8)
        st = np.zeros(max(n, 1), dtype=np.int32)
        _check(self.lib.lb_aggregate_signatures(self.h, n, _p(offa, ctypes.c_uint32), _p(buf, ctypes.c_uint8),
                                                _p(sz, ctypes.c_uint32), 1 if validate else 0,
                                                _p(out, ctypes.c_uint8), _p(st, ctypes.c_int32)))
        ob = out.tobytes()
        return [ob[96 * i: 96 * i + 96] for i in range(n)], [int(x) for x in st[:n]]

    def g1_decompress(self, pks48: Sequence[bytes], validate: bool = False) -> Tuple[List[bytes], List[int]]:
        n = len(pks48)
        if n == 0:
            return [], []
        inp = np.frombuffer(b"".join(bytes(p) for p in pks48), dtype=np.uint8).copy()
        out = np.zeros(n * 96, dtype=np.uint8)
        st = np.zeros(n, dtype=np.int32)
        _check(self.lib.lb_g1_decompress(self.h, n, _p(inp, ctypes.c_uint8), _p(out, ctypes.c_uint8),
                                         _p(st, ctypes.c_int32), 1 if validate else 0))
        ob = out.tobytes()
        return [ob[96 * i: 96 * i + 96] for i in range(n)], [int(x) for x in st]

    def sk_to_pk(self, sks: Sequence[int]) -> Tuple[np.ndarray, np.ndarray]:
        n = len(sks)
        sk = np.frombuffer(b"".join(int(s).to_bytes(32, "big") for s in sks), dtype=np.uint8).copy()
        o48 = np.zeros(n * 48, dtype=np.uint8)
        o96 = np.zeros(n * 96, dtype=np.uint8)
        _check(self.lib.lb_sk_to_pk(self.h, n, _p(sk, ctypes.c_uint8), _p(o48, ctypes.c_uint8),
                                    _p(o96, ctypes.c_uint8)))
        return o48.reshape(n, 48), o96.reshape(n, 96)

    def sign(self, sks: Sequence[int], msgs: np.ndarray) -> np.ndarray:
        n = len(sks)
        sk = np.frombuffer(b"".join(int(s).to_bytes(32, "big") for s in sks), dtype=np.uint8).copy()
        m = np.ascontiguousarray(msgs, dtype=np.uint8).reshape(-1)
        assert m.size == 32 * n
        out = np.zeros(n * 96, dtype=np.uint8)
        _check(self.lib.lb_sign(self.h, n, _p(sk, ctypes.c_uint8), _p(m, ctypes.c_uint8), _p(out, ctypes.c_uint8)))
        return out.reshape(n, 96)

    def set_profiling(self, on: bool):
        _check(self.lib.lb_engine_set_profiling(self.h, 1 if on else 0))

    def last_profile(self) -> dict:
        names = (ctypes.c_char_p * 32)()
        ms = (ctypes.c_float * 32)()
        n = ctypes.c_int32(0)
        _check(self.lib.lb_engine_last_profile(self.h, names, ms, 32, ctypes.byref(n)))
        return {names[i].decode(): float(ms[i]) for i in range(n.value)}
```

Baseline: 11.05 million sets/s.

## Precompute per-pubkey fixed-base comb tables for single-key set blinding

When a pubkey is appended to the GPU-resident table, a new kernel builds a 72-entry affine window table for it (9 windows by 8 digits, with GLV beta used to cover the high half of the scalar). During batch verify, sets that hold a single indexed pubkey are routed to a new kernel. That kernel computes the 64-bit blinding multiplication as 18 mixed additions from table lookups, in place of a double-and-add ladder. Multi-key sets still use the existing ladder through a selection list. The cost is a large device memory footprint (default cap 8 GiB), extra work at table append, and a table load per window that is bound by memory latency.

```diff
diff --git a/include/lodestar_bls.h b/include/lodestar_bls.h
--- a/include/lodestar_bls.h
+++ b/include/lodestar_bls.h
@@ -89,6 +89,8 @@
 int32_t lb_pubkey_table_append(lb_engine* e, uint32_t n, const uint8_t* keys, uint32_t key_size, int32_t validate,
                                int32_t* out_status, uint32_t* out_first_index);
 uint32_t lb_pubkey_table_size(const lb_engine* e);
+uint32_t lb_pubkey_comb_size(const lb_engine* e);
+uint64_t lb_pubkey_comb_sets(const lb_engine* e);
 
 int32_t lb_batch_create_indexed(lb_engine* e, uint32_t n_jobs, const uint32_t* job_offsets,
                                 const uint32_t* set_pk_offsets, const uint32_t* pk_indices,
diff --git a/lodestar_amd/_native.py b/lodestar_amd/_native.py
--- a/lodestar_amd/_native.py
+++ b/lodestar_amd/_native.py
@@ -67,6 +67,8 @@
     "lb_pubkey_table_append": (ctypes.c_int32, [_vp, ctypes.c_uint32, _u8p, ctypes.c_uint32, ctypes.c_int32, _i32p,
                                                 _u32p]),
     "lb_pubkey_table_size": (ctypes.c_uint32, [_vp]),
+    "lb_pubkey_comb_size": (ctypes.c_uint32, [_vp]),
+    "lb_pubkey_comb_sets": (ctypes.c_uint64, [_vp]),
     "lb_batch_create_indexed": (ctypes.c_int32, [_vp, ctypes.c_uint32, _u32p, _u32p, _u32p, _u8p, _u8p, _u32p,
                                                  ctypes.POINTER(_vp)]),
     "lb_engine_set_profiling": (ctypes.c_int32, [_vp, ctypes.c_int32]),
diff --git a/lodestar_amd/build.py b/lodestar_amd/build.py
--- a/lodestar_amd/build.py
+++ b/lodestar_amd/build.py
@@ -100,6 +100,22 @@
     return HARNESS
 
 
+COMB_HARNESS = os.path.join(ROOT, "build", "lb_comb_harness.so")
+
+
+def build_comb_harness(force=False, verbose=True):
+    src = os.path.join(ROOT, "tests", "harness", "lb_comb_harness.cpp")
+    os.makedirs(os.path.dirname(COMB_HARNESS), exist_ok=True)
+    if not force and not _stale(COMB_HARNESS, _deps() + [src]):
+        return COMB_HARNESS
+    cmd = ["g++", "-O2", "-shared", "-fPIC", "-I" + INC, "-I" + CSRC, src, "-o", COMB_HARNESS + ".tmp"]
+    if verbose:
+        print("[build]", " ".join(cmd), flush=True)
+    subprocess.run(cmd, check=True)
+    os.replace(COMB_HARNESS + ".tmp", COMB_HARNESS)
+    return COMB_HARNESS
+
+
 def build_cpu_pool(force=False, verbose=True):
     src = os.path.join(ROOT, "oracle", "cpu_pool.cpp")
     if not os.path.exists(src):
@@ -157,6 +173,7 @@
     build_lib(force)
     build_napi(force)
     build_harness(force)
+    build_comb_harness(force)
     build_cpu_pool(force)
     build_ubench(force)
 
diff --git a/lodestar_amd/csrc/lb_curve.h b/lodestar_amd/csrc/lb_curve.h
--- a/lodestar_amd/csrc/lb_curve.h
+++ b/lodestar_amd/csrc/lb_curve.h
@@ -198,6 +198,49 @@
   return jac_mul_glv_i(t1, t2, t3, w);
 }
 
+#define LB_COMB_J 9
+#define LB_COMB_D 8
+#define LB_COMB_ENTRIES (LB_COMB_J * LB_COMB_D)
+LB_HD int comb_digit(uint64_t w, int k) {
+  const uint64_t h = (k < LB_COMB_J ? (w & 0xffffffffu) : (w >> 32)) + 0x88888888ull;
+  const int j = k < LB_COMB_J ? k : k - LB_COMB_J;
+  return j < 8 ? (int)((h >> (4 * j)) & 15u) - 8 : (int)(h >> 32);
+}
+LB_HD uint32_t comb_entry(uint64_t w, int k) {
+  const int d = comb_digit(w, k), a = d < 0 ? -d : d;
+  return (uint32_t)(LB_COMB_D * (k < LB_COMB_J ? k : k - LB_COMB_J) + (a ? a - 1 : 0));
+}
+template <class F>
+LB_HD jac<F> jac_comb_entry_i(const aff<F>& p, int j, int d) {
+  jac<F> acc = jac_infinity<F>();
+  for (int b = 3; b >= 0; b--) {
+    acc = jac_dbl_i(acc);
+    jac<F> s = jac_add_aff_i<F, true>(acc, p);
+    if ((d >> b) & 1) acc = s;
+  }
+  for (int k = 0; k < 4 * j; k++) acc = jac_dbl_i(acc);
+  return acc;
+}
+template <class F, class Ld>
+LB_HD jac<F> jac_mul_comb_i(Ld&& ld, const F& beta, uint64_t w) {
+  jac<F> acc = jac_infinity<F>();
+  aff<F> nx = ld(comb_entry(w, 0));
+#if defined(__clang__)
+#pragma clang loop unroll(disable)
+#endif
+  for (int k = 0; k < 2 * LB_COMB_J; k++) {
+    aff<F> t = nx;
+    if (k + 1 < 2 * LB_COMB_J) nx = ld(comb_entry(w, k + 1));
+    const int d = comb_digit(w, k);
+    const bool skip = d == 0 || f_is_zero(t.y);
+    if (k >= LB_COMB_J) t.x = f_mul(t.x, beta);
+    t.y = f_select(d < 0, f_neg(t.y), t.y);
+    jac<F> s = jac_add_aff_i<F, true>(acc, t);
+    if (!skip) acc = s;
+  }
+  return acc;
+}
+
 template <class F>
 LB_NI jac<F> jac_mul_u64_jac(jac<F> p, uint64_t k) {
   jac<F> acc = jac_infinity<F>();
diff --git a/lodestar_amd/csrc/lb_engine.hip b/lodestar_amd/csrc/lb_engine.hip
--- a/lodestar_amd/csrc/lb_engine.hip
+++ b/lodestar_amd/csrc/lb_engine.hip
@@ -88,7 +88,10 @@
   std::vector<uint32_t> h_set_chunk_off, h_chunk_lo;
   uint32_t n_chunks = 0;
   bool indexed = false;
-  dbuf d_job_off, d_pk_off, d_pks, d_msgs, d_sigs, d_sig_sizes, d_set_chunk_off, d_chunk_lo;
+  std::vector<uint32_t> h_route;
+  uint32_t n_comb = 0;
+  const void* route_eng = nullptr;
+  dbuf d_job_off, d_pk_off, d_pks, d_msgs, d_sigs, d_sig_sizes, d_set_chunk_off, d_chunk_lo, d_route;
   dbuf d_arena;
   bool has_sizes = false;
   int device = 0;
@@ -102,6 +105,7 @@
     d_sig_sizes.release();
     d_set_chunk_off.release();
     d_chunk_lo.release();
+    d_route.release();
   }
 };
 
@@ -171,6 +175,9 @@
   std::vector<uint64_t> h_scalars;
   dbuf table;
   uint32_t table_n = 0, table_cap = 0;
+  dbuf comb;
+  uint32_t comb_n = 0, comb_cap = 0, comb_max = 0;
+  uint64_t comb_sets = 0;
   dbuf kzg_g1, kzg_g2;
   uint32_t kzg_n = 0;
   bool profiling = false;
@@ -371,6 +378,13 @@
   if (const char* sm = getenv("LB_MSM_G8")) e->msm_g8 = std::atoi(sm) != 0;
   if (const char* sm = getenv("LB_SPEC_GSUM")) e->spec_gsum = std::atoi(sm) != 0;
   if (const char* al = getenv("LB_ALONE")) e->alone_force = std::atoi(al) != 0 ? 1 : 0;
+  {
+    const char* on = getenv("LB_PK_COMB");
+    const char* mb = getenv("LB_PK_COMB_MB");
+    const double mib = mb ? std::max(0.0, strtod(mb, nullptr)) : 8192.0;
+    const uint64_t keys = (uint64_t)(mib * 1048576.0 / (double)(LB_COMB_ENTRIES * sizeof(g1a)));
+    e->comb_max = (on && std::atoi(on) == 0) ? 0u : (uint32_t)std::min<uint64_t>(keys, 0x7fffffffu);
+  }
   bool masked = false;
   std::vector<uint32_t> mask;
   {
@@ -474,7 +488,7 @@
   hipStreamSynchronize(e->stream);
   dbuf* bufs[] = {&e->scalars, &e->sig_aff, &e->sig_inf, &e->sig_status, &e->q, &e->h_aff, &e->rpk, &e->rsig,
                   &e->pk_status, &e->ml, &e->treeP, &e->treeS, &e->job_status, &e->nodes, &e->verdict, &e->parts,
-                  &e->ok, &e->chunk_acc, &e->chunk_status, &e->fS, &e->table, &e->msg_tab,
+                  &e->ok, &e->chunk_acc, &e->chunk_status, &e->fS, &e->table, &e->comb, &e->msg_tab,
                   &e->rep_of, &e->uid_of, &e->uniq_set, &e->n_u, &e->set_uid, &e->gcnt, &e->gpos, &e->goff,
                   &e->gch, &e->chunk_beg, &e->chunk_end, &e->members, &e->set_live, &e->gacc, &e->gp_aff,
                   &e->gp_inf, &e->chunk_root, &e->sig_aos, &e->bcnt, &e->bcursor, &e->boff, &e->bch, &e->bchunk_beg,
@@ -580,6 +594,22 @@
   b->n_chunks = (uint32_t)chunk_lo.size();
   chunk_lo.push_back(n_pks | LB_CHUNK_FIRST);
   b->indexed = indexed;
+  std::vector<uint32_t>& route = b->h_route;
+  route.clear();
+  b->n_comb = 0;
+  b->route_eng = nullptr;
+  if (indexed && e->comb_n) {
+    route.resize(n_sets);
+    uint32_t lo = 0, hi = n_sets;
+    for (uint32_t i = n_sets; i-- > 0;)
+      if (!(set_pk_offsets[i + 1] - set_pk_offsets[i] == 1 && pk_indices[set_pk_offsets[i]] < e->comb_n))
+        route[--hi] = i;
+    for (uint32_t i = 0; i < n_sets; i++)
+      if (set_pk_offsets[i + 1] - set_pk_offsets[i] == 1 && pk_indices[set_pk_offsets[i]] < e->comb_n)
+        route[lo++] = i;
+    b->n_comb = lo;
+    b->route_eng = e;
+  }
   struct part {
     dbuf* d;
     const void* src;
@@ -593,7 +623,8 @@
                          (size_t)n_pks * (indexed ? 4 : 96)},
                         {&b->d_msgs, signing_roots, (size_t)n_sets * 32},
                         {&b->d_sigs, signatures, (size_t)n_sets * 96},
-                        {&b->d_sig_sizes, sig_sizes, sig_sizes ? (size_t)n_sets * 4 : 0}};
+                        {&b->d_sig_sizes, sig_sizes, sig_sizes ? (size_t)n_sets * 4 : 0},
+                        {&b->d_route, route.data(), route.size() * 4}};
   size_t total = 0;
   for (const part& q : parts) total += ((q.bytes > 16 ? q.bytes : 16) + 255) & ~(size_t)255;
   bool staged = total <= kStageMax;
@@ -627,7 +658,7 @@
   if (r != hipSuccess) {
     for (const part& q : parts) q.d->release();
     b->d_arena.release();
-    b->n_jobs = b->n_sets = b->n_pks = b->n_chunks = 0;
+    b->n_jobs = b->n_sets = b->n_pks = b->n_chunks = b->n_comb = 0;
     b->job_off.assign(1, 0u);
     fprintf(stderr, "lodestar_bls: batch upload failed: %s\n", hipGetErrorString(r));
     return LB_ERR_DEVICE;
@@ -691,6 +722,8 @@
 }
 
 uint32_t lb_pubkey_table_size(const lb_engine* e) { return e ? e->table_n : 0; }
+uint32_t lb_pubkey_comb_size(const lb_engine* e) { return e ? e->comb_n : 0; }
+uint64_t lb_pubkey_comb_sets(const lb_engine* e) { return e ? e->comb_sets : 0; }
 
 int32_t lb_pubkey_table_append(lb_engine* e, uint32_t n, const uint8_t* keys, uint32_t key_size, int32_t validate,
                                int32_t* out_status, uint32_t* out_first_index) {
@@ -713,6 +746,28 @@
     e->table = nt;
     e->table_cap = cap;
   }
+  uint32_t comb_need = std::min(need, e->comb_max);
+  if (comb_need > e->comb_cap) {
+    const uint32_t cap = std::min(e->table_cap, e->comb_max);
+    const size_t rec = (size_t)LB_COMB_ENTRIES * sizeof(g1a);
+    dbuf nc;
+    hipError_t rc = nc.ensure((size_t)cap * rec);
+    if (rc == hipSuccess && e->comb_n)
+      rc = hipMemcpyAsync(nc.p, e->comb.p, (size_t)e->comb_n * rec, hipMemcpyDeviceToDevice, e->stream);
+    if (rc == hipSuccess) rc = hipStreamSynchronize(e->stream);
+    if (rc == hipSuccess) {
+      e->comb.release();
+      e->comb = nc;
+      e->comb_cap = cap;
+    } else {
+      nc.release();
+      (void)hipGetLastError();
+      fprintf(stderr, "lodestar_bls: no memory for %u keys' window tables (%s): coverage stays at %u keys\n", cap,
+              hipGetErrorString(rc), e->comb_n);
+      e->comb_max = e->comb_n;
+      comb_need = e->comb_n;
+    }
+  }
   dbuf kin, st;
   hipError_t r = kin.ensure((size_t)n * key_size);
   if (r == hipSuccess) r = st.ensure((size_t)n * 4);
@@ -722,6 +777,12 @@
                        validate, first, e->table.as<uint32_t>(), st.as<int32_t>());
     r = hipGetLastError();
   }
+  if (r == hipSuccess && comb_need > first) {
+    const uint32_t nk = comb_need - first;
+    hipLaunchKernelGGL(k_comb_fill, dim3((nk + 7) / 8, LB_COMB_J), dim3(LB_INV_TPB), 0, e->stream, nk, first,
+                       e->table.as<uint32_t>(), e->comb.as<uint32_t>());
+    r = hipGetLastError();
+  }
   if (r == hipSuccess) r = hipMemcpyAsync(out_status, st.p, (size_t)n * 4, hipMemcpyDeviceToHost, e->stream);
   if (r == hipSuccess) r = hipStreamSynchronize(e->stream);
   kin.release();
@@ -731,6 +792,7 @@
     return LB_ERR_DEVICE;
   }
   e->table_n = need;
+  e->comb_n = std::max(e->comb_n, comb_need);
   return LB_OK;
 }
 
@@ -958,7 +1020,27 @@
       const uint32_t m0 = (pk_split || e->straus_run) ? 1u : 0u;
       const uint32_t m1 = e->straus_run ? 1u : (pk_split ? 2u : 0u);
       if (e->straus_run) LB_HIP(e->pk3.ensure((size_t)ns * sizeof(g1x3)));
-      for (uint32_t mode = m0; mode <= m1; mode++) {
+      const bool route = b->indexed && b->n_comb && b->route_eng == e && !e->straus_run && !pk_rowp;
+      if (route) {
+        const uint32_t n_lad = n - b->n_comb;
+        const uint32_t* sel = b->d_route.as<uint32_t>();
+        hipLaunchKernelGGL(k_pk_blind, dim3(nblk_inv(n)), dim3(LB_INV_TPB), 0, s3, n, nc, b->d_set_chunk_off.as<uint32_t>(),
+                           e->chunk_acc.as<uint32_t>(), e->chunk_status.as<int32_t>(), e->pk_aff.as<uint32_t>(),
+                           e->scalars.as<uint64_t>(), e->rpk.as<uint32_t>(), e->pk_status.as<int32_t>(), 1u, nullptr,
+                           nullptr, 0u);
+        LB_HIP(hipEventRecord(e->ev_pkst, s3));
+        hipLaunchKernelGGL(k_pk_blind_comb, dim3(nblk(b->n_comb)), dim3(LB_TPB), 0, s3, n, b->n_comb, sel,
+                           b->d_pk_off.as<uint32_t>(), b->d_pks.as<uint32_t>(), e->comb.as<uint32_t>(), e->comb_n,
+                           e->pk_aff.as<uint32_t>(), e->scalars.as<uint64_t>(), e->pk_status.as<int32_t>(),
+                           e->rpk.as<uint32_t>());
+        e->comb_sets += b->n_comb;
+        if (n_lad)
+          hipLaunchKernelGGL(k_pk_blind, dim3(nblk_inv(n_lad)), dim3(LB_INV_TPB), 0, s3, n, nc,
+                             b->d_set_chunk_off.as<uint32_t>(), e->chunk_acc.as<uint32_t>(), e->chunk_status.as<int32_t>(),
+                             e->pk_aff.as<uint32_t>(), e->scalars.as<uint64_t>(), e->rpk.as<uint32_t>(),
+                             e->pk_status.as<int32_t>(), 2u, nullptr, sel + b->n_comb, n_lad);
+      }
+      for (uint32_t mode = m0; !route && mode <= m1; mode++) {
         if (mode == 2u && pk_rowp) {
           hipLaunchKernelGGL(k_pk_blind_rowp, dim3(n), dim3(64), 0, s3, n, e->pk_aff.as<uint32_t>(),
                              e->scalars.as<uint64_t>(), e->rpk.as<uint32_t>(), e->pk_status.as<int32_t>());
@@ -967,7 +1049,7 @@
         hipLaunchKernelGGL(k_pk_blind, dim3(nblk_inv(n)), dim3(LB_INV_TPB), 0, s3, n, nc, b->d_set_chunk_off.as<uint32_t>(),
                            e->chunk_acc.as<uint32_t>(), e->chunk_status.as<int32_t>(), e->pk_aff.as<uint32_t>(),
                            e->scalars.as<uint64_t>(), e->rpk.as<uint32_t>(), e->pk_status.as<int32_t>(), mode,
-                           (mode == 1u && e->straus_run) ? e->pk3.as<uint32_t>() : nullptr);
+                           (mode == 1u && e->straus_run) ? e->pk3.as<uint32_t>() : nullptr, nullptr, 0u);
         if (mode == 1u) LB_HIP(hipEventRecord(e->ev_pkst, s3));
       }
     }
@@ -1560,7 +1642,7 @@
     hipLaunchKernelGGL(k_pk_blind, dim3(nblk_inv(n)), dim3(LB_INV_TPB), 0, e->stream, n, b->n_chunks,
                        b->d_set_chunk_off.as<uint32_t>(), e->chunk_acc.as<uint32_t>(), e->chunk_status.as<int32_t>(),
                        e->pk_aff.as<uint32_t>(), e->scalars.as<uint64_t>(), e->rpk.as<uint32_t>(),
-                       e->pk_status.as<int32_t>(), 2u, nullptr);
+                       e->pk_status.as<int32_t>(), 2u, nullptr, nullptr, 0u);
     LB_HIP(hipGetLastError());
     e->rpk_stale = false;
   }
diff --git a/lodestar_amd/csrc/lb_kdecl.h b/lodestar_amd/csrc/lb_kdecl.h
--- a/lodestar_amd/csrc/lb_kdecl.h
+++ b/lodestar_amd/csrc/lb_kdecl.h
@@ -13,7 +13,9 @@
 __global__ void k_pk_chunks(uint32_t nc, const uint32_t* __restrict__ chunk_lo, const uint8_t* __restrict__ pks, uint32_t* __restrict__ chunk_acc, int32_t* __restrict__ chunk_status);
 __global__ void k_pk_chunks_idx(uint32_t nc, const uint32_t* __restrict__ chunk_lo, const uint32_t* __restrict__ idx, const uint32_t* __restrict__ table, uint32_t table_n, uint32_t* __restrict__ chunk_acc, int32_t* __restrict__ chunk_status);
 __global__ void k_table_fill(uint32_t n, const uint8_t* __restrict__ keys, uint32_t key_size, int32_t validate, uint32_t first, uint32_t* __restrict__ table, int32_t* __restrict__ status);
-__global__ void k_pk_blind(uint32_t n, uint32_t nc, const uint32_t* __restrict__ set_chunk_off, const uint32_t* __restrict__ chunk_acc, const int32_t* __restrict__ chunk_status, uint32_t* __restrict__ pk_aff, const uint64_t* __restrict__ scalars, uint32_t* __restrict__ rpk, int32_t* __restrict__ pk_status, uint32_t mode, uint32_t* __restrict__ pk3);
+__global__ void k_pk_blind(uint32_t n, uint32_t nc, const uint32_t* __restrict__ set_chunk_off, const uint32_t* __restrict__ chunk_acc, const int32_t* __restrict__ chunk_status, uint32_t* __restrict__ pk_aff, const uint64_t* __restrict__ scalars, uint32_t* __restrict__ rpk, int32_t* __restrict__ pk_status, uint32_t mode, uint32_t* __restrict__ pk3, const uint32_t* __restrict__ sel, uint32_t n_sel);
+__global__ void k_comb_fill(uint32_t n, uint32_t first, const uint32_t* __restrict__ table, uint32_t* __restrict__ comb);
+__global__ void k_pk_blind_comb(uint32_t n, uint32_t n_sel, const uint32_t* __restrict__ sel, const uint32_t* __restrict__ pk_off, const uint32_t* __restrict__ idx, const uint32_t* __restrict__ comb, uint32_t comb_n, const uint32_t* __restrict__ pk_aff, const uint64_t* __restrict__ scalars, const int32_t* __restrict__ pk_status, uint32_t* __restrict__ rpk);
 __global__ void k_pk_blind_rowp(uint32_t n, const uint32_t* __restrict__ pk_aff, const uint64_t* __restrict__ scalars, uint32_t* __restrict__ rpk, const int32_t* __restrict__ pk_status);
 __global__ void k_sig_subgroup_w4(uint32_t n, const uint32_t* __restrict__ sig_aff, const uint32_t* __restrict__ sig_inf, int32_t* __restrict__ sig_status);
 __global__ void k_sig_blind_w4(uint32_t n, const uint32_t* __restrict__ sig_aff, const uint64_t* __restrict__ scalars, const uint32_t* __restrict__ sig_inf, uint32_t* __restrict__ terms);
@@ -112,4 +114,4 @@
 template __global__ void k_msm_horner_g8<LB_SMSM_W>(const uint32_t* __restrict__ wsum, uint32_t n_inst, uint32_t* __restrict__ out, uint32_t n_out, uint32_t out0);
 #endif
 #endif
-#define LB_N_KGROUPS 15
+#define LB_N_KGROUPS 16
diff --git a/lodestar_amd/csrc/lb_kernels.h b/lodestar_amd/csrc/lb_kernels.h
--- a/lodestar_amd/csrc/lb_kernels.h
+++ b/lodestar_amd/csrc/lb_kernels.h
@@ -933,8 +933,10 @@
                                                          const uint64_t* __restrict__ scalars,
                                                          uint32_t* __restrict__ rpk,
                                                          int32_t* __restrict__ pk_status, uint32_t mode,
-                                                         uint32_t* __restrict__ pk3) {
-  const uint32_t i = blockIdx.x * LB_INV_TPB + threadIdx.x;
+                                                         uint32_t* __restrict__ pk3,
+                                                         const uint32_t* __restrict__ sel, uint32_t n_sel) {
+  uint32_t i = blockIdx.x * LB_INV_TPB + threadIdx.x;
+  if (mode == 2 && sel != nullptr) i = i < n_sel ? sel[i] : n;
   const bool act = i < n;
   int st = LB_ERR_ARGUMENT;
   g1j rj = jac_infinity<fp>();
@@ -1004,6 +1006,60 @@
   aos_st(rpk, i, rj);
   if (ok) soa_st(pk_aff, n, i, pk);
   pk_status[i] = st;
+}
+#endif
+
+#if LB_KG(15)
+__global__ void __launch_bounds__(LB_INV_TPB, LB_MINW_G1) k_comb_fill(uint32_t n, uint32_t first,
+                                                          const uint32_t* __restrict__ table,
+                                                          uint32_t* __restrict__ comb) {
+  const uint32_t k = blockIdx.x * 8 + (threadIdx.x >> 3);
+  const int d = (int)(threadIdx.x & 7u) + 1, j = (int)blockIdx.y;
+  const bool in = k < n;
+  const uint32_t t = first + (in ? k : 0u);
+  const bool act = in && table_flag_ld(table, t) == 0u;
+  jac<lb_g1f> acc = jac_infinity<lb_g1f>();
+  if (act) acc = jac_comb_entry_i<lb_g1f>(aff_as<lb_g1f>(table_ld(table, t)), j, d);
+  const bool inf = jac_is_inf(acc);
+  const fp zi = fp_inv_block<true>(inf ? fp_one() : fp{acc.z});
+  g1a a{fp_zero(), fp_zero()};
+  if (!inf) {
+    const fp zi2 = fp_sqr(zi);
+    a.x = fp_mul(acc.x, zi2);
+    a.y = fp_mul(fp_mul(acc.y, zi2), zi);
+  }
+  if (in) aos_st(comb + ((size_t)t * LB_COMB_ENTRIES + (size_t)(LB_COMB_D * j + d - 1)) * 24, 0, a);
+}
+#endif
+
+#if LB_KG(15)
+__global__ void __launch_bounds__(LB_TPB, LB_MINW_G1) k_pk_blind_comb(uint32_t n, uint32_t n_sel,
+                                                             const uint32_t* __restrict__ sel,
+                                                             const uint32_t* __restrict__ pk_off,
+                                                             const uint32_t* __restrict__ idx,
+                                                             const uint32_t* __restrict__ comb, uint32_t comb_n,
+                                                             const uint32_t* __restrict__ pk_aff,
+                                                             const uint64_t* __restrict__ scalars,
+                                                             const int32_t* __restrict__ pk_status,
+                                                             uint32_t* __restrict__ rpk) {
+  const uint32_t s = lb_tid();
+  if (s >= n_sel) return;
+  const uint32_t i = sel[s];
+  if (i >= n) return;
+  g1j rj = jac_infinity<fp>();
+  if (pk_status[i] == LB_OK) {
+    const uint64_t w = scalars[i];
+    const uint32_t key = idx[pk_off[i]];
+    if (w == 1) {
+      const g1a pk = soa_ld<g1a>(pk_aff, n, i);
+      rj = g1j{pk.x, pk.y, fp_one()};
+    } else if (key < comb_n) {
+      const uint32_t* base = comb + (size_t)key * LB_COMB_ENTRIES * 24;
+      rj = jac_as<fp>(jac_mul_comb_i<lb_g1f>([&](uint32_t e) { return aff_as<lb_g1f>(aos_ld<g1a>(base, e)); },
+                                             lb_g1f{fp_load(LB_GLV_BETA)}, w));
+    }
+  }
+  aos_st(rpk, i, rj);
 }
 #endif
 
diff --git a/lodestar_amd/engine.py b/lodestar_amd/engine.py
--- a/lodestar_amd/engine.py
+++ b/lodestar_amd/engine.py
@@ -240,6 +240,12 @@
     def pubkey_table_size(self) -> int:
         return int(self.lib.lb_pubkey_table_size(self.h))
 
+    def pubkey_comb_size(self) -> int:
+        return int(self.lib.lb_pubkey_comb_size(self.h))
+
+    def pubkey_comb_sets(self) -> int:
+        return int(self.lib.lb_pubkey_comb_sets(self.h))
+
     def aggregate_pubkeys(self, sets_pubkeys: Sequence[Sequence[bytes]]) -> Tuple[List[bytes], List[int]]:
         off = [0]
         flat = []
```

Measured after the change: 11.65 million sets/s, median of 6. +5.4%, better.
